# zhouxian/act3d-chained-diffuser

Measured on AMD Instinct MI355X. Metric: train samples/sec (Act3D keypose fwd+bwd+AdamW step), higher is better.
Workload: dtype fp16 / bf16 MFMA on two-part operands (x = hi + lo; fp32 accumulate) in attention; fp32-accurate linears (f32 MFMA; bf16x3 MFMA from 4096 rows); bf16 frozen backbone + FPN; 1 GPU; Act3D keypose training step, 18-PerAct-task shapes: 4 cameras 256x256, 3 ghost-point levels, 1000 ghost points (333/level), E=60, frozen synthetic CLIP-RN50-shaped backbone + trainable FPN included in the step; per_gpu_batch_keyframes=64, global_batch=64, parallelism=dp1, hipgraph=True, backbone_prefetch=True

## Files before the change

### act3d-chained-diffuser_amd/csrc/a3d_common.h

```cpp
#pragma once
#include <hip/hip_runtime.h>
#include <stdint.h>
#include <math.h>

#define A3D_OK 0
#define A3D_ERR_ARG (-22)
#define A3D_ERR_LAUNCH (-5)
#define A3D_ERR_NOMEM (-12)

namespace a3d {

void set_error(const char* fmt, ...);
int check_launch(const char* what);
int zero_words(void* p, size_t bytes, hipStream_t s, const char* what);

typedef __attribute__((ext_vector_type(4))) float f32x4;
typedef __attribute__((ext_vector_type(8))) short s16x8;
typedef __attribute__((ext_vector_type(8))) __bf16 bf16x8;
typedef __attribute__((ext_vector_type(4))) short s16x4;

constexpr int HD = 15;
constexpr float LOG2E_F = 1.4426950408889634f;
constexpr int HDP = 16;

// ... 83 lines not shown
  *sn = (q & 2) ? -s0 : s0;
  *cs = ((q + 1) & 2) ? -c0 : c0;
}
__host__ __device__ __forceinline__ void fast_sincos(float x, float* sn, float* cs) {
#if defined(A3D_LIBM_SINCOS) && defined(__HIP_DEVICE_COMPILE__)
  sincosf(x, sn, cs);
#else
  if (fabsf(x) >= 200.0f) {
    const double t = (double)x;
    const double k = rint(t * 0.15915494309189535);
    x = (float)fma(-k, 2.4492935982947064e-16, fma(-k, 6.283185307179586, t));
  }
  sincos_poly(x, sn, cs);
#endif
}

__device__ __forceinline__ float add_rn(float a, float b) {
#pragma clang fp contract(off)
  return a + b;
}
__device__ __forceinline__ float sub_rn(float a, float b) {
#pragma clang fp contract(off)
  return a - b;
}
__device__ __forceinline__ float mul_rn(float a, float b) {
#pragma clang fp contract(off)
  return a * b;
}
__device__ __forceinline__ float sqrt_rn(float a) { return __builtin_sqrtf(a); }

__host__ __device__ __forceinline__ void philox4x32_10(uint32_t c0, uint32_t c1, uint32_t c2, uint32_t c3,
                                                       uint32_t k0, uint32_t k1, uint32_t out[4]) {
  for (int r = 0; r < 10; ++r) {
    const uint64_t p0 = (uint64_t)0xD2511F53u * c0;
    const uint64_t p1 = (uint64_t)0xCD9E8D57u * c2;
    const uint32_t n0 = (uint32_t)(p1 >> 32) ^ c1 ^ k0;
    const uint32_t n1 = (uint32_t)p1;
    const uint32_t n2 = (uint32_t)(p0 >> 32) ^ c3 ^ k1;
    const uint32_t n3 = (uint32_t)p0;
    c0 = n0; c1 = n1; c2 = n2; c3 = n3;
    k0 += 0x9E3779B9u; k1 += 0xBB67AE85u;
  }
  out[0] = c0; out[1] = c1; out[2] = c2; out[3] = c3;
}

struct DropKey { uint32_t k0, k1; };
__device__ __forceinline__ DropKey drop_key(const unsigned long long* state) {
  const unsigned long long seed = state[0], offs = state[1];
  const unsigned long long key = seed + offs * 0x9E3779B97F4A7C15ull;
  DropKey k;
  k.k0 = (uint32_t)key;
  k.k1 = (uint32_t)(key >> 32);
  return k;
}
__device__ __forceinline__ uint32_t drop_keep8(DropKey k, uint32_t c0, uint32_t c1, uint32_t c2, uint32_t site,
                                               uint32_t thr16) {
  uint32_t r[4];
  philox4x32_10(c0, c1, c2, site, k.k0, k.k1, r);
  uint32_t bits = 0;
#pragma unroll
  for (int w = 0; w < 4; ++w) {
    bits |= ((r[w] & 0xFFFFu) >= thr16 ? 1u : 0u) << (2 * w);
    bits |= ((r[w] >> 16) >= thr16 ? 1u : 0u) << (2 * w + 1);
  }
  return bits;
}

__device__ __forceinline__ bool xcd_decode(int per_group, int ngroups, int& group, int& within) {
  const int id = blockIdx.x;
  const int xcd = id & 7, slot = id >> 3;
  group = (slot / per_group) * 8 + xcd;
  within = slot % per_group;
  return group < ngroups;
}
static inline int xcd_grid(int ngroups, int per_group) { return ((ngroups + 7) / 8) * 8 * per_group; }

static inline int cdiv(int a, int b) { return (a + b - 1) / b; }

bool conv1x1_deep_serves(int K, int N);
int conv1x1_deep_slabs(size_t M, int K, int N);
int conv1x1_deep_launch(const void* x, const void* w, const float* in_scale, const float* in_shift, int in_relu, void* y, float* partial,
                        size_t M, int K, int N, hipStream_t s);

}
```

### act3d-chained-diffuser_amd/csrc/attention16.hip

```cpp
#include "attn_ring.h"
#include "../../include/act3d_hip.h"
#include <stdlib.h>

namespace a3d {

constexpr float LO_SPAN = 6.0f;
constexpr int A3D_ATTN16_V_ROWS = 1, A3D_ATTN16_NOGRAD = 2;
constexpr int FWD_NB = 4;
template <bool DROP, int QT, int PP, bool VR>
__global__ __launch_bounds__(256, 2) void attn16_fwd_kernel(
    const unsigned short* __restrict__ Qr, const unsigned short* __restrict__ Kr, const unsigned short* __restrict__ Vp,
    const unsigned char* __restrict__ kmask, float* __restrict__ O, float* __restrict__ LSE2, float* __restrict__ Op,
    float* __restrict__ Mp, float* __restrict__ Lp, int B, int H, int Lq, int Lqp, int S, int Sp, int nsplit,
    const unsigned long long* __restrict__ drop_state, unsigned int drop_site, unsigned int drop_thr, float drop_scale) {
  __shared__ __attribute__((aligned(16))) unsigned short Ksm[FWD_NB][C16 * 32];
  __shared__ __attribute__((aligned(16))) unsigned short Vsm[FWD_NB][4 * 16 * 32];
  __shared__ unsigned int maskW[MASKW];

  const int t = threadIdx.x, lane = t & 63;
  const int wave = __builtin_amdgcn_readfirstlane(t >> 6);
  const int li = lane & 15, g = lane >> 4;
  constexpr int QW = 64 * QT;
  const int tiles_x = (Lqp + QW - 1) / QW;
  int group, within;
// ... 568 lines not shown
      s16x8 kf[2], vf[2], kp[2];
#pragma unroll
      for (int T = 0; T < 2; ++T) {
        kf[T] = *reinterpret_cast<const s16x8*>(kb + DQ_KJ(hf * 2 + T));
        vf[T] = *reinterpret_cast<const s16x8*>(kb + C16 * 32 + DQ_KJ(hf * 2 + T));
      }
      kp[0] = tr_frag(tb0 + hf * 1024, 0, 128);
      kp[1] = tr_frag(tb1 + hf * 1024, 0, 128);
      f32x4 sT[QT][2], dpT[QT][2];
      if (masked) {
        const unsigned int word = maskW[c * 2 + hf];
#pragma unroll
        for (int T = 0; T < 2; ++T) {
          const f32x4 b4 = bias_of(word, g, T);
#pragma unroll
          for (int u = 0; u < QT; ++u) sT[u][T] = mfma_f16(kf[T], qhi[u], cS[u] + b4);
        }
      } else {
#pragma unroll
        for (int u = 0; u < QT; ++u)
#pragma unroll
          for (int T = 0; T < 2; ++T) sT[u][T] = mfma_f16(kf[T], qhi[u], cS[u]);
      }
#pragma unroll
      for (int u = 0; u < QT; ++u)
#pragma unroll
        for (int T = 0; T < 2; ++T) {
          dpT[u][T] = mfma_f16(vf[T], dohi[u], cD[u]);
          sT[u][T] = mfma_f16(kf[T], qlo[u], sT[u][T]);
        }
#pragma unroll
      for (int u = 0; u < QT; ++u)
#pragma unroll
        for (int T = 0; T < 2; ++T) dpT[u][T] = mfma_f16(vf[T], dolo[u], dpT[u][T]);
#pragma unroll
      for (int u = 0; u < QT; ++u) {
        unsigned int keep = 0xFFu;
        if (DROP) keep = drop_keep8(dkey, (uint32_t)(c * (C16 / 8) + hf * 4 + g), (uint32_t)(qbase + u * 16 + li), (uint32_t)bh, drop_site, drop_thr);
        unsigned int w[4], wl[4];
#pragma unroll
        for (int T = 0; T < 2; ++T) {
#pragma unroll
          for (int pr = 0; pr < 2; ++pr) {
            const float p0 = __builtin_amdgcn_exp2f(sT[u][T][2 * pr]), p1 = __builtin_amdgcn_exp2f(sT[u][T][2 * pr + 1]);
            float g0, g1;
            if (DROP) {
              const int j = T * 4 + 2 * pr;
              const float m0 = ((keep >> j) & 1u) ? drop_scale : 0.f, m1 = ((keep >> (j + 1)) & 1u) ? drop_scale : 0.f;
              g0 = p0 * __builtin_fmaf(m0, dpT[u][T][2 * pr], nd[u]);
              g1 = p1 * __builtin_fmaf(m1, dpT[u][T][2 * pr + 1], nd[u]);
            } else {
              g0 = p0 * dpT[u][T][2 * pr];
              g1 = p1 * dpT[u][T][2 * pr + 1];
            }
            if (GP == 2) pk_f16_2(g0, g1, w[T * 2 + pr], wl[T * 2 + pr]);
            else w[T * 2 + pr] = pk_f16(g0, g1);
          }
        }
        const s16x8 gf = __builtin_bit_cast(s16x8, (u32x4_){w[0], w[1], w[2], w[3]});
        f32x4& acc = hf ? acc1[u] : acc0[u];
        acc = mfma_f16(kp[0], gf, acc);
        acc = mfma_f16(kp[1], gf, acc);
        if (GP == 2) acc = mfma_f16(kp[0], __builtin_bit_cast(s16x8, (u32x4_){wl[0], wl[1], wl[2], wl[3]}), acc);
      }
    }
  }
  wait_vm<0>();
#undef DQ_KJ
#pragma unroll
  for (int u = 0; u < QT; ++u) {
    if (!active[u]) continue;
    const size_t row = (((size_t)sp * B + b) * H + h) * Lqp + qbase + u * 16 + li;
    f32x4 acc;
#pragma unroll
    for (int r = 0; r < 4; ++r) acc[r] = (acc0[u][r] + acc1[u][r]) * rs[u];
    *reinterpret_cast<f32x4*>(&dQp[row * HDP + g * 4]) = acc;
  }
}

constexpr int DKV_NB = 2;
template <bool DROP, int KT, int GP>
__global__ __launch_bounds__(256, 2) void attn16_bwd_dkv_kernel(
    const unsigned short* __restrict__ pack, const unsigned short* __restrict__ Kr, const unsigned short* __restrict__ Vr,
    const unsigned char* __restrict__ kmask, float* __restrict__ dK, float* __restrict__ dV, int B, int H, int Lqp, int S,
    int Sp, const unsigned long long* __restrict__ drop_state, unsigned int drop_site, unsigned int drop_thr,
    float drop_scale) {
  __shared__ __attribute__((aligned(16))) unsigned short pk[DKV_NB][PK_HALFS];
  __shared__ __attribute__((aligned(16))) unsigned char maskS[2][DROP ? 8 * KT * C16 : 16];
  const int t = threadIdx.x, lane = t & 63;
  const int wave = __builtin_amdgcn_readfirstlane(t >> 6);
  const int li = lane & 15, g = lane >> 4;
  constexpr int KW = 64 * KT;
  int group, within;
  if (!xcd_decode((Sp + KW - 1) / KW, B * H, group, within)) return;
  group = __builtin_amdgcn_readfirstlane(group);
  within = __builtin_amdgcn_readfirstlane(within);
  const int b = __builtin_amdgcn_readfirstlane(group / H), h = group - b * H;
  const size_t bh = (size_t)b * H + h;

  s16x8 khh[KT], kll[KT], vhh[KT], vll[KT];
  f32x4 bias4[KT];
  int key[KT];
#pragma unroll
  for (int u = 0; u < KT; ++u) {
    key[u] = within * KW + (wave * KT + u) * 16 + li;
    khh[u] = s16x8{0, 0, 0, 0, 0, 0, 0, 0};
    kll[u] = khh[u]; vhh[u] = khh[u]; vll[u] = khh[u];
    bool valid = false;
    if (key[u] < Sp) {
      const unsigned short* kp = Kr + (bh * Sp + key[u]) * 32;
      const unsigned short* vp = Vr + (bh * Sp + key[u]) * 32;
      khh[u] = *reinterpret_cast<const s16x8*>(kp + (g & 1) * 8);
      kll[u] = *reinterpret_cast<const s16x8*>(kp + 16 + (g & 1) * 8);
      vhh[u] = *reinterpret_cast<const s16x8*>(vp + (g & 1) * 8);
      vll[u] = *reinterpret_cast<const s16x8*>(vp + 16 + (g & 1) * 8);
      valid = key[u] < S;
      if (valid && kmask) valid = kmask[(size_t)b * S + key[u]] == 0;
    }
    const float bias_k = valid ? 0.f : -INFINITY;
    bias4[u] = f32x4{bias_k, bias_k, bias_k, bias_k};
  }
  const bool masked = (kmask != nullptr) || (within * KW + KW > S);
  bool live[KT];
  bool any_live = false;
#pragma unroll
  for (int u = 0; u < KT; ++u) {
    live[u] = within * KW + (wave * KT + u) * 16 < S;
    any_live = any_live || live[u];
  }
  DropKey dkey = {0u, 0u};
  if (DROP) dkey = drop_key(drop_state);
#pragma unroll
  for (int u = 0; u < KT; ++u) { A3D_PIN(khh[u]); A3D_PIN(kll[u]); A3D_PIN(vhh[u]); A3D_PIN(vll[u]); A3D_PIN(bias4[u]); }
  if (DROP) { A3D_PIN(dkey.k0); A3D_PIN(dkey.k1); }

  const int nch = Lqp / C16;
  const unsigned short* pbase = pack + bh * nch * (size_t)PK_HALFS + wave * 2560 + lane * 8;
  auto issue = [&](int c, int slot) {
    const unsigned short* src = pbase + (size_t)min(c, nch - 1) * PK_HALFS;
#pragma unroll
    for (int i = 0; i < 5; ++i) glds16(src + i * 512, &pk[slot][wave * 2560 + i * 512]);
  };

#define DKV_QJ(j) ((((j) >> 1) * 32 + ((j) & 1) * 4) * 32)
  const int qoff0 = tile_off((li >> 2) * 8 + (li & 3), g);
  const int poff = plane_off(li, g);

  f32x4 dk0[KT], dk1[KT], dv0[KT], dv1[KT];
#pragma unroll
  for (int u = 0; u < KT; ++u) { dk0[u] = f32x4{0.f, 0.f, 0.f, 0.f}; dk1[u] = dk0[u]; dv0[u] = dk0[u]; dv1[u] = dk0[u]; }
  int e_ref = -1000;
#pragma unroll
  for (int i = 0; i < DKV_NB - 1; ++i) issue(i, i);
  for (int c = 0; c < nch; ++c) {
    const int slot = c % DKV_NB;
    wait_vm<5 * (DKV_NB - 2)>();
    ring_barrier();
    issue(c + DKV_NB - 1, (slot + DKV_NB - 1) % DKV_NB);
    const unsigned short* P = pk[slot];
    const int e_c = __builtin_amdgcn_readfirstlane(*reinterpret_cast<const int*>(P + PK_HDR));
    if (e_c <= -1000) continue;
    const int halves = __builtin_amdgcn_readfirstlane(reinterpret_cast<const int*>(P + PK_HDR)[1]);
    if (e_c != e_ref) {
      if (e_ref > -1000) {
        const float f = ldexpf(1.0f, min(e_ref - e_c, 126));
#pragma unroll
        for (int u = 0; u < KT; ++u)
#pragma unroll
          for (int r = 0; r < 4; ++r) { dk0[u][r] *= f; dk1[u][r] *= f; dv0[u][r] *= f; dv1[u][r] *= f; }
// ... 26 lines not shown
#pragma unroll
      for (int pl = 0; pl < 2; ++pl) {
        qtp[pl] = *reinterpret_cast<const s16x8*>(Pp + PK_QPL + ((pl * 2 + hf) * 16) * 32);
        otp[pl] = *reinterpret_cast<const s16x8*>(Pp + PK_OPL + ((pl * 2 + hf) * 16) * 32);
      }
      f32x4 s[KT][2], dp[KT][2];
      if (masked) {
#pragma unroll
        for (int u = 0; u < KT; ++u)
#pragma unroll
          for (int T = 0; T < 2; ++T) s[u][T] = mfma_f16(qf[T], khh[u], nl4[T] + bias4[u]);
      } else {
#pragma unroll
        for (int u = 0; u < KT; ++u)
#pragma unroll
          for (int T = 0; T < 2; ++T) s[u][T] = mfma_f16(qf[T], khh[u], nl4[T]);
      }
#pragma unroll
      for (int u = 0; u < KT; ++u)
#pragma unroll
        for (int T = 0; T < 2; ++T) {
          dp[u][T] = mfma_f16(of[T], vhh[u], DROP ? f32x4{0.f, 0.f, 0.f, 0.f} : nd4[T]);
          s[u][T] = mfma_f16(qf[T], kll[u], s[u][T]);
        }
#pragma unroll
      for (int u = 0; u < KT; ++u)
#pragma unroll
        for (int T = 0; T < 2; ++T) dp[u][T] = mfma_f16(of[T], vll[u], dp[u][T]);
#pragma unroll
      for (int u = 0; u < KT; ++u) {
        if (!live[u]) continue;
        unsigned long long keep8 = 0;
        if (DROP) keep8 = *reinterpret_cast<const unsigned long long*>(&maskS[c & 1][((wave * KT + u) * 2 + (li >> 3)) * C16 + hf * 32 + g * 8]);
        unsigned int pw[4], pl_[4], gw[4], gl[4];
#pragma unroll
        for (int T = 0; T < 2; ++T) {
#pragma unroll
          for (int pr = 0; pr < 2; ++pr) {
            float p0 = __builtin_amdgcn_exp2f(s[u][T][2 * pr]), p1 = __builtin_amdgcn_exp2f(s[u][T][2 * pr + 1]);
            float g0, g1;
            if (DROP) {
              const int j = T * 4 + 2 * pr;
              const float m0 = ((keep8 >> (8 * j + (li & 7))) & 1ull) ? drop_scale : 0.f;
              const float m1 = ((keep8 >> (8 * (j + 1) + (li & 7))) & 1ull) ? drop_scale : 0.f;
              g0 = p0 * __builtin_fmaf(m0, dp[u][T][2 * pr], nd4[T][2 * pr]);
              g1 = p1 * __builtin_fmaf(m1, dp[u][T][2 * pr + 1], nd4[T][2 * pr + 1]);
              p0 *= m0;
              p1 *= m1;
            } else {
              g0 = p0 * dp[u][T][2 * pr];
              g1 = p1 * dp[u][T][2 * pr + 1];
            }
#ifdef A3D_BF16_SPLIT_RNE
            pk_bf16_2(p0, p1, pw[T * 2 + pr], pl_[T * 2 + pr]);
            pk_bf16_2(g0, g1, gw[T * 2 + pr], gl[T * 2 + pr]);
#else
            pk_bf16_2t(p0, p1, pw[T * 2 + pr], pl_[T * 2 + pr]);
            pk_bf16_2t(g0, g1, gw[T * 2 + pr], gl[T * 2 + pr]);
#endif
          }
        }
        const s16x8 pf = __builtin_bit_cast(s16x8, (u32x4_){pw[0], pw[1], pw[2], pw[3]});
        const s16x8 gf = __builtin_bit_cast(s16x8, (u32x4_){gw[0], gw[1], gw[2], gw[3]});
        f32x4& dv = hf ? dv1[u] : dv0[u];
        f32x4& dk = hf ? dk1[u] : dk0[u];
        dv = mfma_bf16_16x16x32(otp[0], pf, dv);
        dk = mfma_bf16_16x16x32(qtp[0], gf, dk);
        dv = mfma_bf16_16x16x32(otp[1], pf, dv);
        dk = mfma_bf16_16x16x32(qtp[1], gf, dk);
        dv = mfma_bf16_16x16x32(otp[0], __builtin_bit_cast(s16x8, (u32x4_){pl_[0], pl_[1], pl_[2], pl_[3]}), dv);
        dk = mfma_bf16_16x16x32(qtp[0], __builtin_bit_cast(s16x8, (u32x4_){gl[0], gl[1], gl[2], gl[3]}), dk);
      }
    }
  }
  wait_vm<0>();
#undef DKV_QJ
  const float sk = (e_ref > -1000) ? ldexpf(1.0f, e_ref - (int)B_OFF) : 0.f, sv = sk * LOG2E_F;
#pragma unroll
  for (int u = 0; u < KT; ++u) {
    if (key[u] >= Sp) continue;
    f32x4 dk, dv;
#pragma unroll
    for (int r = 0; r < 4; ++r) { dk[r] = (dk0[u][r] + dk1[u][r]) * sk; dv[r] = (dv0[u][r] + dv1[u][r]) * sv; }
    *reinterpret_cast<f32x4*>(&dK[(bh * Sp + key[u]) * HDP + g * 4]) = dk;
    *reinterpret_cast<f32x4*>(&dV[(bh * Sp + key[u]) * HDP + g * 4]) = dv;
  }
}

}

using namespace a3d;

int a3d::attn16_check_shapes(const char* fn, int B, int H, int Lq, int Lqp, int S, int Sp, int nsplit, int qmod) {
  if (B <= 0 || H <= 0 || Lq <= 0 || Lqp < Lq || (Lqp % qmod) != 0 || S <= 0 || Sp < S || (Sp % C16) != 0 || nsplit < 1 ||
      nsplit > 64 || Sp > MASKW * 32) {
    set_error("%s: bad argument (B=%d H=%d Lq=%d Lqp=%d S=%d Sp=%d nsplit=%d; need Lqp %% %d == 0, Sp %% 64 == 0, Sp <= %d)", fn,
              B, H, Lq, Lqp, S, Sp, nsplit, qmod, MASKW * 32);
    return A3D_ERR_ARG;
  }
  return A3D_OK;
}

static int drop_params(const char* fn, const unsigned long long* drop_state, float drop_p, bool& drop, unsigned int& thr,
                       float& dscale) {
  drop = drop_state != nullptr && drop_p > 0.f;
  if (drop_state && !(drop_p >= 0.f && drop_p < 1.f)) {
    set_error("%s: dropout probability %g outside [0, 1)", fn, (double)drop_p);
    return A3D_ERR_ARG;
  }
  thr = drop ? (unsigned int)lrintf(drop_p * 65536.0f) : 0u;
  dscale = drop ? 1.0f / (1.0f - drop_p) : 1.0f;
  return A3D_OK;
}

static int attn16_fwd_launch(const char* fn, const void* Qr, const void* Kr, const void* Vp, const unsigned char* kmask, float* O,
                             float* LSE2, float* ws, int B, int H, int Lq, int Lqp, int S, int Sp, int nsplit,
                             const unsigned long long* drop_state, unsigned int drop_site, float drop_p, int flags, void* stream);
extern "C" int a3d_attn16_fwd(const void* Qr, const void* Kr, const void* Vp, const unsigned char* kmask, float* O,
                              float* LSE2, float* ws, int B, int H, int Lq, int Lqp, int S, int Sp, int nsplit,
                              const unsigned long long* drop_state, unsigned int drop_site, float drop_p, void* stream) {
  return attn16_fwd_launch("a3d_attn16_fwd", Qr, Kr, Vp, kmask, O, LSE2, ws, B, H, Lq, Lqp, S, Sp, nsplit, drop_state, drop_site,
                           drop_p, 0, stream);
}
extern "C" int a3d_attn16_fwd_rows(const void* Qr, const void* Kr, const void* Vr, const unsigned char* kmask, float* O,
                                   float* LSE2, float* ws, int B, int H, int Lq, int Lqp, int S, int Sp, int nsplit,
                                   const unsigned long long* drop_state, unsigned int drop_site, float drop_p, int nograd,
                                   void* stream) {
  return attn16_fwd_launch("a3d_attn16_fwd_rows", Qr, Kr, Vr, kmask, O, LSE2, ws, B, H, Lq, Lqp, S, Sp, nsplit, drop_state,
                           drop_site, drop_p, A3D_ATTN16_V_ROWS | (nograd ? A3D_ATTN16_NOGRAD : 0), stream);
}
static int attn16_fwd_launch(const char* fn, const void* Qr, const void* Kr, const void* Vp, const unsigned char* kmask, float* O,
                             float* LSE2, float* ws, int B, int H, int Lq, int Lqp, int S, int Sp, int nsplit,
                             const unsigned long long* drop_state, unsigned int drop_site, float drop_p, int flags, void* stream) {
  const bool v_rows = (flags & A3D_ATTN16_V_ROWS) != 0, nograd = (flags & A3D_ATTN16_NOGRAD) != 0;
  int rc = attn16_check_shapes(fn, B, H, Lq, Lqp, S, Sp, nsplit, 16);
  if (rc) return rc;
  if (!Qr || !Kr || !Vp || !O || !LSE2 || (nsplit > 1 && !ws)) { set_error("%s: null pointer", fn); return A3D_ERR_ARG; }
  bool drop; unsigned int thr; float dscale;
  rc = drop_params(fn, drop_state, drop_p, drop, thr, dscale);
  if (rc) return rc;
  hipStream_t s = (hipStream_t)stream;
  const size_t rows = (size_t)B * H * Lqp;
  float* Op = ws;
  float* Mp = ws ? ws + (size_t)nsplit * rows * HDP : nullptr;
  float* Lp = ws ? Mp + (size_t)nsplit * rows : nullptr;
  static const int qt_env = getenv("A3D_ATTN_QT") ? atoi(getenv("A3D_ATTN_QT")) : 0;
  const int QT = qt_env ? qt_env : (Lq > 64 ? 2 : 1);
  dim3 grid(xcd_grid(B * H, cdiv(Lqp, 64 * QT) * nsplit));
  const unsigned long long* nostate = nullptr;
  static const bool fast = getenv("A3D_ATTN_FAST") && atoi(getenv("A3D_ATTN_FAST")) != 0;
#define A3D_L16F(DROPV, QTV, PPV, ST, SITE, THR, SC)                                                                     \
  do { if (v_rows) hipLaunchKernelGGL((attn16_fwd_kernel<DROPV, QTV, PPV, true>), grid, dim3(256), 0, s, (const unsigned short*)Qr, \
                     (const unsigned short*)Kr, (const unsigned short*)Vp, kmask, O, LSE2, Op, Mp, Lp, B, H, Lq, Lqp, S, \
                     Sp, nsplit, ST, SITE, THR, SC);                                                                     \
       else hipLaunchKernelGGL((attn16_fwd_kernel<DROPV, QTV, PPV, false>), grid, dim3(256), 0, s, (const unsigned short*)Qr, \
                     (const unsigned short*)Kr, (const unsigned short*)Vp, kmask, O, LSE2, Op, Mp, Lp, B, H, Lq, Lqp, S, \
                     Sp, nsplit, ST, SITE, THR, SC); } while (0)
  static const bool lo_adapt_env = getenv("A3D_ATTN_LO_ADAPT") && atoi(getenv("A3D_ATTN_LO_ADAPT")) != 0;
  const bool lo_adapt = nograd || lo_adapt_env;
#define A3D_L16F_PP(DROPV, QTV, ST, SITE, THR, SC)                                                                       \
  do { if (fast) A3D_L16F(DROPV, QTV, 1, ST, SITE, THR, SC); else if (lo_adapt) A3D_L16F(DROPV, QTV, 2, ST, SITE, THR, SC);   \
       else A3D_L16F(DROPV, QTV, 3, ST, SITE, THR, SC); } while (0)
  if (drop) {
    if (QT == 2) A3D_L16F_PP(true, 2, drop_state, drop_site, thr, dscale);
    else A3D_L16F_PP(true, 1, drop_state, drop_site, thr, dscale);
  } else {
    if (QT == 2) A3D_L16F_PP(false, 2, nostate, 0u, 0u, 1.0f);
    else A3D_L16F_PP(false, 1, nostate, 0u, 0u, 1.0f);
  }
#undef A3D_L16F_PP
#undef A3D_L16F
  rc = check_launch(fn);
  if (rc) return rc;
  if (nsplit > 1) rc = attn16_launch_combine(Op, Mp, Lp, O, LSE2, B, H, Lq, Lqp, nsplit, s);
  return rc;
}

int a3d::attn16_launch_combine(const float* Op, const float* Mp, const float* Lp, float* O, float* LSE2, int B, int H, int Lq,
                               int Lqp, int nsplit, hipStream_t s) {
  const size_t rows = (size_t)B * H * Lqp;
  const int cg = (int)std::min<size_t>((rows * HDP + 255) / 256, 4096);
  hipLaunchKernelGGL(attn16_combine_kernel, dim3(cg), dim3(256), 0, s, Op, Mp, Lp, O, LSE2, B, H, Lq, Lqp, nsplit);
  return check_launch("a3d_attn16_fwd(combine)");
}

extern "C" size_t a3d_attn16_bwd_pack_bytes(int B, int H, int Lqp) {
  return (size_t)B * H * (Lqp / C16) * PK_HALFS * sizeof(unsigned short);
}

extern "C" int a3d_attn16_bwd(const void* Qr, const void* Qp, const void* Kr, const void* Kp, const void* Vr,
                              const unsigned char* kmask, const float* O, const float* dO, const float* LSE2, void* dOr,
                              void* pack, float* D, int* rexp, float* dQp, float* dK, float* dV, int B, int H, int Lq,
                              int Lqp, int S, int Sp, int nsplit, const unsigned long long* drop_state,
                              unsigned int drop_site, float drop_p, void* stream) {
  int rc = attn16_check_shapes("a3d_attn16_bwd", B, H, Lq, Lqp, S, Sp, nsplit, 64);
  if (rc) return rc;
  (void)Qp; (void)Kp;
  if (!Qr || !Kr || !Vr || !O || !dO || !LSE2 || !dOr || !pack || !D || !rexp || !dQp || !dK || !dV) {
    set_error("a3d_attn16_bwd: null pointer");
    return A3D_ERR_ARG;
  }
  bool drop; unsigned int thr; float dscale;
  rc = drop_params("a3d_attn16_bwd", drop_state, drop_p, drop, thr, dscale);
  if (rc) return rc;
  hipStream_t s = (hipStream_t)stream;
  const size_t lds = (size_t)Lqp * 12 + (size_t)2 * PREP_GROUP * 64 * 64;
  constexpr size_t PREP_LDS_MAX = 150 * 1024;
  if (lds > PREP_LDS_MAX) {
    const size_t max_lqp = (PREP_LDS_MAX - (size_t)2 * PREP_GROUP * 64 * 64) / 12 / 64 * 64;
    set_error("a3d_attn16_bwd: Lqp = %d exceeds the per-(b, h) row sort of the prep kernel (12 B of LDS per query: Lqp <= %zu); "
              "use the bf16x3 backward (a3d_attn_bwd_bf16) for longer query sets", Lqp, max_lqp);
    return A3D_ERR_ARG;
  }
  static bool attr_set = false;
  if (!attr_set) {
    (void)hipFuncSetAttribute((const void*)attn16_bwd_prep_kernel, hipFuncAttributeMaxDynamicSharedMemorySize, (int)PREP_LDS_MAX);
    attr_set = true;
  }
  hipLaunchKernelGGL(attn16_bwd_prep_kernel, dim3(B * H), dim3(256), lds, s, dO, O, LSE2, (const unsigned short*)Qr,
                     (unsigned short*)dOr, D, rexp, (unsigned short*)pack, B, H, Lq, Lqp);
  rc = check_launch("a3d_attn16_bwd(prep)");
  if (rc) return rc;
  static const int qt_env = getenv("A3D_ATTN_QT") ? atoi(getenv("A3D_ATTN_QT")) : 0;
  const int QT = qt_env ? qt_env : (Lq > 64 ? 2 : 1);
  const int KT = qt_env ? qt_env : (((size_t)B * H * (Sp / 128) >= 1024 && Lq > 16) ? 2 : 1);
  const dim3 gq(xcd_grid(B * H, cdiv(Lqp, 64 * QT) * nsplit)), gk(xcd_grid(B * H, cdiv(Sp, 64 * KT)));
  const unsigned long long* nostate = nullptr;
  static const bool fast = getenv("A3D_ATTN_FAST") && atoi(getenv("A3D_ATTN_FAST")) != 0;
#define A3D_L16Q_(DROPV, QTV, GPV, ST, SITE, THR, SC)                                                                     \
  hipLaunchKernelGGL((attn16_bwd_dq_kernel<DROPV, QTV, GPV>), gq, dim3(256), 0, s, (const unsigned short*)Qr,            \
                     (const unsigned short*)Kr, (const unsigned short*)Vr, kmask,                                         \
                     (const unsigned short*)dOr, LSE2, D, rexp, dQp, B, H, Lq, Lqp, S, Sp, nsplit, ST, SITE, THR, SC)
#define A3D_L16K_(DROPV, KTV, GPV, ST, SITE, THR, SC)                                                                     \
  hipLaunchKernelGGL((attn16_bwd_dkv_kernel<DROPV, KTV, GPV>), gk, dim3(256), 0, s, (const unsigned short*)pack,         \
                     (const unsigned short*)Kr, (const unsigned short*)Vr, kmask, dK, dV, B, H, Lqp, S, Sp, ST, SITE,    \
                     THR, SC)
#define A3D_L16Q(DROPV, QTV, ST, SITE, THR, SC) \
  do { if (fast) A3D_L16Q_(DROPV, QTV, 1, ST, SITE, THR, SC); else A3D_L16Q_(DROPV, QTV, 2, ST, SITE, THR, SC); } while (0)
#define A3D_L16K(DROPV, KTV, ST, SITE, THR, SC) \
  do { if (fast) A3D_L16K_(DROPV, KTV, 1, ST, SITE, THR, SC); else A3D_L16K_(DROPV, KTV, 2, ST, SITE, THR, SC); } while (0)
  if (drop) {
    if (QT == 2) A3D_L16Q(true, 2, drop_state, drop_site, thr, dscale);
    else A3D_L16Q(true, 1, drop_state, drop_site, thr, dscale);
  } else {
    if (QT == 2) A3D_L16Q(false, 2, nostate, 0u, 0u, 1.0f);
    else A3D_L16Q(false, 1, nostate, 0u, 0u, 1.0f);
  }
  rc = check_launch("a3d_attn16_bwd(dq)");
  if (rc) return rc;
  if (drop) {
    if (KT == 2) A3D_L16K(true, 2, drop_state, drop_site, thr, dscale);
    else A3D_L16K(true, 1, drop_state, drop_site, thr, dscale);
  } else {
    if (KT == 2) A3D_L16K(false, 2, nostate, 0u, 0u, 1.0f);
    else A3D_L16K(false, 1, nostate, 0u, 0u, 1.0f);
  }
#undef A3D_L16Q
#undef A3D_L16K
#undef A3D_L16Q_
#undef A3D_L16K_
  return check_launch("a3d_attn16_bwd(dkv)");
}
```

### act3d-chained-diffuser_amd/csrc/linear.hip

```cpp
#include "a3d_common.h"
#include "../../include/act3d_hip.h"
#include <stdlib.h>

namespace a3d {

bool linear_split_applicable(const float* X, int ldx, const float* W, int ldw, const float* bias, const float* Y, int ldy,
                             const float* mask, int ldm, int M, int N, int K, int act);
int linear_split_launch(const float* X, int ldx, const float* W, int ldw, const float* bias, float* Y, int ldy, const float* mask,
                        int ldm, int M, int N, int K, int act, int w_transposed, hipStream_t s);
bool linear_wgrad_split_applicable(const float* dY, int lddy, const float* X, int ldx, int M);
int linear_wgrad_split_launch(const float* dY, int lddy, const float* X, int ldx, int has_bias, int M, int N, int K, int nsplit,
                              int rows_per_split, float* partial, hipStream_t s);

constexpr int LT_BM = 64;
constexpr int LT_BN = 64;
constexpr int LT_KC = 64;
constexpr int LT_LD = 68;

__device__ __forceinline__ float4 ld4_guard(const float* p, int k, int K, bool vec) {
  float4 v = make_float4(0.f, 0.f, 0.f, 0.f);
  if (vec && k + 3 < K) return *reinterpret_cast<const float4*>(p);
  if (k + 0 < K) v.x = p[0];
  if (k + 1 < K) v.y = p[1];
  if (k + 2 < K) v.z = p[2];
  if (k + 3 < K) v.w = p[3];
  return v;
}

template <bool WT, bool DROP>
__global__ __launch_bounds__(256) void linear_fwd_kernel(
    const float* __restrict__ X, int ldx, const float* __restrict__ W, int ldw,
    const float* __restrict__ bias, float* __restrict__ Y, int ldy,
    const float* __restrict__ mask, int ldm, int M, int N, int K, int act,
    const unsigned long long* __restrict__ drop_state, uint32_t drop_site, uint32_t drop_thr16, float drop_scale) {
  __shared__ __attribute__((aligned(16))) float Xs[LT_BM * LT_LD];
  __shared__ __attribute__((aligned(16))) float Ws[LT_BN * LT_LD];
  const int t = threadIdx.x;
  const int lane = t & 63, wave = t >> 6;
  const int li = lane & 15, g = lane >> 4;
  const int m0 = blockIdx.x * LT_BM, n0 = blockIdx.y * LT_BN;

  f32x4 acc[4];
#pragma unroll
  for (int i = 0; i < 4; ++i) acc[i] = f32x4{0.f, 0.f, 0.f, 0.f};

  const bool x_vec = ((ldx & 3) == 0) && ((((uintptr_t)X) & 15) == 0);
  const bool w_vec = ((ldw & 3) == 0) && ((((uintptr_t)W) & 15) == 0);
  const int sr = t >> 2, sk = (t & 3) * 4;
  const int tk = t >> 4, tn = (t & 15) * 4;

  float4 xr[4], wr[4];
  auto load_chunk = [&](int k0) {
#pragma unroll
    for (int i = 0; i < 4; ++i) {
      const int k = k0 + sk + 16 * i;
      const int m = m0 + sr;
      xr[i] = (m < M && k < K) ? ld4_guard(X + (size_t)m * ldx + k, k, K, x_vec) : make_float4(0.f, 0.f, 0.f, 0.f);
      if (!WT) {
        const int n = n0 + sr;
        wr[i] = (n < N && k < K) ? ld4_guard(W + (size_t)n * ldw + k, k, K, w_vec) : make_float4(0.f, 0.f, 0.f, 0.f);
      } else {
        const int kk = k0 + tk + 16 * i, n = n0 + tn;
        wr[i] = (kk < K && n < N) ? ld4_guard(W + (size_t)kk * ldw + n, n, N, w_vec) : make_float4(0.f, 0.f, 0.f, 0.f);
      }
    }
  };
  auto store_chunk = [&]() {
#pragma unroll
    for (int i = 0; i < 4; ++i) {
      *reinterpret_cast<float4*>(&Xs[sr * LT_LD + sk + 16 * i]) = xr[i];
      if (!WT) {
        *reinterpret_cast<float4*>(&Ws[sr * LT_LD + sk + 16 * i]) = wr[i];
      } else {
        const int kk = tk + 16 * i;
        Ws[(tn + 0) * LT_LD + kk] = wr[i].x;
        Ws[(tn + 1) * LT_LD + kk] = wr[i].y;
        Ws[(tn + 2) * LT_LD + kk] = wr[i].z;
        Ws[(tn + 3) * LT_LD + kk] = wr[i].w;
      }
    }
  };

  load_chunk(0);
  for (int k0 = 0; k0 < K; k0 += LT_KC) {
    store_chunk();
    __syncthreads();
    if (k0 + LT_KC < K) load_chunk(k0 + LT_KC);
    const int ksteps = min(4, (K - k0 + 15) >> 4);
    for (int s4 = 0; s4 < ksteps; ++s4) {
      const float4 a = *reinterpret_cast<const float4*>(&Xs[(wave * 16 + li) * LT_LD + s4 * 16 + g * 4]);
#pragma unroll
      for (int nt = 0; nt < 4; ++nt) {
        const float4 b = *reinterpret_cast<const float4*>(&Ws[(nt * 16 + li) * LT_LD + s4 * 16 + g * 4]);
        acc[nt] = mfma_f32_16x16x4(a.x, b.x, acc[nt]);
        acc[nt] = mfma_f32_16x16x4(a.y, b.y, acc[nt]);
// ... 36 lines not shown
__global__ __launch_bounds__(256) void linear_wgrad_kernel(
    const float* __restrict__ dY, int lddy, const float* __restrict__ X, int ldx,
    float* __restrict__ dW, int lddw, float* __restrict__ db, int M, int N, int K, int rows_per_split,
    float* __restrict__ partial) {
  __shared__ __attribute__((aligned(16))) float Ys[WG_MC * WG_LD];
  __shared__ __attribute__((aligned(16))) float Xs[WG_MC * WG_LD];
  const int t = threadIdx.x;
  const int lane = t & 63, wave = t >> 6;
  const int li = lane & 15, g = lane >> 4;
  const int n0 = blockIdx.x * 64, k0 = blockIdx.y * 64;
  const int mbeg = blockIdx.z * rows_per_split;
  const int mend = min(M, mbeg + rows_per_split);
  const int KE = db ? K + 1 : K;

  f32x4 acc[4];
#pragma unroll
  for (int i = 0; i < 4; ++i) acc[i] = f32x4{0.f, 0.f, 0.f, 0.f};

  const bool y_vec = ((lddy & 3) == 0) && ((((uintptr_t)dY) & 15) == 0) && ((n0 & 3) == 0);
  const bool x_vec = ((ldx & 3) == 0) && ((((uintptr_t)X) & 15) == 0);
  const int sm = t >> 4, sc = (t & 15) * 4;
  float4 yr[4], xr[4];
  auto load_stage = [&](int mb) {
#pragma unroll
    for (int i = 0; i < 4; ++i) {
      const int m = mb + sm + 16 * i;
      float4 vy = make_float4(0.f, 0.f, 0.f, 0.f), vx = vy;
      if (m < mend) {
        vy = ld4_guard(dY + (size_t)m * lddy + n0 + sc, n0 + sc, N, y_vec);
        const int k = k0 + sc;
        vx = ld4_guard(X + (size_t)m * ldx + k, k, K, x_vec);
        if (db) {
          if (k + 0 == K) vx.x = 1.f;
          if (k + 1 == K) vx.y = 1.f;
          if (k + 2 == K) vx.z = 1.f;
          if (k + 3 == K) vx.w = 1.f;
        }
      }
      yr[i] = vy;
      xr[i] = vx;
    }
  };
  load_stage(mbeg);
  for (int mb = mbeg; mb < mend; mb += WG_MC) {
#pragma unroll
    for (int i = 0; i < 4; ++i) {
      *reinterpret_cast<float4*>(&Ys[(sm + 16 * i) * WG_LD + sc]) = yr[i];
      *reinterpret_cast<float4*>(&Xs[(sm + 16 * i) * WG_LD + sc]) = xr[i];
    }
    __syncthreads();
    if (mb + WG_MC < mend) load_stage(mb + WG_MC);
    const int msteps = min(4, (mend - mb + 15) >> 4);
    for (int mm = 0; mm < msteps; ++mm) {
      float a[4];
#pragma unroll
      for (int j = 0; j < 4; ++j) a[j] = Ys[(mm * 16 + g * 4 + j) * WG_LD + wave * 16 + li];
#pragma unroll
      for (int kt = 0; kt < 4; ++kt) {
#pragma unroll
        for (int j = 0; j < 4; ++j) {
          const float b = Xs[(mm * 16 + g * 4 + j) * WG_LD + kt * 16 + li];
          acc[kt] = mfma_f32_16x16x4(a[j], b, acc[kt]);
        }
      }
    }
    __syncthreads();
  }
#pragma unroll
  for (int kt = 0; kt < 4; ++kt) {
    const int k = k0 + kt * 16 + li;
    if (k >= KE) continue;
#pragma unroll
    for (int r = 0; r < 4; ++r) {
      const int n = n0 + wave * 16 + g * 4 + r;
      if (n >= N) continue;
      const float v = acc[kt][r];
      if (partial) partial[((size_t)blockIdx.z * N + n) * KE + k] = v;
      else if (k < K) atomicAdd(&dW[(size_t)n * lddw + k], v);
      else atomicAdd(&db[n], v);
    }
  }
}

__global__ __launch_bounds__(1024) void wgrad_reduce_kernel(const float* __restrict__ partial, int nsplit,
                                                            float* __restrict__ dW, int lddw, float* __restrict__ db,
                                                            int N, int K, int KE) {
  __shared__ float red[16][64];
  const int lane = threadIdx.x & 63, zg = threadIdx.x >> 6;
  const int idx = blockIdx.x * 64 + lane;
  const int total = N * KE;
  float s0 = 0.f, s1 = 0.f;
  if (idx < total) {
    int z = zg;
    for (; z + 16 < nsplit; z += 32) {
      s0 += partial[(size_t)z * total + idx];
      s1 += partial[(size_t)(z + 16) * total + idx];
    }
    if (z < nsplit) s0 += partial[(size_t)z * total + idx];
  }
  red[zg][lane] = s0 + s1;
  __syncthreads();
  if (zg != 0 || idx >= total) return;
  float v = 0.f;
#pragma unroll
  for (int u = 0; u < 16; ++u) v += red[u][lane];
  const int n = idx / KE, k = idx - n * KE;
  if (k < K) dW[(size_t)n * lddw + k] += v;
  else db[n] += v;
}

__global__ __launch_bounds__(256) void add_ln_fwd_kernel(
    const float* __restrict__ A, const float* __restrict__ R, const float* __restrict__ gamma,
    const float* __restrict__ beta, float* __restrict__ Y, float* __restrict__ mean_out,
    float* __restrict__ rstd_out, int M, int E, float eps) {
  const int lane = threadIdx.x & 63;
  const int wave_global = blockIdx.x * 4 + (threadIdx.x >> 6);
  const int nwaves = gridDim.x * 4;
  for (int m = wave_global; m < M; m += nwaves) {
    float v[8];
    float s = 0.f;
#pragma unroll
    for (int i = 0; i < 8; ++i) {
      const int e = lane + i * 64;
      float x = 0.f;
      if (e < E) {
        x = A[(size_t)m * E + e];
        if (R) x += R[(size_t)m * E + e];
      }
      v[i] = x;
      s += x;
    }
    const float mean = wave_sum(s) / (float)E;
    float q = 0.f;
#pragma unroll
    for (int i = 0; i < 8; ++i) {
      const int e = lane + i * 64;
      if (e < E) { const float d = v[i] - mean; q += d * d; }
    }
    const float var = wave_sum(q) / (float)E;
    const float rstd = 1.0f / sqrtf(var + eps);
#pragma unroll
    for (int i = 0; i < 8; ++i) {
      const int e = lane + i * 64;
      if (e < E) Y[(size_t)m * E + e] = (v[i] - mean) * rstd * gamma[e] + beta[e];
    }
    if (lane == 0) { mean_out[m] = mean; rstd_out[m] = rstd; }
  }
}

__global__ __launch_bounds__(256) void add_ln_bwd_kernel(
    const float* __restrict__ A, const float* __restrict__ R, const float* __restrict__ gamma,
    const float* __restrict__ mean_in, const float* __restrict__ rstd_in,
    const float* __restrict__ dY, float* __restrict__ dS, float* __restrict__ dgamma,
    float* __restrict__ dbeta, int M, int E) {
  __shared__ float red_g[4][512];
  __shared__ float red_b[4][512];
  const int lane = threadIdx.x & 63, wave = threadIdx.x >> 6;
  const int wave_global = blockIdx.x * 4 + wave;
  const int nwaves = gridDim.x * 4;
  float pg[8], pb[8];
#pragma unroll
  for (int i = 0; i < 8; ++i) { pg[i] = 0.f; pb[i] = 0.f; }
  for (int m = wave_global; m < M; m += nwaves) {
    const float mean = mean_in[m], rstd = rstd_in[m];
    float xh[8], gy[8];
    float s1 = 0.f, s2 = 0.f;
#pragma unroll
    for (int i = 0; i < 8; ++i) {
      const int e = lane + i * 64;
      xh[i] = 0.f; gy[i] = 0.f;
      if (e < E) {
        float x = A[(size_t)m * E + e];
        if (R) x += R[(size_t)m * E + e];
        const float dy = dY[(size_t)m * E + e];
        xh[i] = (x - mean) * rstd;
        gy[i] = dy * gamma[e];
        pg[i] += dy * xh[i];
        pb[i] += dy;
        s1 += gy[i];
        s2 += gy[i] * xh[i];
      }
    }
    s1 = wave_sum(s1) / (float)E;
    s2 = wave_sum(s2) / (float)E;
#pragma unroll
    for (int i = 0; i < 8; ++i) {
      const int e = lane + i * 64;
      if (e < E) dS[(size_t)m * E + e] = rstd * (gy[i] - s1 - xh[i] * s2);
    }
  }
  if (dgamma) {
// ... 27 lines not shown
  const int e0 = l * 4;
  const bool act = e0 < E;
  float gm[4] = {0.f, 0.f, 0.f, 0.f};
  if (act) {
#pragma unroll
    for (int j = 0; j < 4; ++j) gm[j] = gamma[e0 + j];
  }
  float pg[4] = {0.f, 0.f, 0.f, 0.f}, pb[4] = {0.f, 0.f, 0.f, 0.f};
  const int m_beg = blockIdx.x * rows_per_wg, m_end = min(M, m_beg + rows_per_wg);
  const float inv_e = 1.0f / (float)E;
  for (int m0 = m_beg + wave * RPW; m0 < m_end; m0 += 4 * RPW) {
    const int m = m0 + sub;
    const bool ok = act && m < m_end;
    float4 x = make_float4(0.f, 0.f, 0.f, 0.f), dy = x;
    float mean = 0.f, rstd = 0.f;
    if (ok) {
      x = *reinterpret_cast<const float4*>(A + (size_t)m * E + e0);
      if (R) {
        const float4 r = *reinterpret_cast<const float4*>(R + (size_t)m * E + e0);
        x.x += r.x; x.y += r.y; x.z += r.z; x.w += r.w;
      }
      dy = *reinterpret_cast<const float4*>(dY + (size_t)m * E + e0);
      mean = mean_in[m];
      rstd = rstd_in[m];
    }
    const float xv[4] = {x.x, x.y, x.z, x.w}, dv[4] = {dy.x, dy.y, dy.z, dy.w};
    float xh[4], gy[4], s1 = 0.f, s2 = 0.f;
#pragma unroll
    for (int j = 0; j < 4; ++j) {
      xh[j] = ok ? (xv[j] - mean) * rstd : 0.f;
      gy[j] = dv[j] * gm[j];
      pg[j] += dv[j] * xh[j];
      pb[j] += dv[j];
      s1 += gy[j];
      s2 += gy[j] * xh[j];
    }
#pragma unroll
    for (int o = 1; o < LPR; o <<= 1) { s1 += __shfl_xor(s1, o, 64); s2 += __shfl_xor(s2, o, 64); }
    s1 *= inv_e;
    s2 *= inv_e;
    if (ok) {
      const float4 o = make_float4(rstd * (gy[0] - s1 - xh[0] * s2), rstd * (gy[1] - s1 - xh[1] * s2),
                                   rstd * (gy[2] - s1 - xh[2] * s2), rstd * (gy[3] - s1 - xh[3] * s2));
      *reinterpret_cast<float4*>(dS + (size_t)m * E + e0) = o;
      if (DROP) {
        const size_t idx = (size_t)m * E + e0;
        const uint32_t keep = drop_keep8(drop_key(drop_state), (uint32_t)(idx >> 3), (uint32_t)(idx >> 35), 0xFFFFFFFFu, drop_site,
                                         drop_thr16) >> (idx & 4);
        *reinterpret_cast<float4*>(dSd + idx) = make_float4((keep & 1u) ? o.x * drop_scale : 0.f, (keep & 2u) ? o.y * drop_scale : 0.f,
                                                            (keep & 4u) ? o.z * drop_scale : 0.f, (keep & 8u) ? o.w * drop_scale : 0.f);
      }
    }
  }
  if (dgamma) {
#pragma unroll
    for (int j = 0; j < 4; ++j) { red_g[wave * RPW + sub][e0 + j] = pg[j]; red_b[wave * RPW + sub][e0 + j] = pb[j]; }
    __syncthreads();
    for (int e = t; e < E; e += 256) {
      float sg = 0.f, sb = 0.f;
#pragma unroll
      for (int u = 0; u < SLOTS; ++u) { sg += red_g[u][e]; sb += red_b[u][e]; }
      atomicAdd(&dgamma[e], sg);
      atomicAdd(&dbeta[e], sb);
    }
  }
}

}

using namespace a3d;

extern "C" int a3d_linear_fwd(const float* X, int ldx, const float* W, int ldw, const float* bias,
                              float* Y, int ldy, const float* mask, int ldm, int M, int N, int K,
                              int act, int w_transposed, void* stream) {
  if (!X || !W || !Y || M < 0 || N <= 0 || K <= 0 || ldx < K || ldy < N) {
    set_error("a3d_linear_fwd: bad argument (M=%d N=%d K=%d ldx=%d ldy=%d)", M, N, K, ldx, ldy);
    return A3D_ERR_ARG;
  }
  if (act == 2 && !mask) { set_error("a3d_linear_fwd: act=2 needs a mask"); return A3D_ERR_ARG; }
  if (M == 0) return A3D_OK;
  dim3 grid(cdiv(M, LT_BM), cdiv(N, LT_BN));
  hipStream_t s = (hipStream_t)stream;
  if (linear_split_applicable(X, ldx, W, ldw, bias, Y, ldy, mask, ldm, M, N, K, act))
    return linear_split_launch(X, ldx, W, ldw, bias, Y, ldy, mask, ldm, M, N, K, act, w_transposed, s);
  if (w_transposed)
    hipLaunchKernelGGL((linear_fwd_kernel<true, false>), grid, dim3(256), 0, s, X, ldx, W, ldw, bias, Y, ldy, mask, ldm, M, N, K, act,
                       (const unsigned long long*)nullptr, 0u, 0u, 0.f);
  else
    hipLaunchKernelGGL((linear_fwd_kernel<false, false>), grid, dim3(256), 0, s, X, ldx, W, ldw, bias, Y, ldy, mask, ldm, M, N, K, act,
                       (const unsigned long long*)nullptr, 0u, 0u, 0.f);
  return check_launch("a3d_linear_fwd");
}

static int linear_drop_params(const char* fn, float p, uint32_t* thr16, float* scale) {
  if (!(p >= 0.f) || !(p < 1.f)) {
    set_error("%s: dropout probability %g outside [0, 1)", fn, (double)p);
    return A3D_ERR_ARG;
  }
  *thr16 = (uint32_t)lrintf(p * 65536.0f);
  *scale = 1.0f / (1.0f - p);
  return A3D_OK;
}

extern "C" int a3d_linear_fwd_drop(const float* X, int ldx, const float* W, int ldw, const float* bias, float* Y, int ldy,
                                   const float* mask, int ldm, int M, int N, int K, int act, int w_transposed,
                                   const unsigned long long* state, unsigned int site, float p, void* stream) {
  if (!X || !W || !Y || !state || M < 0 || N <= 0 || K <= 0 || ldx < K || ldy != N || act == 3) {
    set_error("a3d_linear_fwd_drop: bad argument (M=%d N=%d K=%d ldx=%d ldy=%d act=%d; the output must be contiguous, ldy == N, and "
              "act 3 has no dropout form)", M, N, K, ldx, ldy, act);
    return A3D_ERR_ARG;
  }
  if (act == 2 && !mask) { set_error("a3d_linear_fwd_drop: act=2 needs a mask"); return A3D_ERR_ARG; }
  uint32_t thr; float scale;
  int rc = linear_drop_params("a3d_linear_fwd_drop", p, &thr, &scale);
  if (rc) return rc;
  if (M == 0) return A3D_OK;
  if ((N & 7) || linear_split_applicable(X, ldx, W, ldw, bias, Y, ldy, mask, ldm, M, N, K, act)) {
    rc = a3d_linear_fwd(X, ldx, W, ldw, bias, Y, ldy, mask, ldm, M, N, K, act, w_transposed, stream);
    return rc ? rc : a3d_dropout(Y, Y, (size_t)M * N, state, site, p, stream);
  }
  dim3 grid(cdiv(M, LT_BM), cdiv(N, LT_BN));
  hipStream_t s = (hipStream_t)stream;
  if (w_transposed)
    hipLaunchKernelGGL((linear_fwd_kernel<true, true>), grid, dim3(256), 0, s, X, ldx, W, ldw, bias, Y, ldy, mask, ldm, M, N, K, act,
                       state, (uint32_t)site, thr, scale);
  else
    hipLaunchKernelGGL((linear_fwd_kernel<false, true>), grid, dim3(256), 0, s, X, ldx, W, ldw, bias, Y, ldy, mask, ldm, M, N, K, act,
                       state, (uint32_t)site, thr, scale);
  return check_launch("a3d_linear_fwd_drop");
}

static int wg_two_stage_min_rows() {
  static const int v = getenv("A3D_WGRAD_TWO_STAGE_MIN_ROWS") ? atoi(getenv("A3D_WGRAD_TWO_STAGE_MIN_ROWS")) : 1024;
  return v;
}

static void wgrad_plan(int M, int N, int KE, bool have_ws, int* nsplit_out, int* rows_out, bool* two_stage) {
  const int tiles = cdiv(N, 64) * cdiv(KE, 64);
  int nsplit;
  *two_stage = have_ws && M >= wg_two_stage_min_rows();
  if (*two_stage) {
    static int target2 = getenv("A3D_WGRAD_WGS2") ? atoi(getenv("A3D_WGRAD_WGS2")) : 1024;
    nsplit = max(1, min(cdiv(M, WG_MC), cdiv(target2, tiles)));
    if (cdiv(M, nsplit) > 256) nsplit = max(nsplit, min(cdiv(M, 256), 4 * cdiv(target2, tiles)));
  } else {
    static int target_wgs = getenv("A3D_WGRAD_WGS") ? atoi(getenv("A3D_WGRAD_WGS")) : 256;
    nsplit = max(1, min(cdiv(M, 256), cdiv(target_wgs, tiles)));
  }
  int rows = cdiv(cdiv(M, nsplit), WG_MC) * WG_MC;
  *nsplit_out = cdiv(M, rows);
  *rows_out = rows;
}

extern "C" size_t a3d_linear_wgrad_ws_bytes(int M, int N, int K, int has_bias) {
  if (M <= 0 || N <= 0 || K <= 0) return 0;
  const int KE = has_bias ? K + 1 : K;
  int nsplit, rows;
  bool two;
  wgrad_plan(M, N, KE, true, &nsplit, &rows, &two);
  return two ? (size_t)nsplit * N * KE * sizeof(float) : 0;
}

extern "C" int a3d_linear_wgrad_ws(const float* dY, int lddy, const float* X, int ldx, float* dW, int lddw,
                                   float* db, int M, int N, int K, float* ws, size_t ws_bytes, void* stream) {
  if (!dY || !X || !dW || M < 0 || N <= 0 || K <= 0) {
    set_error("a3d_linear_wgrad: bad argument (M=%d N=%d K=%d)", M, N, K);
    return A3D_ERR_ARG;
  }
  if (M == 0) return A3D_OK;
  const int KE = db ? K + 1 : K;
  int nsplit, rows;
  bool two_stage;
  wgrad_plan(M, N, KE, ws != nullptr, &nsplit, &rows, &two_stage);
  if (two_stage && ws_bytes < (size_t)nsplit * N * KE * sizeof(float)) {
    set_error("a3d_linear_wgrad_ws: workspace too small (%zu bytes, need %zu)", ws_bytes,
              (size_t)nsplit * N * KE * sizeof(float));
    return A3D_ERR_ARG;
  }
  dim3 grid(cdiv(N, 64), cdiv(KE, 64), nsplit);
  if (two_stage && linear_wgrad_split_applicable(dY, lddy, X, ldx, M)) {
    const int rc = linear_wgrad_split_launch(dY, lddy, X, ldx, db != nullptr, M, N, K, nsplit, rows, ws, (hipStream_t)stream);
    if (rc) return rc;
  } else
  hipLaunchKernelGGL(linear_wgrad_kernel, grid, dim3(256), 0, (hipStream_t)stream, dY, lddy, X, ldx, dW,
                     lddw, db, M, N, K, rows, two_stage ? ws : nullptr);
  if (two_stage)
    hipLaunchKernelGGL(wgrad_reduce_kernel, dim3(cdiv(N * KE, 64)), dim3(1024), 0, (hipStream_t)stream, ws, nsplit, dW,
                       lddw, db, N, K, KE);
  return check_launch("a3d_linear_wgrad");
}

extern "C" int a3d_sq_wgrad_reduce(const float* partial, int nsplit, float* dW, int lddw, float* db, int E, void* stream) {
  if (!partial || !dW || !db || nsplit < 1 || E <= 0) { set_error("a3d_sq_wgrad_reduce: bad argument"); return A3D_ERR_ARG; }
  hipLaunchKernelGGL(wgrad_reduce_kernel, dim3(cdiv(E * (E + 1), 64)), dim3(1024), 0, (hipStream_t)stream, partial, nsplit, dW,
                     lddw, db, E, E, E + 1);
  return check_launch("a3d_sq_wgrad_reduce");
}

extern "C" int a3d_linear_wgrad(const float* dY, int lddy, const float* X, int ldx, float* dW, int lddw,
                                float* db, int M, int N, int K, void* stream) {
  return a3d_linear_wgrad_ws(dY, lddy, X, ldx, dW, lddw, db, M, N, K, nullptr, 0, stream);
}

extern "C" int a3d_add_layernorm_fwd(const float* A, const float* R, const float* gamma, const float* beta,
                                     float* Y, float* mean, float* rstd, int M, int E, float eps,
                                     void* stream) {
  if (!A || !gamma || !beta || !Y || !mean || !rstd || E <= 0 || E > 512 || M < 0) {
    set_error("a3d_add_layernorm_fwd: bad argument (M=%d E=%d)", M, E);
    return A3D_ERR_ARG;
  }
  if (M == 0) return A3D_OK;
  const int grid = min(cdiv(M, 4), 4096);
  hipLaunchKernelGGL(add_ln_fwd_kernel, dim3(grid), dim3(256), 0, (hipStream_t)stream, A, R, gamma, beta, Y,
                     mean, rstd, M, E, eps);
  return check_launch("a3d_add_layernorm_fwd");
}

extern "C" int a3d_add_layernorm_bwd(const float* A, const float* R, const float* gamma, const float* mean,
                                     const float* rstd, const float* dY, float* dS, float* dgamma,
                                     float* dbeta, int M, int E, void* stream) {
  if (!A || !gamma || !mean || !rstd || !dY || !dS || E <= 0 || E > 512 || M < 0 || (!dgamma != !dbeta)) {
    set_error("a3d_add_layernorm_bwd: bad argument (M=%d E=%d)", M, E);
    return A3D_ERR_ARG;
  }
  if (M == 0) return A3D_OK;
  if (E > 64 && E <= 128 && (E & 3) == 0 && ((((uintptr_t)A) | ((uintptr_t)R) | ((uintptr_t)dY) | ((uintptr_t)dS)) & 15) == 0) {
    const int per_pass = E <= 64 ? 16 : 8;
    int rpw = per_pass;
    while (cdiv(M, rpw) > 2048 && rpw < 16 * per_pass) rpw *= 2;
    const int grid = cdiv(M, rpw);
    if (E <= 64)
      hipLaunchKernelGGL((add_ln_bwd_rows_kernel<16, false>), dim3(grid), dim3(256), 0, (hipStream_t)stream, A, R, gamma, mean, rstd, dY, dS,
                         dgamma, dbeta, M, E, rpw, (float*)nullptr, (const unsigned long long*)nullptr, 0u, 0u, 0.f);
    else
      hipLaunchKernelGGL((add_ln_bwd_rows_kernel<32, false>), dim3(grid), dim3(256), 0, (hipStream_t)stream, A, R, gamma, mean, rstd, dY, dS,
                         dgamma, dbeta, M, E, rpw, (float*)nullptr, (const unsigned long long*)nullptr, 0u, 0u, 0.f);
    return check_launch("a3d_add_layernorm_bwd");
  }
  const int grid = min(cdiv(M, 16), 1024);
  hipLaunchKernelGGL(add_ln_bwd_kernel, dim3(grid), dim3(256), 0, (hipStream_t)stream, A, R, gamma, mean,
                     rstd, dY, dS, dgamma, dbeta, M, E);
  return check_launch("a3d_add_layernorm_bwd");
}

extern "C" int a3d_add_layernorm_bwd_drop(const float* A, const float* R, const float* gamma, const float* mean, const float* rstd,
                                          const float* dY, float* dS, float* dS_drop, float* dgamma, float* dbeta, int M, int E,
                                          const unsigned long long* state, unsigned int site, float p, void* stream) {
  if (!A || !gamma || !mean || !rstd || !dY || !dS || !dS_drop || !state || dS_drop == dS || E <= 0 || E > 512 || M < 0 ||
      (!dgamma != !dbeta)) {
    set_error("a3d_add_layernorm_bwd_drop: bad argument (M=%d E=%d; dS_drop must be a second buffer)", M, E);
    return A3D_ERR_ARG;
  }
  uint32_t thr; float scale;
  int rc = linear_drop_params("a3d_add_layernorm_bwd_drop", p, &thr, &scale);
  if (rc) return rc;
  if (M == 0) return A3D_OK;
  if (E > 64 && E <= 128 && (E & 7) == 0 &&
      ((((uintptr_t)A) | ((uintptr_t)R) | ((uintptr_t)dY) | ((uintptr_t)dS) | ((uintptr_t)dS_drop)) & 15) == 0) {
    int rpw = 8;
    while (cdiv(M, rpw) > 2048 && rpw < 128) rpw *= 2;
    hipLaunchKernelGGL((add_ln_bwd_rows_kernel<32, true>), dim3(cdiv(M, rpw)), dim3(256), 0, (hipStream_t)stream, A, R, gamma, mean, rstd,
                       dY, dS, dgamma, dbeta, M, E, rpw, dS_drop, state, (uint32_t)site, thr, scale);
    return check_launch("a3d_add_layernorm_bwd_drop");
  }
  rc = a3d_add_layernorm_bwd(A, R, gamma, mean, rstd, dY, dS, dgamma, dbeta, M, E, stream);
  return rc ? rc : a3d_dropout(dS, dS_drop, (size_t)M * E, state, site, p, stream);
}
```

### act3d-chained-diffuser_amd/csrc/linear_split.hip

```cpp
#include "a3d_common.h"
#include "../../include/act3d_hip.h"
#include <stdlib.h>

namespace a3d {

typedef __attribute__((ext_vector_type(2))) float ls_f32x2;
typedef __attribute__((ext_vector_type(2))) __bf16 ls_bf16x2;

__device__ __forceinline__ void split3(float a, float b, unsigned int& h, unsigned int& m, unsigned int& l) {
  h = __builtin_bit_cast(unsigned int, __builtin_convertvector((ls_f32x2){a, b}, ls_bf16x2));
  float ra = a - __uint_as_float(h << 16), rb = b - __uint_as_float(h & 0xFFFF0000u);
  m = __builtin_bit_cast(unsigned int, __builtin_convertvector((ls_f32x2){ra, rb}, ls_bf16x2));
  ra -= __uint_as_float(m << 16);
  rb -= __uint_as_float(m & 0xFFFF0000u);
  l = __builtin_bit_cast(unsigned int, __builtin_convertvector((ls_f32x2){ra, rb}, ls_bf16x2));
}

template <int WN, bool WT>
__global__ __launch_bounds__(256, 2) void linear_split_kernel(
    const float* __restrict__ X, int ldx, const float* __restrict__ W, int ldw, const float* __restrict__ bias,
    float* __restrict__ Y, int ldy, const float* __restrict__ mask, int ldm, int M, int N, int K, int act) {
  constexpr int WM = 4 / WN, BM = 32 * WM, BN = 64 * WN;
  constexpr int XL = BM * 8 / 256, WL = BN * 8 / 256;
  __shared__ __attribute__((aligned(16))) unsigned short Xs[3][BM * 32];
  __shared__ __attribute__((aligned(16))) unsigned short Ws[3][BN * 32];
  const int t = threadIdx.x, lane = t & 63, wave = t >> 6;
  const int li = lane & 15, g = lane >> 4;
  const int wm = wave / WN, wn = wave % WN;
  const int ncb = (N + BN - 1) / BN, nrb = (M + BM - 1) / BM;
  int rb, cb;
  if (!xcd_decode(ncb, nrb, rb, cb)) return;
  const int m0 = rb * BM, n0 = cb * BN;
  const int ksteps = (K + 31) >> 5;

  const bool w_vec = ((ldw & 3) == 0) && ((((uintptr_t)W) & 15) == 0);
  auto ldw4 = [&](const float* p) {
    if (w_vec) return *reinterpret_cast<const float4*>(p);
    return make_float4(p[0], p[1], p[2], p[3]);
  };
  float4 xr[XL], wr[WL];
  auto load = [&](int ks) {
#pragma unroll
    for (int i = 0; i < XL; ++i) {
      const int idx = t + i * 256, row = idx >> 3, k = ks * 32 + (idx & 7) * 4;
      const int m = min(m0 + row, M - 1);
      xr[i] = (k < K) ? *reinterpret_cast<const float4*>(X + (size_t)m * ldx + k) : make_float4(0.f, 0.f, 0.f, 0.f);
    }
#pragma unroll
    for (int i = 0; i < WL; ++i) {
      const int idx = t + i * 256;
      if (!WT) {
        const int row = idx >> 3, k = ks * 32 + (idx & 7) * 4;
        const int n = min(n0 + row, N - 1);
        wr[i] = (k < K) ? ldw4(W + (size_t)n * ldw + k) : make_float4(0.f, 0.f, 0.f, 0.f);
      } else {
        const int kk = idx / (BN / 4), j = idx - kk * (BN / 4);
        const int k = ks * 32 + kk, n = min(n0 + j * 4, N - 4);
        wr[i] = (k < K) ? ldw4(W + (size_t)k * ldw + n) : make_float4(0.f, 0.f, 0.f, 0.f);
      }
    }
  };
  auto stage = [&]() {
#pragma unroll
    for (int i = 0; i < XL; ++i) {
      const int idx = t + i * 256, row = idx >> 3, s4 = idx & 7;
      unsigned int h0, m0_, l0, h1, m1, l1;
      split3(xr[i].x, xr[i].y, h0, m0_, l0);
      split3(xr[i].z, xr[i].w, h1, m1, l1);
      const int off = plane_off(row, s4 >> 1) + (s4 & 1) * 4;
      *reinterpret_cast<uint2*>(&Xs[0][off]) = make_uint2(h0, h1);
      *reinterpret_cast<uint2*>(&Xs[1][off]) = make_uint2(m0_, m1);
      *reinterpret_cast<uint2*>(&Xs[2][off]) = make_uint2(l0, l1);
    }
#pragma unroll
    for (int i = 0; i < WL; ++i) {
      const int idx = t + i * 256;
      unsigned int h0, m0_, l0, h1, m1, l1;
      split3(wr[i].x, wr[i].y, h0, m0_, l0);
      split3(wr[i].z, wr[i].w, h1, m1, l1);
      if (!WT) {
        const int row = idx >> 3, s4 = idx & 7;
        const int off = plane_off(row, s4 >> 1) + (s4 & 1) * 4;
        *reinterpret_cast<uint2*>(&Ws[0][off]) = make_uint2(h0, h1);
        *reinterpret_cast<uint2*>(&Ws[1][off]) = make_uint2(m0_, m1);
        *reinterpret_cast<uint2*>(&Ws[2][off]) = make_uint2(l0, l1);
      } else {
        const int kk = idx / (BN / 4), j = idx - kk * (BN / 4);
        const unsigned int hs[4] = {h0 & 0xFFFFu, h0 >> 16, h1 & 0xFFFFu, h1 >> 16};
        const unsigned int ms[4] = {m0_ & 0xFFFFu, m0_ >> 16, m1 & 0xFFFFu, m1 >> 16};
        const unsigned int ls[4] = {l0 & 0xFFFFu, l0 >> 16, l1 & 0xFFFFu, l1 >> 16};
#pragma unroll
        for (int e = 0; e < 4; ++e) {
          const int off = plane_off(j * 4 + e, kk >> 3) + (kk & 7);
          Ws[0][off] = (unsigned short)hs[e];
          Ws[1][off] = (unsigned short)ms[e];
          Ws[2][off] = (unsigned short)ls[e];
        }
      }
    }
  };

  f32x4 acc[4][2];
#pragma unroll
  for (int a = 0; a < 4; ++a)
#pragma unroll
    for (int b = 0; b < 2; ++b) acc[a][b] = f32x4{0.f, 0.f, 0.f, 0.f};

  load(0);
  for (int ks = 0; ks < ksteps; ++ks) {
    if (ks > 0) __syncthreads();
    stage();
    __syncthreads();
    if (ks + 1 < ksteps) load(ks + 1);
    s16x8 xa[3][2], wb[3][4];
#pragma unroll
    for (int p = 0; p < 3; ++p) {
#pragma unroll
      for (int tm = 0; tm < 2; ++tm) xa[p][tm] = *reinterpret_cast<const s16x8*>(&Xs[p][plane_off(wm * 32 + tm * 16 + li, g)]);
#pragma unroll
      for (int tn = 0; tn < 4; ++tn) wb[p][tn] = *reinterpret_cast<const s16x8*>(&Ws[p][plane_off(wn * 64 + tn * 16 + li, g)]);
    }
#pragma unroll
    for (int tn = 0; tn < 4; ++tn)
#pragma unroll
      for (int tm = 0; tm < 2; ++tm) {
        f32x4 c = acc[tn][tm];
        c = mfma_bf16_16x16x32(wb[1][tn], xa[1][tm], c);
        c = mfma_bf16_16x16x32(wb[0][tn], xa[2][tm], c);
        c = mfma_bf16_16x16x32(wb[2][tn], xa[0][tm], c);
        c = mfma_bf16_16x16x32(wb[0][tn], xa[1][tm], c);
        c = mfma_bf16_16x16x32(wb[1][tn], xa[0][tm], c);
        c = mfma_bf16_16x16x32(wb[0][tn], xa[0][tm], c);
        acc[tn][tm] = c;
      }
  }

#pragma unroll
  for (int tm = 0; tm < 2; ++tm) {
    const int m = m0 + wm * 32 + tm * 16 + li;
    if (m >= M) continue;
#pragma unroll
    for (int tn = 0; tn < 4; ++tn) {
      const int n = n0 + wn * 64 + tn * 16 + g * 4;
      if (n >= N) continue;
      float4 v = make_float4(acc[tn][tm][0], acc[tn][tm][1], acc[tn][tm][2], acc[tn][tm][3]);
      if (bias) { v.x += bias[n]; v.y += bias[n + 1]; v.z += bias[n + 2]; v.w += bias[n + 3]; }
      if (act == 1) {
        v.x = fmaxf(v.x, 0.f); v.y = fmaxf(v.y, 0.f); v.z = fmaxf(v.z, 0.f); v.w = fmaxf(v.w, 0.f);
      } else if (act == 2) {
        const float4 mk = *reinterpret_cast<const float4*>(mask + (size_t)m * ldm + n);
        v.x = mk.x > 0.f ? v.x : 0.f; v.y = mk.y > 0.f ? v.y : 0.f; v.z = mk.z > 0.f ? v.z : 0.f; v.w = mk.w > 0.f ? v.w : 0.f;
      } else if (act == 3) {
        const float4 old = *reinterpret_cast<const float4*>(Y + (size_t)m * ldy + n);
        v.x += old.x; v.y += old.y; v.z += old.z; v.w += old.w;
      }
      *reinterpret_cast<float4*>(Y + (size_t)m * ldy + n) = v;
    }
  }
}

bool linear_split_applicable(const float* X, int ldx, const float* W, int ldw, const float* bias, const float* Y, int ldy,
                             const float* mask, int ldm, int M, int N, int K, int act) {
  static const bool on = !(getenv("A3D_LINEAR_SPLIT") && atoi(getenv("A3D_LINEAR_SPLIT")) == 0);
  static const int min_m = getenv("A3D_LINEAR_SPLIT_MIN_M") ? atoi(getenv("A3D_LINEAR_SPLIT_MIN_M")) : 4096;
  if (!on || M < min_m || K < 32 || N < 32 || (K & 3) || (N & 3) || ((ldx | ldy) & 3)) return false;
  if ((((uintptr_t)X | (uintptr_t)Y) & 15) != 0) return false;
  if (act == 2 && (!mask || (ldm & 3) || (((uintptr_t)mask) & 15) != 0)) return false;
  return true;
}

int linear_split_launch(const float* X, int ldx, const float* W, int ldw, const float* bias, float* Y, int ldy, const float* mask,
                        int ldm, int M, int N, int K, int act, int w_transposed, hipStream_t s) {
  const bool wide = N > 64;
  const int BM = wide ? 64 : 128, BN = wide ? 128 : 64;
  dim3 grid(xcd_grid(cdiv(M, BM), cdiv(N, BN)));
#define A3D_LS(WNV, WTV) \
  hipLaunchKernelGGL((linear_split_kernel<WNV, WTV>), grid, dim3(256), 0, s, X, ldx, W, ldw, bias, Y, ldy, mask, ldm, M, N, K, act)
  if (wide) { if (w_transposed) A3D_LS(2, true); else A3D_LS(2, false); }
  else { if (w_transposed) A3D_LS(1, true); else A3D_LS(1, false); }
#undef A3D_LS
  return check_launch("a3d_linear_fwd(split)");
}

__global__ __launch_bounds__(256, 2) void linear_wgrad_split_kernel(
    const float* __restrict__ dY, int lddy, const float* __restrict__ X, int ldx, int has_bias, int M, int N, int K,
    int rows_per_split, float* __restrict__ partial) {
  __shared__ __attribute__((aligned(16))) unsigned short Ys[3][64 * 32];
  __shared__ __attribute__((aligned(16))) unsigned short Xt[3][64 * 32];
  const int t = threadIdx.x, lane = t & 63, wave = t >> 6;
  const int li = lane & 15, g = lane >> 4;
  const int n0 = blockIdx.x * 64, k0 = blockIdx.y * 64;
  const int mbeg = blockIdx.z * rows_per_split;
  const int mend = min(M, mbeg + rows_per_split);
  const int KE = has_bias ? K + 1 : K;
  const int mp = t >> 4, c4 = (t & 15) * 4;

  auto ld4 = [&](const float* base, int ld, int m, int c, int C, bool ones) {
    float4 v = make_float4(0.f, 0.f, 0.f, 0.f);
    if (m >= mend) return v;
    const float* p = base + (size_t)m * ld + c;
    if (c + 3 < C) return *reinterpret_cast<const float4*>(p);
    if (c + 0 < C) v.x = p[0]; else if (ones && c + 0 == C) v.x = 1.f;
    if (c + 1 < C) v.y = p[1]; else if (ones && c + 1 == C) v.y = 1.f;
    if (c + 2 < C) v.z = p[2]; else if (ones && c + 2 == C) v.z = 1.f;
    if (c + 3 < C) v.w = p[3]; else if (ones && c + 3 == C) v.w = 1.f;
    return v;
  };
  float4 yr[2], xr[2];
  auto load = [&](int mb) {
#pragma unroll
    for (int u = 0; u < 2; ++u) {
      yr[u] = ld4(dY, lddy, mb + 2 * mp + u, n0 + c4, N, false);
      xr[u] = ld4(X, ldx, mb + 2 * mp + u, k0 + c4, K, has_bias != 0);
    }
  };
  auto stage_one = [&](unsigned short (*T)[64 * 32], const float4& r0, const float4& r1) {
    const float a[4] = {r0.x, r0.y, r0.z, r0.w}, b[4] = {r1.x, r1.y, r1.z, r1.w};
#pragma unroll
    for (int e = 0; e < 4; ++e) {
      unsigned int h, m, l;
      split3(a[e], b[e], h, m, l);
      const int off = plane_off(c4 + e, mp >> 2) + (mp & 3) * 2;
      *reinterpret_cast<unsigned int*>(&T[0][off]) = h;
      *reinterpret_cast<unsigned int*>(&T[1][off]) = m;
      *reinterpret_cast<unsigned int*>(&T[2][off]) = l;
    }
  };

  f32x4 acc[4];
#pragma unroll
  for (int i = 0; i < 4; ++i) acc[i] = f32x4{0.f, 0.f, 0.f, 0.f};
  load(mbeg);
  for (int mb = mbeg; mb < mend; mb += 32) {
    if (mb > mbeg) __syncthreads();
    stage_one(Ys, yr[0], yr[1]);
    stage_one(Xt, xr[0], xr[1]);
    __syncthreads();
    if (mb + 32 < mend) load(mb + 32);
    s16x8 ya[3], xb[3][4];
#pragma unroll
    for (int p = 0; p < 3; ++p) {
      ya[p] = *reinterpret_cast<const s16x8*>(&Ys[p][plane_off(wave * 16 + li, g)]);
#pragma unroll
      for (int kt = 0; kt < 4; ++kt) xb[p][kt] = *reinterpret_cast<const s16x8*>(&Xt[p][plane_off(kt * 16 + li, g)]);
    }
#pragma unroll
    for (int kt = 0; kt < 4; ++kt) {
      f32x4 c = acc[kt];
      c = mfma_bf16_16x16x32(ya[1], xb[1][kt], c);
      c = mfma_bf16_16x16x32(ya[0], xb[2][kt], c);
      c = mfma_bf16_16x16x32(ya[2], xb[0][kt], c);
      c = mfma_bf16_16x16x32(ya[0], xb[1][kt], c);
      c = mfma_bf16_16x16x32(ya[1], xb[0][kt], c);
      c = mfma_bf16_16x16x32(ya[0], xb[0][kt], c);
      acc[kt] = c;
    }
  }
#pragma unroll
  for (int kt = 0; kt < 4; ++kt) {
    const int k = k0 + kt * 16 + li;
    if (k >= KE) continue;
#pragma unroll
    for (int r = 0; r < 4; ++r) {
      const int n = n0 + wave * 16 + g * 4 + r;
      if (n < N) partial[((size_t)blockIdx.z * N + n) * KE + k] = acc[kt][r];
    }
  }
}

bool linear_wgrad_split_applicable(const float* dY, int lddy, const float* X, int ldx, int M) {
  static const bool on = !(getenv("A3D_LINEAR_SPLIT") && atoi(getenv("A3D_LINEAR_SPLIT")) == 0) &&
                         !(getenv("A3D_WGRAD_SPLIT") && atoi(getenv("A3D_WGRAD_SPLIT")) == 0);
  static const int min_m = getenv("A3D_LINEAR_SPLIT_MIN_M") ? atoi(getenv("A3D_LINEAR_SPLIT_MIN_M")) : 4096;
  return on && M >= min_m && ((lddy | ldx) & 3) == 0 && ((((uintptr_t)dY | (uintptr_t)X) & 15) == 0);
}

int linear_wgrad_split_launch(const float* dY, int lddy, const float* X, int ldx, int has_bias, int M, int N, int K, int nsplit,
                              int rows_per_split, float* partial, hipStream_t s) {
  const int KE = has_bias ? K + 1 : K;
  dim3 grid(cdiv(N, 64), cdiv(KE, 64), nsplit);
  hipLaunchKernelGGL(linear_wgrad_split_kernel, grid, dim3(256), 0, s, dY, lddy, X, ldx, has_bias, M, N, K, rows_per_split, partial);
  return check_launch("a3d_linear_wgrad(split)");
}

}
```

### act3d-chained-diffuser_amd/lib.py

```python
import ctypes as C
import os

import torch

_PKG_DIR = os.path.dirname(os.path.abspath(__file__))
LIB_PATH = os.path.join(_PKG_DIR, os.path.basename(os.environ.get("A3D_LIB", "libact3d_hip.so")))

_p = C.c_void_p
_i = C.c_int
_f = C.c_float
_z = C.c_size_t
_u64 = C.c_ulonglong



def _struct(name, fields):
    return type(name, (C.Structure,), {"_fields_": [(f, t) for f, t in fields]})


DnHeadParams = _struct("DnHeadParams", [(n, _p) for n in ("enc_w0", "enc_b0", "enc_w1", "enc_b1", "sem", "lang_kv")] +
                       [("S_lang", _i)] + [(n, _p) for n in ("q_w", "q_b", "out_w", "out_b", "ln_g", "ln_b")])
DnCrossParams = _struct("DnCrossParams", [(n, _p) for n in ("sem", "mod", "q_w", "q_b", "freq", "Kf", "Vt")])
DnRestParams = _struct("DnRestParams", [(n, _p) for n in (
    "c_out_w", "c_out_b", "c_ln_g", "c_ln_b", "sem", "s_mod", "s_in_w", "s_in_b", "s_out_w", "s_out_b", "s_ln_g", "s_ln_b", "freq",
    "kmask", "f_mod", "f_w1", "f_b1", "f_w2", "f_b2", "f_ln_g", "f_ln_b")] + [("F", _i)])
DnLayerParams = _struct("DnLayerParams", [("cross", DnCrossParams), ("rest", DnRestParams)])
DnTailParams = _struct("DnTailParams", [(n, _p) for n in (
    "pos_w0", "pos_b0", "pos_w1", "pos_b1", "rot_w0", "rot_b0", "rot_w1", "rot_b1", "noise", "cond_data", "cond_mask", "coef_pos",
    "coef_rot")])

QsParams = _struct("QsParams", [(n, _p) for n in ("wv", "bv", "wo", "bo", "g1", "b1", "w1", "c1", "w2", "c2", "g2", "b2")])
QsGrads = _struct("QsGrads", [(n, _p) for n in ("dwv", "dbv", "dwo", "dbo", "dg1", "db1", "dw1", "dc1", "dw2", "dc2", "dg2", "db2")])

SIGNATURES = {
    "a3d_version": (_i, []),
    "a3d_last_error_string": (C.c_char_p, []),
    "a3d_linear_fwd": (_i, [_p, _i, _p, _i, _p, _p, _i, _p, _i, _i, _i, _i, _i, _i, _p]),
    "a3d_linear_wgrad": (_i, [_p, _i, _p, _i, _p, _i, _p, _i, _i, _i, _p]),
    "a3d_linear_wgrad_ws": (_i, [_p, _i, _p, _i, _p, _i, _p, _i, _i, _i, _p, _z, _p]),
    "a3d_linear_wgrad_ws_bytes": (_z, [_i, _i, _i, _i]),
    "a3d_add_layernorm_fwd": (_i, [_p, _p, _p, _p, _p, _p, _p, _i, _i, _f, _p]),
    "a3d_add_layernorm_bwd": (_i, [_p, _p, _p, _p, _p, _p, _p, _p, _p, _i, _i, _p]),
    "a3d_rope_split_qk": (_i, [_p, _i, _p, _p, _f, _p, _i, _i, _i, _i, _i, _p]),
    "a3d_split_vt": (_i, [_p, _i, _p, _i, _i, _i, _i, _i, _p]),
    "a3d_proj_rope_split": (_i, [_p, _i, _p, _i, _p, _i, _p, _f, _p, _i, _p, _p, _f, _p, _i, _p, _p, _i, _i, _i, _i, _i, _p]),
    "a3d_rope_split": (_i, [_p, _i, _p, _p, _f, _p, _i, _p, _i, _i, _i, _i, _i, _p]),
    "a3d_rope_merge_bwd": (_i, [_p, _i, _p, _p, _f, _p, _i, _i, _i, _i, _i, _i, _p]),
    "a3d_attn_fwd": (_i, [_p, _p, _p, _p, _p, _p, _p, _i, _i, _i, _i, _i, _i, _i, _p]),
    "a3d_attn_fwd_ws_floats": (_z, [_i, _i, _i, _i]),
    "a3d_attn_bwd_bf16": (_i, [_p] * 15 + [_i] * 7 + [_p]),
    "a3d_rope_split16": (_i, [_p, _i, _p, _p, _f, _p, _p, _i, _i, _i, _i, _i, _i, _p]),
    "a3d_proj_rope_split16": (_i, [_p, _i, _p, _i, _p, _i, _p, _f, _p, _p, _i, _p, _f, _p, _p, _i, _p, _i, _i, _i, _i, _i, _p]),
    "a3d_attn16_fwd": (_i, [_p] * 7 + [_i] * 7 + [_p, C.c_uint, _f, _p]),
    "a3d_attn16_fwd_rows": (_i, [_p] * 7 + [_i] * 7 + [_p, C.c_uint, _f, _i, _p]),
    "a3d_conv3x3_tile_count": (_z, [_z, _i, _i]),
    "a3d_conv3x3_dgrad_tiles_ws_ints": (_z, [_z, _i, _i]),
    "a3d_conv3x3_mark_tiles": (_i, [_p, _i, _i, _i, _i, _i, _p, _p]),
    "a3d_conv3x3_dgrad_tiles": (_i, [_p, _p, _p, _p, _p, _z, _i, _i, _p]),
    "a3d_conv3x3_wgrad_tokens_ws_floats": (_z, []),
    "a3d_conv3x3_wgrad_tokens": (_i, [_p, _p, _p, _i, _i, _p, _p, _i, _i, _i, _i, _i, _i, _p]),
    "a3d_attn16_bwd_pack_bytes": (_z, [_i, _i, _i]),
    "a3d_dbg_dn_prof": (_i, [_p]),
    "a3d_attn8_operand_bytes": (_z, [_i, _i, _i]),
    "a3d_attn8_fwd": (_i, [_p] * 8 + [_i] * 7 + [_p]),
    "a3d_attn16_bwd": (_i, [_p] * 16 + [_i] * 7 + [_p, C.c_uint, _f, _p]),
    "a3d_pose_to_signal": (_i, [_p, _p, _p, _i, _i, _p]),
    "a3d_signal_to_pose": (_i, [_p, _p, _p, _i, _i, _p]),
    "a3d_traj_condition": (_i, [_p, _i, _p, _i, _p] + [_p] * 8 + [_i] * 5 + [_p]),
    "a3d_traj_rank": (_i, [_p, _p, _p, _i, _p] + [_f] * 6 + [_p] * 5 + [_i] * 4 + [_p]),
    "a3d_traj_errors": (_i, [_p, _p, _p, _i, _i, _i, _p]),
    "a3d_keypose_errors": (_i, [_p, _p, _p, _p, _i, _p, _i, _i, _i, _p]),
    "a3d_sym_quat_loss": (_i, [_p, _p, _i, _f, _p, _p, _i, _p]),
    "a3d_sq_fwd_ws_floats": (_z, [_i, _i, _i, _i]),
    "a3d_sq_attn_fwd": (_i, [_p, _p, _p, _i, _p, _p, _i, _p, _p, _p, _p, _p, _p, _p, _i, _i, _i, _i, _i, _p]),
    "a3d_sq_bwd_ws_floats": (_z, [_i, _i, _i, _i]),
    "a3d_sq_attn_bwd": (_i, [_p, _p, _p, _i, _p, _p, _i, _p, _p, _p, _p, _p, _p, _p, _p, _p, _i, _p, _p, _i, _p, _i, _i, _i, _i,
                             _i, _p]),
    "a3d_sq_attn_bwd_acc": (_i, [_p, _p, _p, _i, _p, _p, _i, _p, _p, _p, _p, _p, _p, _p, _p, _p, _i, _p, _p, _i, _p, _i, _i, _i, _i,
                                 _i, _i, _p]),
    "a3d_qs_pre_fwd": (_i, [_p, _p, _p, _p, _p, _f, _p, _i, _i, _i, _p]),
    "a3d_qs_pre_bwd": (_i, [_p, _i, _p, _p, _f, _p, _p, _p, _p, _p, _i, _i, _i, _p]),
    "a3d_qs_save_floats": (_z, [_i, _i]),
    "a3d_qs_post_fwd": (_i, [_p, _p, _p, _p, _p, _i, _i, _i, _p]),
    "a3d_qs_post_bwd": (_i, [_p, _p, _p, _p, _p, _p, _p, _p, _p, _i, _i, _i, _p]),
    "a3d_sq_wgrad_reduce": (_i, [_p, _i, _p, _i, _p, _i, _p]),
    "a3d_dn_head": (_i, [_p, _i, _p, _p, _i, _i, _i, _i, _p]),
    "a3d_dn_cross_ws_floats": (_z, [_i, _i, _i]),
    "a3d_dn_cross": (_i, [_p, _p, _i, _p, _p, _i, _i, _i, _i, _i, _i, _i, _p]),
    "a3d_dn_rest": (_i, [_p, _p, _i, _p, _p, _p, _i, _i, _i, _i, _i, _p]),
    "a3d_dn_tail": (_i, [_p, _p, _p, _i, _p, _p, _i, _i, _i, _i, _p]),
    "a3d_dn_tail_sched": (_i, [_p, _p, _p, _i, _p, _p, _i, _i, _i, _i, _i, _p]),
    "a3d_dn_persist_splits": (_i, [_i, _i]),
    "a3d_dn_persist_sync_ints": (_z, [_i, _i, _i, _i]),
    "a3d_dn_persist_kvx_floats": (_z, [_i, _i, _i]),
    "a3d_dn_persist_prof": (_i, [_p, _i, _i, _i, _i, _p]),
    "a3d_dn_persist_xbuf_floats": (_z, [_i, _i]),
    "a3d_dn_persist": (_i, [_p, _i, _i, _i, _p, _p, _p, _p, _p, _p, _p, _p] + [_i] * 10 + [_p]),
    "a3d_dn_persist_sched": (_i, [_p, _i, _i, _i, _p, _p, _p, _p, _p, _p, _p, _p] + [_i] * 12 + [_p]),
    "a3d_dn_persist_group_of": (_i, [_i, _i, _i, _i, _p]),
    "a3d_dn_persist_group": (_i, [_p, _i, _i, _i, _p, _p, _p, _p, _p, _p, _p, _p] + [_i] * 13 + [_p]),
    "a3d_rope_rows_f32": (_i, [_p, _i, _p, _p, _f, _p, _i, _i, _i, _i, _i, _p]),
    "a3d_dropout": (_i, [_p, _p, _z, _p, C.c_uint, _f, _p]),
    "a3d_dropout_mask": (_i, [_p, _z, _p, C.c_uint, C.c_uint, C.c_uint, _f, _p]),
    "a3d_linear_fwd_drop": (_i, [_p, _i, _p, _i, _p, _p, _i, _p, _i, _i, _i, _i, _i, _i, _p, C.c_uint, _f, _p]),
    "a3d_add_layernorm_bwd_drop": (_i, [_p] * 10 + [_i, _i, _p, C.c_uint, _f, _p]),
    "a3d_attn_fwd_dropout": (_i, [_p, _p, _p, _p, _p, _p, _p, _i, _i, _i, _i, _i, _i, _i, _p, C.c_uint, _f, _p]),
    "a3d_attn_bwd_bf16_dropout": (_i, [_p] * 15 + [_i] * 7 + [_p, C.c_uint, _f, _p]),
    "a3d_pcd_downsample": (_i, [_p, _p, _i, _i, _i, _i, _i, _p]),
    "a3d_knn_topk_ws_bytes": (_z, [_i, _i]),
    "a3d_knn_topk": (_i, [_p, _p, _p, _p, _p, _i, _i, _i, _p]),
    "a3d_traj_nn_topk": (_i, [_p, _i, _p, _p, _p, _p, _i, _i, _i, _p]),
    "a3d_build_context": (_i, [_p, _p, _p, _p, _i, _i, _i, _i, _i, _p]),
    "a3d_build_context_bwd": (_i, [_p, _p, _p, _p, _i, _i, _i, _i, _i, _i, _p]),
    "a3d_build_context_bf16": (_i, [_p, _i, _p, _p, _p, _p, _i, _i, _i, _i, _i, _p]),
    "a3d_colsum_rows_ws_floats": (_z, [_i, _i, _i]),
    "a3d_colsum_rows": (_i, [_p, _i, _i, _i, _i, _i, _p, _i, _p, _p]),
    "a3d_build_context_bwd_bf16": (_i, [_p, _p, _p, _i, _p, _i, _i, _i, _i, _i, _i, _p]),
    "a3d_mask_logits_fwd": (_i, [_p, _p, _p, _i, _i, _i, _p]),
    "a3d_mask_logits_bwd": (_i, [_p, _p, _p, _p, _p, _i, _i, _i, _i, _p]),
    "a3d_argmax_gather": (_i, [_p, _p, _p, _p, _i, _i, _p]),
    "a3d_soft_ce_loss": (_i, [_p, _p, _p, _p, _p, _p, _i, _i, _f, _f, _f, _p]),
    "a3d_elem_loss": (_i, [_p, _p, _i, _i, _f, _p, _p, _p]),
    "a3d_scale_by_scalar": (_i, [_p, _p, _p, _z, _p]),
    "a3d_quat_sigmoid_fwd": (_i, [_p, _p, _p, _i, _p]),
    "a3d_quat_sigmoid_bwd": (_i, [_p, _p, _p, _p, _i, _p]),
    "a3d_ortho6d_sigmoid_fwd": (_i, [_p, _p, _p, _i, _p]),
    "a3d_ortho6d_sigmoid_bwd": (_i, [_p, _p, _p, _p, _i, _p]),
    "a3d_select_row_fwd": (_i, [_p, _p, _p, _i, _i, _i, _p]),
    "a3d_select_row_bwd": (_i, [_p, _p, _p, _i, _i, _i, _p]),
    "a3d_sample_ghost_points": (_i, [_p, _p, _p, _f, _p, _i, _i, _i, _i, _p]),
    "a3d_rng_advance": (_i, [_p, _u64, _p]),
    "a3d_philox4x32_10_host": (None, [_p, _p, _p]),
    "a3d_sincos_host": (None, [_p, _p, _p, _z]),
    "a3d_adamw_step": (_i, [_p, _p, _p, _p, _p, _p, _p, _i, _z, _z, _f, _f, _f, _f, _f, _f, _f, _p]),
    "a3d_dbg_mfma_bf16": (_i, [_p, _p, _p, _p]),
    "a3d_dbg_mfma_f32": (_i, [_p, _p, _p, _p]),
    "a3d_dbg_cvt_pk_bf16": (_i, [_p, _p, _i, _p]),
    "a3d_bn_nslab": (_i, [_z, _i]),
    "a3d_bn_grid_cap": (_i, [_i]),
    "a3d_conv1x1_streams": (_i, [_i, _i]),
    "a3d_conv1x1_nslab": (_i, [_z, _i, _i]),
    "a3d_conv1x1_bn_fwd": (_i, [_p, _p, _p, _p, _i, _p, _p, _z, _i, _i, _p]),
    "a3d_conv1x1_topdown_serves": (_i, [_i, _i]),
    "a3d_conv1x1_topdown_fwd": (_i, [_p, _p, _p, _i, _p, _p, _z, _i, _i, _i, _i, _p]),
    "a3d_conv3x3_serves": (_i, [_i, _i, _i, _i]),
    "a3d_conv1x1_deep_mode": (_i, [_i]),
    "a3d_stem_conv_nslab": (_i, [_z, _i, _i]),
    "a3d_stem_conv_bn_fwd": (_i, [_p, _p, _p, _p, _p, _p, _z, _i, _i, _p]),
# ... 85 lines not shown
```

### act3d-chained-diffuser_amd/ops.py

```python
import math
import os

import torch

from . import lib as L

F32 = torch.float32
QKW = 48


def ceil_to(x, m):
    return (x + m - 1) // m * m


def _c(t):
    return t if t.is_contiguous() else t.contiguous()


def grad_buf(p):
    if p.grad is None:
        p.grad = torch.zeros_like(p, memory_format=torch.contiguous_format)
    return p.grad


_freq_cache = {}


def rope_freq(E, device):
    key = (E, str(device))
    if key not in _freq_cache:
        _freq_cache[key] = torch.exp(
            torch.arange(0, E // 3, 2, dtype=F32, device=device) * (-math.log(10000.0) / (E // 3))).contiguous()
    return _freq_cache[key]


DROP_FOLD = os.environ.get("A3D_DROPOUT_FOLD", "1") != "0"


def linear_raw(x_ptr, ldx, W_ptr, ldw, b_ptr, M, N, K, device, act=0, mask_ptr=None, ldm=0, transposed=False,
               out=None, drop=None, site=0):
    y = out if out is not None else torch.empty((M, N), device=device, dtype=F32)
    if drop is not None and DROP_FOLD:
        L.call("a3d_linear_fwd_drop", x_ptr, ldx, W_ptr, ldw, b_ptr, y.data_ptr(), N, mask_ptr, ldm, M, N, K, act,
               1 if transposed else 0, drop.state.data_ptr(), int(site), drop.p, L.stream())
        return y
    L.call("a3d_linear_fwd", x_ptr, ldx, W_ptr, ldw, b_ptr, y.data_ptr(), N, mask_ptr, ldm, M, N, K, act,
           1 if transposed else 0, L.stream())
    if drop is not None:
        L.call("a3d_dropout", y.data_ptr(), y.data_ptr(), y.numel(), drop.state.data_ptr(), int(site), drop.p, L.stream())
    return y


def linear2d(x2d, W, b, act=0, drop=None, site=0):
    M, K = x2d.shape
    N = W.shape[0]
    if W.shape[1] != K or (b is not None and b.numel() != N):
        raise ValueError("linear: activation rows of %d features against a weight of shape %s / bias of %s" %
                         (K, tuple(W.shape), None if b is None else tuple(b.shape)))
    return linear_raw(x2d.data_ptr(), K, W.data_ptr(), W.shape[1], None if b is None else b.data_ptr(), M, N, K,
                      x2d.device, act=act, drop=drop, site=site)


def dgrad2d(dy2d, W, mask=None, drop=None, site=0, accum_into=None):
    M, N = dy2d.shape
    K = W.shape[1]
    if accum_into is not None:
        if mask is not None or drop is not None or tuple(accum_into.shape) != (M, K) or not accum_into.is_contiguous():
            raise ValueError("dgrad2d: accum_into takes a contiguous [M, K] buffer and neither mask nor dropout")
        return linear_raw(dy2d.data_ptr(), N, W.data_ptr(), K, None, M, K, N, dy2d.device, act=3, transposed=True, out=accum_into)
    return linear_raw(dy2d.data_ptr(), N, W.data_ptr(), K, None, M, K, N, dy2d.device,
                      act=2 if mask is not None else 0, mask_ptr=None if mask is None else mask.data_ptr(),
                      ldm=K, transposed=True, drop=drop, site=site)


def wgrad_raw(dy_ptr, lddy, x_ptr, ldx, gw_ptr, lddw, gb_ptr, M, N, K, device, st=None):
    nbytes = L.load().a3d_linear_wgrad_ws_bytes(M, N, K, 0 if gb_ptr is None else 1)
    ws = torch.empty((nbytes // 4,), device=device, dtype=F32) if nbytes else None
    L.call("a3d_linear_wgrad_ws", dy_ptr, lddy, x_ptr, ldx, gw_ptr, lddw, gb_ptr, M, N, K,
           None if ws is None else ws.data_ptr(), nbytes, st if st is not None else L.stream())


def wgrad2d(dy2d, x2d, W, b):
    M, N = dy2d.shape
    K = x2d.shape[1]
    gW = grad_buf(W)
    gb = grad_buf(b) if b is not None else None
    wgrad_raw(dy2d.data_ptr(), N, x2d.data_ptr(), K, gW.data_ptr(), gW.shape[1],
              None if gb is None else gb.data_ptr(), M, N, K, dy2d.device)


def add_layernorm(a2d, r2d, g, b, eps=1e-5):
    M, E = a2d.shape
    y = torch.empty_like(a2d)
    mean = torch.empty((M,), device=a2d.device, dtype=F32)
    rstd = torch.empty((M,), device=a2d.device, dtype=F32)
    L.call("a3d_add_layernorm_fwd", a2d.data_ptr(), None if r2d is None else r2d.data_ptr(), g.data_ptr(),
           b.data_ptr(), y.data_ptr(), mean.data_ptr(), rstd.data_ptr(), M, E, eps, L.stream())
    return y, mean, rstd


def add_layernorm_bwd(a2d, r2d, g, b, mean, rstd, dy2d, drop=None, site=0):
    M, E = a2d.shape
    ds = torch.empty_like(a2d)
    gg, gb = grad_buf(g), grad_buf(b)
    if drop is not None and DROP_FOLD:
        dsd = torch.empty_like(a2d)
        L.call("a3d_add_layernorm_bwd_drop", a2d.data_ptr(), None if r2d is None else r2d.data_ptr(), g.data_ptr(),
               mean.data_ptr(), rstd.data_ptr(), dy2d.data_ptr(), ds.data_ptr(), dsd.data_ptr(), gg.data_ptr(), gb.data_ptr(),
               M, E, drop.state.data_ptr(), int(site), drop.p, L.stream())
        return ds, dsd
    L.call("a3d_add_layernorm_bwd", a2d.data_ptr(), None if r2d is None else r2d.data_ptr(), g.data_ptr(),
           mean.data_ptr(), rstd.data_ptr(), dy2d.data_ptr(), ds.data_ptr(), gg.data_ptr(), gb.data_ptr(), M, E,
           L.stream())
    if drop is not None:
        return ds, dropout_raw(ds, drop, site)
    return ds


ATTN_TARGET_WGS = int(os.environ.get("A3D_ATTN_WGS", "768"))


def pick_nsplit(B, H, Lqp, Sp):
    qw = 128 if Lqp > 64 else 64
    wgs = B * H * ((Lqp + qw - 1) // qw)
    ns = max(1, min(16, Sp // 64, -(-ATTN_TARGET_WGS // wgs)))
    return ns


ATTN_MODE = os.environ.get("A3D_ATTN_MODE", "f16")
if ATTN_MODE not in ("f16", "bf16x3", "fp8"):
    raise ValueError("A3D_ATTN_MODE must be f16, bf16x3 or fp8, got %r" % ATTN_MODE)
LOG2E = 1.4426950408889634


ATTN16_BWD_MAX_LQP = 7296


def _use16(Lq, need_bwd):
    return ATTN_MODE in ("f16", "fp8") and not (need_bwd and ceil_to(Lq, 64) > ATTN16_BWD_MAX_LQP)


PLANE_PARTS = 2


V_PLANES = 2 | 4
V_ROWS = 2 | 8

ROWS_ONLY = os.environ.get("A3D_ATTN_ROWS_ONLY", "1") == "1"


def _rows_only():
    return ROWS_ONLY and ATTN_MODE != "fp8"


def _alloc16(B, H, Lqp, Sp, device, need_bwd):
    hf = torch.float16
    Qr = torch.empty((B, H, Lqp, 32), device=device, dtype=hf)
    Kr = torch.empty((B, H, Sp, 32), device=device, dtype=hf)
    if _rows_only():
        return Qr, Kr, None, None, None, torch.empty((B, H, Sp, 32), device=device, dtype=hf)
# ... 109 lines not shown
        proj(q_in, 0, (qx, scale, Qs.data_ptr(), QKW, nz(Qt)), None, Lq, Lqp)
        if mode == "kv":
            proj(k_in, E, (kx, 1.0, Ks.data_ptr(), QKW, nz(Kt)), (None, 1.0, nz(Vs), 32, Vt.data_ptr()), S, Sp)
        else:
            proj(k_in, E, (kx, 1.0, Ks.data_ptr(), QKW, nz(Kt)), None, S, Sp)
            proj(v_in, 2 * E, (None, 1.0, nz(Vs), 32, Vt.data_ptr()), None, S, Sp)
    return Qs, Ks, Vt, Lqp, Sp, scale, freq, (Qt, Kt, Vs)


class DropCtx:

    def __init__(self, state, p):
        self.state, self.p = state, float(p)


def site_id(name, sub=0):
    import zlib
    return ((zlib.crc32(name.encode()) & 0xFFFFFFF8) | sub) & 0xFFFFFFFF


def dropout_raw(x, drop, site, out=None):
    y = torch.empty_like(x) if out is None else out
    L.call("a3d_dropout", x.data_ptr(), y.data_ptr(), x.numel(), drop.state.data_ptr(), int(site), drop.p, L.stream())
    return y


class DropoutFn(torch.autograd.Function):

    @staticmethod
    def forward(ctx, x, drop, site):
        L.require_gpu(x)
        ctx.drop, ctx.site = drop, site
        return dropout_raw(_c(x), drop, site)

    @staticmethod
    def backward(ctx, dy):
        return dropout_raw(_c(dy), ctx.drop, ctx.site), None, None


def dropout_mask(drop, site, n, bh=None, q=None):
    out = torch.empty((n,), device=drop.state.device, dtype=torch.uint8)
    L.call("a3d_dropout_mask", out.data_ptr(), n, drop.state.data_ptr(), 0xFFFFFFFF if bh is None else int(bh),
           0 if q is None else int(q), int(site), drop.p, L.stream())
    return out


def attn_core_fwd(Qs, Ks, Vt, kmask, B, H, Lq, Lqp, S, Sp, nsplit, drop=None, site=0, need_bwd=False, nograd=False):
    dev = Qs.device
    E = H * 15
    O = torch.empty((B, Lq, E), device=dev, dtype=F32)
    LSE = torch.empty((B, H, Lqp), device=dev, dtype=F32)
    ws = None
    if nsplit > 1:
        ws = torch.empty((nsplit * B * H * Lqp * 18,), device=dev, dtype=F32)
    if Qs.dtype == torch.float16:
        dropping = drop is not None and drop.p > 0
        if ATTN_MODE == "fp8" and not dropping and not need_bwd:
            if Vt.dim() == 4:
                raise RuntimeError("attn_core_fwd: the fp8 mode packs its value operand from value PLANES; these operands were built "
                                   "in the rows-only set (build them with ops.ATTN_MODE == 'fp8')")
            ops8 = torch.empty((L.load().a3d_attn8_operand_bytes(B, H, Sp),), device=dev, dtype=torch.uint8)
            L.call("a3d_attn8_fwd", Qs.data_ptr(), Ks.data_ptr(), Vt.data_ptr(), ops8.data_ptr(),
                   None if kmask is None else kmask.data_ptr(), O.data_ptr(), LSE.data_ptr(),
                   None if ws is None else ws.data_ptr(), B, H, Lq, Lqp, S, Sp, nsplit, L.stream())
            return O, LSE
        if Vt.dim() == 4:
            L.call("a3d_attn16_fwd_rows", Qs.data_ptr(), Ks.data_ptr(), Vt.data_ptr(), None if kmask is None else kmask.data_ptr(),
                   O.data_ptr(), LSE.data_ptr(), None if ws is None else ws.data_ptr(), B, H, Lq, Lqp, S, Sp, nsplit,
                   drop.state.data_ptr() if dropping else None, int(site), drop.p if dropping else 0.0, 1 if nograd else 0, L.stream())
            return O, LSE
        L.call("a3d_attn16_fwd", Qs.data_ptr(), Ks.data_ptr(), Vt.data_ptr(), None if kmask is None else kmask.data_ptr(),
               O.data_ptr(), LSE.data_ptr(), None if ws is None else ws.data_ptr(), B, H, Lq, Lqp, S, Sp, nsplit,
               drop.state.data_ptr() if dropping else None, int(site), drop.p if dropping else 0.0, L.stream())
        return O, LSE
    args = (Qs.data_ptr(), Ks.data_ptr(), Vt.data_ptr(), None if kmask is None else kmask.data_ptr(),
            O.data_ptr(), LSE.data_ptr(), None if ws is None else ws.data_ptr(), B, H, Lq, Lqp, S, Sp, nsplit)
    if drop is not None and drop.p > 0:
        L.call("a3d_attn_fwd_dropout", *args, drop.state.data_ptr(), int(site), drop.p, L.stream())
    else:
        L.call("a3d_attn_fwd", *args, L.stream())
    return O, LSE


def attn_core_bwd(Qs, Ks, Vt, kmask, O, dO, LSE, B, H, Lq, Lqp, S, Sp, nsplit, extra=None, drop=None, site=0):
    dev = Qs.device
    dropping = drop is not None and drop.p > 0
    D = torch.empty((B, H, Lqp), device=dev, dtype=F32)
    dQp = torch.empty((nsplit, B, H, Lqp, 16), device=dev, dtype=F32)
    dK = torch.empty((B, H, Sp, 16), device=dev, dtype=F32)
    dV = torch.empty((B, H, Sp, 16), device=dev, dtype=F32)
    km = None if kmask is None else kmask.data_ptr()
    if Qs.dtype == torch.float16:
        if extra is None or extra[2] is None:
            raise RuntimeError("attn_core_bwd: the forward wrote no value rows (it ran with need_bwd=False on the planes operand set)")
        Vr = extra[2]
        dOr = torch.empty((B, H, Lqp, 32), device=dev, dtype=torch.float16)
        dOp = torch.empty((L.load().a3d_attn16_bwd_pack_bytes(B, H, Lqp) // 2,), device=dev, dtype=torch.float16)
        rexp = torch.empty((B, H, Lqp), device=dev, dtype=torch.int32)
        L.call("a3d_attn16_bwd", Qs.data_ptr(), None, Ks.data_ptr(), None, Vr.data_ptr(), km, O.data_ptr(),
               dO.data_ptr(), LSE.data_ptr(), dOr.data_ptr(), dOp.data_ptr(), D.data_ptr(), rexp.data_ptr(), dQp.data_ptr(),
               dK.data_ptr(), dV.data_ptr(), B, H, Lq, Lqp, S, Sp, nsplit, drop.state.data_ptr() if dropping else None,
               int(site), drop.p if dropping else 0.0, L.stream())
        return dQp, dK, dV
    if extra is None or extra[0] is None:
        raise RuntimeError("attn_core_bwd: the forward wrote no backward operand formats (it ran with need_bwd=False)")
    Qt, Kt, Vs = extra
    dOs = torch.empty((B, H, Lqp, 32), device=dev, dtype=torch.bfloat16)
    dOt = torch.empty((B, H, 2, 16, Lqp), device=dev, dtype=torch.bfloat16)
    args = (Qs.data_ptr(), Qt.data_ptr(), Ks.data_ptr(), Kt.data_ptr(), Vs.data_ptr(), km,
            O.data_ptr(), dO.data_ptr(), LSE.data_ptr(), dOs.data_ptr(), dOt.data_ptr(), D.data_ptr(), dQp.data_ptr(),
            dK.data_ptr(), dV.data_ptr(), B, H, Lq, Lqp, S, Sp, nsplit)
    if dropping:
        L.call("a3d_attn_bwd_bf16_dropout", *args, drop.state.data_ptr(), int(site), drop.p, L.stream())
    else:
        L.call("a3d_attn_bwd_bf16", *args, L.stream())
    return dQp, dK, dV


def rope_merge(dR, nsplit, xyz, freq, scale, out_ptr, ldy, B, N, Npad, E, H):
    L.call("a3d_rope_merge_bwd", dR.data_ptr(), nsplit, None if xyz is None else xyz.data_ptr(), freq.data_ptr(),
           scale, out_ptr, ldy, B, N, Npad, E, H, L.stream())


CTX_GRAD_SINK = os.environ.get("A3D_CTX_SINK", "1") not in ("0", "", "off")


CTX_DEFER = os.environ.get("A3D_CTX_DEFER", "1") not in ("0", "", "off")


class GradSink:
    live = []

    def __init__(self, shape, device):
        self.shape, self.device = tuple(shape), device
        self.buf, self.event = None, None
        self.writers = 0
        self.expected = 0
        self.dkv, self.parked, self.x = None, [], None

    def park(self, x, E2):
        cur = torch.cuda.current_stream(self.device)
        if self.event is not None:
            cur.wait_event(self.event)
        M = self.shape[0] * self.shape[1]
        cap = max(self.expected, len(self.parked) + 1)
        if self.dkv is None:
            self.dkv = torch.empty((M, cap * E2), device=self.device, dtype=F32)
            self.x = x
        else:
            self.dkv.record_stream(cur)
        if (len(self.parked) + 1) * E2 > self.dkv.shape[1]:
            raise RuntimeError("GradSink.park: more deferred writers than registered consumers")
        return self.dkv.data_ptr() + len(self.parked) * E2 * 4, self.dkv.shape[1]

    def parked_done(self, w_kv, gw_kv, gb_kv):
        self.parked.append((w_kv, gw_kv, gb_kv))
        return self.end()

    def _flush_parked(self):
        n = len(self.parked)
        E2, E = self.parked[0][0].shape
        M, K, ld = self.dkv.shape[0], n * E2, self.dkv.shape[1]
        wstack = torch.cat([w for w, _, _ in self.parked], dim=0)
        acc = self.buf is not None
        if not acc:
            self.buf = torch.empty(self.shape, device=self.device, dtype=F32)
        linear_raw(self.dkv.data_ptr(), ld, wstack.data_ptr(), E, None, M, E, K, self.device, act=3 if acc else 0, transposed=True,
                   out=self.buf.view(M, E))
        gstack = torch.zeros((K, E), device=self.device, dtype=F32)
        gbstack = torch.zeros((K,), device=self.device, dtype=F32)
        wgrad_raw(self.dkv.data_ptr(), ld, self.x.data_ptr(), E, gstack.data_ptr(), E, gbstack.data_ptr(), M, K, E, self.device)
        for i, (_, gw, gb) in enumerate(self.parked):
            gw.add_(gstack[i * E2:(i + 1) * E2])
            gb.add_(gbstack[i * E2:(i + 1) * E2])
        self.dkv, self.parked, self.x = None, [], None

    def begin(self):
        cur = torch.cuda.current_stream(self.device)
        if self.event is not None:
            cur.wait_event(self.event)
        acc = self.buf is not None
        if not acc:
            self.buf = torch.empty(self.shape, device=self.device, dtype=F32)
        else:
            self.buf.record_stream(cur)
        return self.buf, acc

    def end(self):
        self.event = torch.cuda.Event()
        self.event.record(torch.cuda.current_stream(self.device))
        self.writers += 1
        return None

    def drain(self):
        cur = torch.cuda.current_stream(self.device)
        if self.event is not None:
            cur.wait_event(self.event)
        if self.parked:
            if self.buf is not None:
                self.buf.record_stream(cur)
            self.dkv.record_stream(cur)
            self._flush_parked()
        out = self.buf
        if out is not None:
            out.record_stream(cur)
        self.buf, self.event, self.writers = None, None, 0
        return out


class _SinkGateFn(torch.autograd.Function):
    @staticmethod
    def forward(ctx, t, sink):
        ctx.sink = sink
        ctx.set_materialize_grads(False)
        return t.view_as(t)

    @staticmethod
    def backward(ctx, g):
        total = ctx.sink.drain()
        if total is None:
            return g, None
        return (total if g is None else total + g), None


def begin_grad_sinks():
    for sk in GradSink.live:
        sk.buf, sk.event, sk.writers = None, None, 0
        sk.dkv, sk.parked, sk.x = None, [], None
    GradSink.live = []


def attach_grad_sink(t, registry=None):
    if not (CTX_GRAD_SINK and t.is_cuda and t.requires_grad and t.dtype == F32 and torch.is_grad_enabled()):
        return t
    sk = GradSink(t.shape, t.device)
    (GradSink.live if registry is None else registry).append(sk)
    out = _SinkGateFn.apply(t, sk)
    out._a3d_sink = sk
    return out


class AttnBlockFn(torch.autograd.Function):
    @staticmethod
    def forward(ctx, q_in, k_in, v_in, resid, q_xyz, k_xyz, kmask, in_w, in_b, out_w, out_b, ln_g, ln_b, H, mode,
                drop=None, site=0, grad_mode=True, sink=None, q_is_resid=False):
        L.require_gpu(q_in, k_in, v_in, resid)
        if drop is not None and drop.p <= 0:
            drop = None
        q_in, k_in, v_in, resid = _c(q_in), _c(k_in), _c(v_in), _c(resid)
        B, Lq, E = q_in.shape
        S = k_in.shape[1]
        dev = q_in.device
        if q_xyz is not None:
            q_xyz, k_xyz = _c(q_xyz.to(F32)), _c(k_xyz.to(F32))
        if kmask is not None:
            kmask = _c(kmask.to(torch.uint8))
        wp, bp = in_w.data_ptr(), in_b.data_ptr()
        f4 = 4
        need_bwd = bool(grad_mode) and (any(ctx.needs_input_grad) or in_w.requires_grad)
        if FUSED_PROJ and E % 4 == 0 and E <= 128:
            fused = attn_operands_fused16 if _use16(Lq, need_bwd) else attn_operands_fused
            Qs, Ks, Vt, Lqp, Sp, scale, freq, extra = fused(mode, q_in, k_in, v_in, wp, bp, q_xyz, k_xyz, B, Lq, S, E, H, dev,
                                                            need_bwd)
        else:
            if mode == "qk":
                qk_pre = linear_raw(q_in.data_ptr(), E, wp, E, bp, B * Lq, 2 * E, E, dev)
                q_ptr, ldq = qk_pre.data_ptr(), 2 * E
                k_ptr, ldk = qk_pre.data_ptr() + E * f4, 2 * E
                v_pre = linear_raw(v_in.data_ptr(), E, wp + 2 * E * E * f4, E, bp + 2 * E * f4, B * S, E, E, dev)
                v_ptr, ldv = v_pre.data_ptr(), E
                keep = (qk_pre, v_pre)
            else:
                q_pre = linear_raw(q_in.data_ptr(), E, wp, E, bp, B * Lq, E, E, dev)
                q_ptr, ldq = q_pre.data_ptr(), E
                if mode == "kv":
                    kv_pre = linear_raw(k_in.data_ptr(), E, wp + E * E * f4, E, bp + E * f4, B * S, 2 * E, E, dev)
                    k_ptr, ldk = kv_pre.data_ptr(), 2 * E
                    v_ptr, ldv = kv_pre.data_ptr() + E * f4, 2 * E
                    keep = (q_pre, kv_pre)
                else:
                    k_pre = linear_raw(k_in.data_ptr(), E, wp + E * E * f4, E, bp + E * f4, B * S, E, E, dev)
                    v_pre = linear_raw(v_in.data_ptr(), E, wp + 2 * E * E * f4, E, bp + 2 * E * f4, B * S, E, E, dev)
                    k_ptr, ldk, v_ptr, ldv = k_pre.data_ptr(), E, v_pre.data_ptr(), E
                    keep = (q_pre, k_pre, v_pre)
            unfused = attn_operands16 if _use16(Lq, need_bwd) else attn_operands
            Qs, Ks, Vt, Lqp, Sp, scale, freq, extra = unfused(q_ptr, ldq, k_ptr, ldk, v_ptr, ldv, q_xyz, k_xyz, B, Lq,
                                                              S, E, H, dev, need_bwd=need_bwd)
            del keep
        nsplit = pick_nsplit(B, H, Lqp, Sp)
        O, LSE = attn_core_fwd(Qs, Ks, Vt, kmask, B, H, Lq, Lqp, S, Sp, nsplit, drop=drop, site=site, need_bwd=need_bwd,
                               nograd=not need_bwd)
        Y = linear2d(O.view(B * Lq, E), out_w, out_b, drop=drop, site=site + 1)
        y, mean, rstd = add_layernorm(resid.view(B * Lq, E), Y, ln_g, ln_b)
        ctx.save_for_backward(q_in, k_in, v_in, resid, Y, mean, rstd, Qs, Ks, Vt, O, LSE,
                              q_xyz if q_xyz is not None else torch.empty(0, device=dev),
                              k_xyz if k_xyz is not None else torch.empty(0, device=dev),
                              kmask if kmask is not None else torch.empty(0, device=dev))
        ctx.params = (in_w, in_b, out_w, out_b, ln_g, ln_b)
        ctx.extra = extra
        ctx.need_bwd = need_bwd
        ctx.drop, ctx.site = drop, site
        ctx.meta = (B, Lq, S, E, H, Lqp, Sp, scale, nsplit, mode, q_xyz is not None, kmask is not None)
        ctx.q_is_resid = bool(q_is_resid)
        ctx.sink = sink if (sink is not None and need_bwd and mode == "kv" and ctx.needs_input_grad[1] and
                            tuple(k_in.shape) == sink.shape) else None
        if ctx.sink is not None:
            ctx.sink.expected += 1
        return y.view(B, Lq, E)

    @staticmethod
    def backward(ctx, dy):
        (q_in, k_in, v_in, resid, Y, mean, rstd, Qs, Ks, Vt, O, LSE, q_xyz, k_xyz, kmask) = ctx.saved_tensors
        in_w, in_b, out_w, out_b, ln_g, ln_b = ctx.params
        B, Lq, S, E, H, Lqp, Sp, scale, nsplit, mode, has_xyz, has_mask = ctx.meta
        dev = dy.device
        if not ctx.need_bwd:
            raise RuntimeError("AttnBlockFn.backward: the forward ran with grad_mode=False (a gradient-free pass: adaptive low part "
                               "of P, no backward operand formats); call it through ops.attn_block or pass "
                               "grad_mode=torch.is_grad_enabled()")
        if not has_xyz:
            q_xyz = k_xyz = None
        if not has_mask:
            kmask = None
        freq = rope_freq(E, dev)
        dy = _c(dy).view(B * Lq, E)
        f4 = 4
        if ctx.drop is None:
            dS = dYo = add_layernorm_bwd(resid.view(B * Lq, E), Y, ln_g, ln_b, mean, rstd, dy)
        else:
            dS, dYo = add_layernorm_bwd(resid.view(B * Lq, E), Y, ln_g, ln_b, mean, rstd, dy, drop=ctx.drop, site=ctx.site + 1)
        dO = dgrad2d(dYo, out_w)
        wgrad2d(dYo, O.view(B * Lq, E), out_w, out_b)
        dQp, dK, dV = attn_core_bwd(Qs, Ks, Vt, kmask, O, dO.view(B, Lq, E), LSE, B, H, Lq, Lqp, S, Sp, nsplit,
                                    extra=ctx.extra, drop=ctx.drop, site=ctx.site)
        gW, gb = grad_buf(in_w), grad_buf(in_b)
        st = L.stream()
        need_q, need_k, need_v = ctx.needs_input_grad[0], ctx.needs_input_grad[1], ctx.needs_input_grad[2]
        d_q_in = d_k_in = d_v_in = None
        fold_q = ctx.q_is_resid and ctx.needs_input_grad[3]
        if mode == "qk":
            dqk = torch.empty((B * Lq, 2 * E), device=dev, dtype=F32)
            rope_merge(dQp, nsplit, q_xyz, freq, scale, dqk.data_ptr(), 2 * E, B, Lq, Lqp, E, H)
            rope_merge(dK, 1, k_xyz, freq, 1.0, dqk.data_ptr() + E * f4, 2 * E, B, S, Sp, E, H)
            dv_pre = torch.empty((B * S, E), device=dev, dtype=F32)
            rope_merge(dV, 1, None, freq, 1.0, dv_pre.data_ptr(), E, B, S, Sp, E, H)
            wgrad_raw(dqk.data_ptr(), 2 * E, q_in.data_ptr(), E, gW.data_ptr(), E, gb.data_ptr(),
                   B * Lq, 2 * E, E, dev, st)
            wgrad_raw(dv_pre.data_ptr(), E, v_in.data_ptr(), E, gW.data_ptr() + 2 * E * E * f4, E,
                   gb.data_ptr() + 2 * E * f4, B * S, E, E, dev, st)
            if (need_q or need_k) and fold_q:
                linear_raw(dqk.data_ptr(), 2 * E, in_w.data_ptr(), E, None, B * Lq, E, 2 * E, dev, act=3, transposed=True, out=dS)
            elif need_q or need_k:
                d_q_in = linear_raw(dqk.data_ptr(), 2 * E, in_w.data_ptr(), E, None, B * Lq, E, 2 * E, dev,
                                    transposed=True).view(B, Lq, E)
            if need_v:
                d_v_in = linear_raw(dv_pre.data_ptr(), E, in_w.data_ptr() + 2 * E * E * f4, E, None, B * S, E, E, dev,
                                    transposed=True).view(B, S, E)
        else:
            dq_pre = torch.empty((B * Lq, E), device=dev, dtype=F32)
            rope_merge(dQp, nsplit, q_xyz, freq, scale, dq_pre.data_ptr(), E, B, Lq, Lqp, E, H)
            wgrad_raw(dq_pre.data_ptr(), E, q_in.data_ptr(), E, gW.data_ptr(), E, gb.data_ptr(),
                   B * Lq, E, E, dev, st)
            if need_q and fold_q:
                dgrad2d(dq_pre, in_w[:E], accum_into=dS)
            elif need_q:
                d_q_in = dgrad2d(dq_pre, in_w[:E]).view(B, Lq, E)
            if mode == "kv" and ctx.sink is not None and CTX_DEFER:
                ptr, ld = ctx.sink.park(k_in, 2 * E)
                rope_merge(dK, 1, k_xyz, freq, 1.0, ptr, ld, B, S, Sp, E, H)
                rope_merge(dV, 1, None, freq, 1.0, ptr + E * f4, ld, B, S, Sp, E, H)
                d_k_in = ctx.sink.parked_done(in_w[E:], gW[E:], gb[E:])
            elif mode == "kv":
                dkv = torch.empty((B * S, 2 * E), device=dev, dtype=F32)
                rope_merge(dK, 1, k_xyz, freq, 1.0, dkv.data_ptr(), 2 * E, B, S, Sp, E, H)
                rope_merge(dV, 1, None, freq, 1.0, dkv.data_ptr() + E * f4, 2 * E, B, S, Sp, E, H)
                wgrad_raw(dkv.data_ptr(), 2 * E, k_in.data_ptr(), E, gW.data_ptr() + E * E * f4, E,
                       gb.data_ptr() + E * f4, B * S, 2 * E, E, dev, st)
                if ctx.sink is not None:
                    buf, acc = ctx.sink.begin()
                    linear_raw(dkv.data_ptr(), 2 * E, in_w.data_ptr() + E * E * f4, E, None, B * S, E, 2 * E, dev,
                               act=3 if acc else 0, transposed=True, out=buf.view(B * S, E))
                    d_k_in = ctx.sink.end()
                elif need_k or need_v:
                    d_k_in = linear_raw(dkv.data_ptr(), 2 * E, in_w.data_ptr() + E * E * f4, E, None, B * S, E, 2 * E,
                                        dev, transposed=True).view(B, S, E)
            else:
                dk_pre = torch.empty((B * S, E), device=dev, dtype=F32)
                dv_pre = torch.empty((B * S, E), device=dev, dtype=F32)
                rope_merge(dK, 1, k_xyz, freq, 1.0, dk_pre.data_ptr(), E, B, S, Sp, E, H)
                rope_merge(dV, 1, None, freq, 1.0, dv_pre.data_ptr(), E, B, S, Sp, E, H)
                wgrad_raw(dk_pre.data_ptr(), E, k_in.data_ptr(), E, gW.data_ptr() + E * E * f4, E,
                       gb.data_ptr() + E * f4, B * S, E, E, dev, st)
                wgrad_raw(dv_pre.data_ptr(), E, v_in.data_ptr(), E, gW.data_ptr() + 2 * E * E * f4,
                       E, gb.data_ptr() + 2 * E * f4, B * S, E, E, dev, st)
                if need_k:
                    d_k_in = dgrad2d(dk_pre, in_w[E:2 * E]).view(B, S, E)
                if need_v:
                    d_v_in = dgrad2d(dv_pre, in_w[2 * E:]).view(B, S, E)
        d_resid = dS.view(B, Lq, E) if ctx.needs_input_grad[3] else None
        return (d_q_in, d_k_in, d_v_in, d_resid) + (None,) * 16


SINGLE_QUERY = os.environ.get("A3D_SINGLE_QUERY", "1") == "1"
SQ_TARGET_WGS = int(os.environ.get("A3D_SQ_WGS", "512"))


def sq_nsplit(B, S):
    return max(1, min((S + 63) // 64, SQ_TARGET_WGS // B))


class SingleQueryAttnBlockFn(torch.autograd.Function):

    @staticmethod
    def forward(ctx, q_in, kv_in, resid, q_xyz, k_xyz, in_w, in_b, out_w, out_b, ln_g, ln_b, H):
        L.require_gpu(q_in, kv_in, resid)
        q_in, kv_in, resid = _c(q_in), _c(kv_in), _c(resid)
        B, _, E = q_in.shape
        S = kv_in.shape[1]
        dev = q_in.device
        f4 = 4
        if q_xyz is not None:
            q_xyz, k_xyz = _c(q_xyz.to(F32)), _c(k_xyz.to(F32))
        freq = rope_freq(E, dev)
        scale = float(E // H) ** -0.5
        wp, bp = in_w.data_ptr(), in_b.data_ptr()
        nz = lambda t: None if t is None else t.data_ptr()
        q_pre = linear_raw(q_in.data_ptr(), E, wp, E, bp, B, E, E, dev)
        qrot = torch.empty((B, H, 1, 16), device=dev, dtype=F32)
        L.call("a3d_rope_rows_f32", q_pre.data_ptr(), E, nz(q_xyz), freq.data_ptr(), scale, qrot.data_ptr(), B, 1, 1, E, H, L.stream())
        nsplit = sq_nsplit(B, S)
        lib = L.load()
        ws = torch.empty((lib.a3d_sq_fwd_ws_floats(B, H, E, nsplit),), device=dev, dtype=F32)
        xbar = torch.empty((B, H, E), device=dev, dtype=F32)
        lse = torch.empty((B, H), device=dev, dtype=F32)
        o = torch.empty((B, E), device=dev, dtype=F32)
        L.call("a3d_sq_attn_fwd", kv_in.data_ptr(), nz(k_xyz), wp + E * E * f4, E, bp + E * f4, wp + 2 * E * E * f4, E,
               bp + 2 * E * f4, qrot.data_ptr(), freq.data_ptr(), ws.data_ptr(), xbar.data_ptr(), lse.data_ptr(), o.data_ptr(), B, S, E,
               H, nsplit, L.stream())
        Y = linear2d(o, out_w, out_b)
        y, mean, rstd = add_layernorm(resid.view(B, E), Y, ln_g, ln_b)
        ctx.save_for_backward(q_in, kv_in, resid, Y, mean, rstd, qrot, xbar, lse, o,
                              q_xyz if q_xyz is not None else torch.empty(0, device=dev),
                              k_xyz if k_xyz is not None else torch.empty(0, device=dev))
        ctx.params = (in_w, in_b, out_w, out_b, ln_g, ln_b)
        ctx.meta = (B, S, E, H, scale, nsplit, q_xyz is not None)
        return y.view(B, 1, E)

    @staticmethod
    def backward(ctx, dy):
        q_in, kv_in, resid, Y, mean, rstd, qrot, xbar, lse, o, q_xyz, k_xyz = ctx.saved_tensors
        in_w, in_b, out_w, out_b, ln_g, ln_b = ctx.params
        B, S, E, H, scale, nsplit, has_xyz = ctx.meta
        dev = dy.device
        f4 = 4
        if not has_xyz:
            q_xyz = k_xyz = None
        freq = rope_freq(E, dev)
        nz = lambda t: None if t is None else t.data_ptr()
        dS = add_layernorm_bwd(resid.view(B, E), Y, ln_g, ln_b, mean, rstd, _c(dy).view(B, E))
        dO = dgrad2d(dS, out_w)
        wgrad2d(dS, o, out_w, out_b)
        gW, gb = grad_buf(in_w), grad_buf(in_b)
        wp, bp = in_w.data_ptr(), in_b.data_ptr()
        lib = L.load()
        ws = torch.empty((lib.a3d_sq_bwd_ws_floats(B, H, E, nsplit),), device=dev, dtype=F32)
        dX = torch.empty((B, S, E), device=dev, dtype=F32)
        dqp = torch.empty((nsplit, B, H, 1, 16), device=dev, dtype=F32)
        L.call("a3d_sq_attn_bwd", kv_in.data_ptr(), nz(k_xyz), wp + E * E * f4, E, bp + E * f4, wp + 2 * E * E * f4, E, qrot.data_ptr(),
# ... 721 lines not shown
```

### include/act3d_hip.h

```cpp
#ifndef ACT3D_HIP_H
#define ACT3D_HIP_H
#include <stddef.h>
#include <stdint.h>
#ifdef __cplusplus
extern "C" {
#endif

int a3d_version(void);
const char* a3d_last_error_string(void);

int a3d_linear_fwd(const float* X, int ldx, const float* W, int ldw, const float* bias, float* Y, int ldy,
                   const float* mask, int ldm, int M, int N, int K, int act, int w_transposed, void* stream);
int a3d_linear_wgrad(const float* dY, int lddy, const float* X, int ldx, float* dW, int lddw, float* db, int M,
                     int N, int K, void* stream);
size_t a3d_linear_wgrad_ws_bytes(int M, int N, int K, int has_bias);
int a3d_linear_wgrad_ws(const float* dY, int lddy, const float* X, int ldx, float* dW, int lddw, float* db, int M,
                        int N, int K, float* ws, size_t ws_bytes, void* stream);
int a3d_add_layernorm_fwd(const float* A, const float* R, const float* gamma, const float* beta, float* Y,
                          float* mean, float* rstd, int M, int E, float eps, void* stream);
int a3d_add_layernorm_bwd(const float* A, const float* R, const float* gamma, const float* mean, const float* rstd,
                          const float* dY, float* dS, float* dgamma, float* dbeta, int M, int E, void* stream);

int a3d_rope_split_qk(const float* Y, int ldy, const float* xyz, const float* freq, float scale, void* dst, int B,
                      int N, int Npad, int E, int H, void* stream);
int a3d_split_vt(const float* Y, int ldy, void* dst, int B, int N, int Npad, int E, int H, void* stream);
int a3d_rope_split(const float* Y, int ldy, const float* xyz, const float* freq, float scale, void* rows_out,
                   int rows_width, void* planes_out, int B, int N, int Npad, int E, int H, void* stream);
int a3d_proj_rope_split(const float* X, int ldx, const float* W, int ldw, const float* bias, int K, const float* xyz0,
                        float scale0, void* rows0, int rows0_width, void* planes0, const float* xyz1, float scale1,
                        void* rows1, int rows1_width, void* planes1, const float* freq, int B, int N, int Npad, int E,
                        int H, void* stream);
int a3d_rope_merge_bwd(const float* dR, int nsplit, const float* xyz, const float* freq, float scale, float* dY,
                       int ldy, int B, int N, int Npad, int E, int H, void* stream);

int a3d_attn_fwd(const void* Qs, const void* Ks, const void* Vt, const unsigned char* kmask, float* O, float* LSE,
                 float* ws, int B, int H, int Lq, int Lqp, int S, int Sp, int nsplit, void* stream);
size_t a3d_attn_fwd_ws_floats(int B, int H, int Lqp, int nsplit);
int a3d_attn_bwd_bf16(const void* Qs, const void* Qt, const void* Ks, const void* Kt, const void* Vs,
                      const unsigned char* kmask, const float* O, const float* dO, const float* LSE, void* dOs,
                      void* dOt, float* D, float* dQp, float* dK, float* dV, int B, int H, int Lq, int Lqp, int S,
                      int Sp, int nsplit, void* stream);

int a3d_dropout(const float* x, float* y, size_t n, const unsigned long long* drop_state, unsigned int site, float p,
                void* stream);
int a3d_linear_fwd_drop(const float* X, int ldx, const float* W, int ldw, const float* bias, float* Y, int ldy,
                        const float* mask, int ldm, int M, int N, int K, int act, int w_transposed,
                        const unsigned long long* drop_state, unsigned int site, float p, void* stream);
int a3d_add_layernorm_bwd_drop(const float* A, const float* R, const float* gamma, const float* mean, const float* rstd,
                               const float* dY, float* dS, float* dS_drop, float* dgamma, float* dbeta, int M, int E,
                               const unsigned long long* drop_state, unsigned int site, float p, void* stream);
int a3d_dropout_mask(unsigned char* out, size_t n, const unsigned long long* drop_state, unsigned int c2, unsigned int c1,
                     unsigned int site, float p, void* stream);
int a3d_rope_split16(const float* Y, int ldy, const float* xyz, const float* freq, float scale, void* rows_out,
                     void* planes_out, int plane_parts, int B, int N, int Npad, int E, int H, void* stream);
int a3d_proj_rope_split16(const float* X, int ldx, const float* W, int ldw, const float* bias, int K, const float* xyz0,
                          float scale0, void* rows0, void* planes0, int parts0, const float* xyz1, float scale1, void* rows1,
                          void* planes1, int parts1, const float* freq, int B, int N, int Npad, int E, int H, void* stream);
int a3d_attn16_fwd(const void* Qr, const void* Kr, const void* Vp, const unsigned char* kmask, float* O, float* LSE2,
                   float* ws, int B, int H, int Lq, int Lqp, int S, int Sp, int nsplit,
                   const unsigned long long* drop_state, unsigned int drop_site, float drop_p, void* stream);
int a3d_attn16_fwd_rows(const void* Qr, const void* Kr, const void* Vr, const unsigned char* kmask, float* O, float* LSE2,
                        float* ws, int B, int H, int Lq, int Lqp, int S, int Sp, int nsplit,
                        const unsigned long long* drop_state, unsigned int drop_site, float drop_p, int nograd, void* stream);
size_t a3d_attn16_bwd_pack_bytes(int B, int H, int Lqp);
int a3d_attn16_bwd(const void* Qr, const void* Qp, const void* Kr, const void* Kp, const void* Vr,
                   const unsigned char* kmask, const float* O, const float* dO, const float* LSE2, void* dOr, void* pack,
                   float* D, int* rexp, float* dQp, float* dK, float* dV, int B, int H, int Lq, int Lqp, int S, int Sp,
                   int nsplit, const unsigned long long* drop_state, unsigned int drop_site, float drop_p, void* stream);

size_t a3d_attn8_operand_bytes(int B, int H, int Sp);
int a3d_attn8_fwd(const void* Qr, const void* Kr, const void* Vp, void* ops8, const unsigned char* kmask, float* O,
                  float* LSE2, float* ws, int B, int H, int Lq, int Lqp, int S, int Sp, int nsplit, void* stream);

int a3d_attn_fwd_dropout(const void* Qs, const void* Ks, const void* Vt, const unsigned char* kmask, float* O, float* LSE,
                         float* ws, int B, int H, int Lq, int Lqp, int S, int Sp, int nsplit,
                         const unsigned long long* drop_state, unsigned int site, float p, void* stream);
int a3d_attn_bwd_bf16_dropout(const void* Qs, const void* Qt, const void* Ks, const void* Kt, const void* Vs,
                              const unsigned char* kmask, const float* O, const float* dO, const float* LSE, void* dOs,
                              void* dOt, float* D, float* dQp, float* dK, float* dV, int B, int H, int Lq, int Lqp, int S,
                              int Sp, int nsplit, const unsigned long long* drop_state, unsigned int site, float p,
                              void* stream);

size_t a3d_sq_fwd_ws_floats(int B, int H, int E, int nsplit);
int a3d_sq_attn_fwd(const float* X, const float* xyz, const float* Wk, int ldw, const float* bk, const float* Wv, int ldwv,
                    const float* bv, const float* qrot, const float* freq, float* ws, float* xbar, float* lse, float* o, int B,
                    int S, int E, int H, int nsplit, void* stream);
size_t a3d_sq_bwd_ws_floats(int B, int H, int E, int nsplit);
int a3d_sq_attn_bwd(const float* X, const float* xyz, const float* Wk, int ldw, const float* bk, const float* Wv, int ldwv,
                    const float* qrot, const float* freq, const float* xbar, const float* lse, const float* dO, float* ws,
                    float* dX, float* dqp, float* dWk, int lddwk, float* dbk, float* dWv, int lddwv, float* dbv, int B, int S,
                    int E, int H, int nsplit, void* stream);
int a3d_sq_attn_bwd_acc(const float* X, const float* xyz, const float* Wk, int ldw, const float* bk, const float* Wv, int ldwv,
                        const float* qrot, const float* freq, const float* xbar, const float* lse, const float* dO, float* ws,
                        float* dX, float* dqp, float* dWk, int lddwk, float* dbk, float* dWv, int lddwv, float* dbv, int B, int S,
                        int E, int H, int nsplit, int accumulate_dX, void* stream);
int a3d_sq_wgrad_reduce(const float* partial, int nsplit, float* dW, int lddw, float* db, int E, void* stream);

int a3d_pcd_downsample(const float* pcd, float* out_xyz, int B, int C, int Hin, int Win, int factor, void* stream);
size_t a3d_knn_topk_ws_bytes(int B, int N);
int a3d_knn_topk(const float* pos, const float* xyz, void* ws, long long* idx_out, float* dist_out, int B, int N,
                 int k, void* stream);
int a3d_traj_nn_topk(const float* traj_xyz, int L, const float* xyz, void* ws, long long* idx_out, float* dist_out, int B,
                     int N, int k, void* stream);
int a3d_build_context(const float* feat, const long long* idx, const float* extra, float* ctx, int B, int Npts,
                      int k, int X, int W, void* stream);
int a3d_build_context_bwd(const float* dctx, const long long* idx, float* dfeat, float* dextra, int B, int Npts,
                          int k, int X, int W, int accumulate, void* stream);

int a3d_build_context_bf16(const void* feat, int ldf, const long long* idx, const float* extra, const float* bias, float* ctx,
                           int B, int Npts, int k, int X, int W, void* stream);
int a3d_build_context_bwd_bf16(const float* dctx, const long long* idx, void* dfeat, int ldf, float* dextra, int B,
                               int Npts, int k, int X, int W, int accumulate, void* stream);
size_t a3d_conv3x3_wgrad_tokens_ws_floats(void);
int a3d_conv3x3_wgrad_tokens(const void* X, const long long* idx, const float* G, int g_rows, int E, float* ws, float* dW,
                             int accumulate, int B, int k, int ncam, int H, int W, void* stream);
size_t a3d_conv3x3_tile_count(size_t images, int H, int W);
size_t a3d_conv3x3_dgrad_tiles_ws_ints(size_t images, int H, int W);
int a3d_conv3x3_mark_tiles(const long long* idx, int B, int k, int ncam, int H, int W, unsigned char* mask, void* stream);
int a3d_conv3x3_dgrad_tiles(const void* dy, const void* wt, const unsigned char* mask, int* ws, void* dx, size_t images, int H, int W,
                            void* stream);
size_t a3d_colsum_rows_ws_floats(int B, int k, int C);
int a3d_colsum_rows(const float* src, int B, int S, int k, int ld, int C, float* out, int nout, float* ws, void* stream);

int a3d_mask_logits_fwd(const float* q, const float* F, float* out, int B, int Ng, int E, void* stream);
int a3d_mask_logits_bwd(const float* q, const float* F, const float* dlog, float* dF, float* dq, int B, int Ng,
                        int E, int accumulate_dF, void* stream);
int a3d_argmax_gather(const float* logits, const float* ghost, long long* top_idx, float* pos, int B, int Ng,
                      void* stream);
int a3d_soft_ce_loss(const float* ghost, const float* gt, const float* logits, float* loss_b, float* loss,
                     float* dlogits, int B, int Ng, float spread, float label_smoothing, float coeff, void* stream);
int a3d_elem_loss(const float* pred, const float* target, int n, int kind, float coeff, float* loss, float* grad,
                  void* stream);
int a3d_scale_by_scalar(const float* x, const float* scalar, float* y, size_t n, void* stream);
int a3d_quat_sigmoid_fwd(const float* pred, float* rot, float* grip, int B, void* stream);
int a3d_quat_sigmoid_bwd(const float* pred, const float* drot, const float* dgrip, float* dpred, int B, void* stream);
int a3d_ortho6d_sigmoid_fwd(const float* pred, float* rot, float* grip, int B, void* stream);
int a3d_ortho6d_sigmoid_bwd(const float* pred, const float* drot, const float* dgrip, float* dpred, int B, void* stream);
int a3d_select_row_fwd(const float* x, const long long* idx, float* y, int B, int N, int W, void* stream);
int a3d_select_row_bwd(const float* dy, const long long* idx, float* dx, int B, int N, int W, void* stream);
int a3d_sample_ghost_points(const unsigned long long* state, const float* bounds, const float* anchor, float radius,
                            float* out, int B, int Ng, int level, int max_attempts, void* stream);
int a3d_rng_advance(unsigned long long* state, unsigned long long n, void* stream);
void a3d_philox4x32_10_host(const uint32_t ctr[4], const uint32_t key[2], uint32_t out[4]);
void a3d_sincos_host(const float* x, float* sn, float* cs, size_t n);
int a3d_adamw_step(float* p, const float* g, float* m, float* v, float* step, const long long* seg_off, float* seg_state,
                   int nseg, size_t n, size_t n_nodecay, float lr, float beta1, float beta2, float eps, float wd_nodecay,
                   float wd_decay, float grad_scale, void* stream);

typedef struct {
  const float *wv, *bv;
  const float *wo, *bo;
// ... 161 lines not shown
```

Before: 3478 samples/s.

## Fuse rope-merge of context dK/dV into attention bwd and rotating GEMM loaders

The attention backward dK/dV kernel can now write unrotated, unpadded per-row gradients straight into the merged context rows. The bf16x3 linear dgrad and wgrad kernels gain a rotating loader that applies the rotary transform while loading, and a sliced wgrad reduce writes each parked block's weight gradient directly. Together these remove the separate rope_merge passes and their padded dK/dV intermediates for the kv-context cross-attention. In exchange the GEMM loaders do more work and there are new fallback paths with warnings when a block's rotation does not match.

```diff
diff --git a/act3d-chained-diffuser_amd/csrc/a3d_common.h b/act3d-chained-diffuser_amd/csrc/a3d_common.h
--- a/act3d-chained-diffuser_amd/csrc/a3d_common.h
+++ b/act3d-chained-diffuser_amd/csrc/a3d_common.h
@@ -189,4 +189,10 @@
 int conv1x1_deep_launch(const void* x, const void* w, const float* in_scale, const float* in_shift, int in_relu, void* y, float* partial,
                         size_t M, int K, int N, hipStream_t s);
 
+struct RotArgs {
+  const float* xyz;
+  const float* freq;
+  int period, width, third;
+};
+
 }
diff --git a/act3d-chained-diffuser_amd/csrc/attention16.hip b/act3d-chained-diffuser_amd/csrc/attention16.hip
--- a/act3d-chained-diffuser_amd/csrc/attention16.hip
+++ b/act3d-chained-diffuser_amd/csrc/attention16.hip
@@ -674,9 +674,9 @@
 template <bool DROP, int KT, int GP>
 __global__ __launch_bounds__(256, 2) void attn16_bwd_dkv_kernel(
     const unsigned short* __restrict__ pack, const unsigned short* __restrict__ Kr, const unsigned short* __restrict__ Vr,
-    const unsigned char* __restrict__ kmask, float* __restrict__ dK, float* __restrict__ dV, int B, int H, int Lqp, int S,
-    int Sp, const unsigned long long* __restrict__ drop_state, unsigned int drop_site, unsigned int drop_thr,
-    float drop_scale) {
+    const unsigned char* __restrict__ kmask, float* __restrict__ dK, float* __restrict__ dV, float* __restrict__ dKm,
+    float* __restrict__ dVm, int ldm, int B, int H, int Lqp, int S, int Sp, const unsigned long long* __restrict__ drop_state,
+    unsigned int drop_site, unsigned int drop_thr, float drop_scale) {
   __shared__ __attribute__((aligned(16))) unsigned short pk[DKV_NB][PK_HALFS];
   __shared__ __attribute__((aligned(16))) unsigned char maskS[2][DROP ? 8 * KT * C16 : 16];
   const int t = threadIdx.x, lane = t & 63;
@@ -869,6 +869,14 @@
     f32x4 dk, dv;
 #pragma unroll
     for (int r = 0; r < 4; ++r) { dk[r] = (dk0[u][r] + dk1[u][r]) * sk; dv[r] = (dv0[u][r] + dv1[u][r]) * sv; }
+    if (dKm) {
+      if (key[u] >= S) continue;
+      const size_t o = ((size_t)b * S + key[u]) * ldm + h * HD + g * 4;
+#pragma unroll
+      for (int r = 0; r < 4; ++r)
+        if (g * 4 + r < HD) { dKm[o + r] = dk[r]; dVm[o + r] = dv[r]; }
+      continue;
+    }
     *reinterpret_cast<f32x4*>(&dK[(bh * Sp + key[u]) * HDP + g * 4]) = dk;
     *reinterpret_cast<f32x4*>(&dV[(bh * Sp + key[u]) * HDP + g * 4]) = dv;
   }
@@ -980,11 +988,25 @@
                               void* pack, float* D, int* rexp, float* dQp, float* dK, float* dV, int B, int H, int Lq,
                               int Lqp, int S, int Sp, int nsplit, const unsigned long long* drop_state,
                               unsigned int drop_site, float drop_p, void* stream) {
+  return a3d_attn16_bwd_merged(Qr, Qp, Kr, Kp, Vr, kmask, O, dO, LSE2, dOr, pack, D, rexp, dQp, dK, dV, B, H, Lq, Lqp, S, Sp, nsplit,
+                               drop_state, drop_site, drop_p, nullptr, nullptr, 0, stream);
+}
+
+extern "C" int a3d_attn16_bwd_merged(const void* Qr, const void* Qp, const void* Kr, const void* Kp, const void* Vr,
+                                     const unsigned char* kmask, const float* O, const float* dO, const float* LSE2, void* dOr,
+                                     void* pack, float* D, int* rexp, float* dQp, float* dK, float* dV, int B, int H, int Lq,
+                                     int Lqp, int S, int Sp, int nsplit, const unsigned long long* drop_state,
+                                     unsigned int drop_site, float drop_p, float* dKm, float* dVm, int ldm, void* stream) {
   int rc = attn16_check_shapes("a3d_attn16_bwd", B, H, Lq, Lqp, S, Sp, nsplit, 64);
   if (rc) return rc;
   (void)Qp; (void)Kp;
-  if (!Qr || !Kr || !Vr || !O || !dO || !LSE2 || !dOr || !pack || !D || !rexp || !dQp || !dK || !dV) {
+  const bool merged = dKm != nullptr || dVm != nullptr;
+  if (!Qr || !Kr || !Vr || !O || !dO || !LSE2 || !dOr || !pack || !D || !rexp || !dQp || (merged ? (!dKm || !dVm) : (!dK || !dV))) {
     set_error("a3d_attn16_bwd: null pointer");
+    return A3D_ERR_ARG;
+  }
+  if (merged && ldm < H * HD) {
+    set_error("a3d_attn16_bwd_merged: row stride %d of the merged rows is below H * 15 = %d", ldm, H * HD);
     return A3D_ERR_ARG;
   }
   bool drop; unsigned int thr; float dscale;
@@ -1020,8 +1042,8 @@
                      (const unsigned short*)dOr, LSE2, D, rexp, dQp, B, H, Lq, Lqp, S, Sp, nsplit, ST, SITE, THR, SC)
 #define A3D_L16K_(DROPV, KTV, GPV, ST, SITE, THR, SC)                                                                     \
   hipLaunchKernelGGL((attn16_bwd_dkv_kernel<DROPV, KTV, GPV>), gk, dim3(256), 0, s, (const unsigned short*)pack,         \
-                     (const unsigned short*)Kr, (const unsigned short*)Vr, kmask, dK, dV, B, H, Lqp, S, Sp, ST, SITE,    \
-                     THR, SC)
+                     (const unsigned short*)Kr, (const unsigned short*)Vr, kmask, dK, dV, dKm, dVm, ldm, B, H, Lqp, S, \
+                     Sp, ST, SITE, THR, SC)
 #define A3D_L16Q(DROPV, QTV, ST, SITE, THR, SC) \
   do { if (fast) A3D_L16Q_(DROPV, QTV, 1, ST, SITE, THR, SC); else A3D_L16Q_(DROPV, QTV, 2, ST, SITE, THR, SC); } while (0)
 #define A3D_L16K(DROPV, KTV, ST, SITE, THR, SC) \
diff --git a/act3d-chained-diffuser_amd/csrc/linear.hip b/act3d-chained-diffuser_amd/csrc/linear.hip
--- a/act3d-chained-diffuser_amd/csrc/linear.hip
+++ b/act3d-chained-diffuser_amd/csrc/linear.hip
@@ -7,10 +7,12 @@
 bool linear_split_applicable(const float* X, int ldx, const float* W, int ldw, const float* bias, const float* Y, int ldy,
                              const float* mask, int ldm, int M, int N, int K, int act);
 int linear_split_launch(const float* X, int ldx, const float* W, int ldw, const float* bias, float* Y, int ldy, const float* mask,
-                        int ldm, int M, int N, int K, int act, int w_transposed, hipStream_t s);
+                        int ldm, int M, int N, int K, int act, int w_transposed, const RotArgs& rot, hipStream_t s);
 bool linear_wgrad_split_applicable(const float* dY, int lddy, const float* X, int ldx, int M);
+bool linear_split_serves_rows(int M);
+bool linear_wgrad_split_serves_rows(int M);
 int linear_wgrad_split_launch(const float* dY, int lddy, const float* X, int ldx, int has_bias, int M, int N, int K, int nsplit,
-                              int rows_per_split, float* partial, hipStream_t s);
+                              int rows_per_split, float* partial, const RotArgs& rot, hipStream_t s);
 
 constexpr int LT_BM = 64;
 constexpr int LT_BN = 64;
@@ -213,13 +215,9 @@
   }
 }
 
-__global__ __launch_bounds__(1024) void wgrad_reduce_kernel(const float* __restrict__ partial, int nsplit,
-                                                            float* __restrict__ dW, int lddw, float* __restrict__ db,
-                                                            int N, int K, int KE) {
+__device__ __forceinline__ bool wgrad_slab_sum(const float* __restrict__ partial, int nsplit, int total, int idx, float* v_out) {
   __shared__ float red[16][64];
   const int lane = threadIdx.x & 63, zg = threadIdx.x >> 6;
-  const int idx = blockIdx.x * 64 + lane;
-  const int total = N * KE;
   float s0 = 0.f, s1 = 0.f;
   if (idx < total) {
     int z = zg;
@@ -231,13 +229,43 @@
   }
   red[zg][lane] = s0 + s1;
   __syncthreads();
-  if (zg != 0 || idx >= total) return;
+  if (zg != 0 || idx >= total) return false;
   float v = 0.f;
 #pragma unroll
   for (int u = 0; u < 16; ++u) v += red[u][lane];
+  *v_out = v;
+  return true;
+}
+
+__global__ __launch_bounds__(1024) void wgrad_reduce_kernel(const float* __restrict__ partial, int nsplit,
+                                                            float* __restrict__ dW, int lddw, float* __restrict__ db,
+                                                            int N, int K, int KE) {
+  const int idx = blockIdx.x * 64 + (threadIdx.x & 63);
+  float v;
+  if (!wgrad_slab_sum(partial, nsplit, N * KE, idx, &v)) return;
   const int n = idx / KE, k = idx - n * KE;
   if (k < K) dW[(size_t)n * lddw + k] += v;
   else db[n] += v;
+}
+
+constexpr int WG_MAX_SLICES = 8;
+struct WgradSlices {
+  float* dW[WG_MAX_SLICES];
+  float* db[WG_MAX_SLICES];
+};
+__global__ __launch_bounds__(1024) void wgrad_reduce_slices_kernel(const float* __restrict__ partial, int nsplit, WgradSlices dst,
+                                                                   int lddw, int slice_rows, int N, int K, int KE) {
+  const int idx = blockIdx.x * 64 + (threadIdx.x & 63);
+  float v;
+  if (!wgrad_slab_sum(partial, nsplit, N * KE, idx, &v)) return;
+  const int n = idx / KE, k = idx - n * KE;
+  const int sl = n / slice_rows, nl = n - sl * slice_rows;
+  float *dW = dst.dW[0], *db = dst.db[0];
+#pragma unroll
+  for (int i = 1; i < WG_MAX_SLICES; ++i)
+    if (sl == i) { dW = dst.dW[i]; db = dst.db[i]; }
+  if (k < K) dW[(size_t)nl * lddw + k] += v;
+  else db[nl] += v;
 }
 
 __global__ __launch_bounds__(256) void add_ln_fwd_kernel(
@@ -431,7 +459,7 @@
   dim3 grid(cdiv(M, LT_BM), cdiv(N, LT_BN));
   hipStream_t s = (hipStream_t)stream;
   if (linear_split_applicable(X, ldx, W, ldw, bias, Y, ldy, mask, ldm, M, N, K, act))
-    return linear_split_launch(X, ldx, W, ldw, bias, Y, ldy, mask, ldm, M, N, K, act, w_transposed, s);
+    return linear_split_launch(X, ldx, W, ldw, bias, Y, ldy, mask, ldm, M, N, K, act, w_transposed, RotArgs{nullptr, nullptr, 1, 0, 1}, s);
   if (w_transposed)
     hipLaunchKernelGGL((linear_fwd_kernel<true, false>), grid, dim3(256), 0, s, X, ldx, W, ldw, bias, Y, ldy, mask, ldm, M, N, K, act,
                        (const unsigned long long*)nullptr, 0u, 0u, 0.f);
@@ -439,6 +467,42 @@
     hipLaunchKernelGGL((linear_fwd_kernel<false, false>), grid, dim3(256), 0, s, X, ldx, W, ldw, bias, Y, ldy, mask, ldm, M, N, K, act,
                        (const unsigned long long*)nullptr, 0u, 0u, 0.f);
   return check_launch("a3d_linear_fwd");
+}
+
+static int rot_args(const char* fn, const float* rot_xyz, const float* rot_freq, int rot_period, int rot_width, int rot_E, int cols,
+                    RotArgs* out) {
+  *out = RotArgs{nullptr, nullptr, 1, 0, 1};
+  if (!rot_xyz) return A3D_OK;
+  const int third = rot_E / 3;
+  if (!rot_freq || rot_period <= 0 || rot_width <= 0 || rot_E <= 0 || (rot_period & 3) || (rot_width & 3) || (rot_E % 3) ||
+      (third & 3) || rot_width > rot_period || rot_width > rot_E || (cols & 3)) {
+    set_error("%s: bad rotation (period=%d width=%d E=%d over rows of %d columns; need period %% 4 == 0, width %% 4 == 0, "
+              "width <= min(period, E), (E / 3) %% 4 == 0, columns %% 4 == 0 and the frequency table)", fn, rot_period, rot_width,
+              rot_E, cols);
+    return A3D_ERR_ARG;
+  }
+  *out = RotArgs{rot_xyz, rot_freq, rot_period, rot_width, third};
+  return A3D_OK;
+}
+
+extern "C" int a3d_linear_fwd_rot(const float* X, int ldx, const float* W, int ldw, const float* bias, float* Y, int ldy,
+                                  const float* mask, int ldm, int M, int N, int K, int act, int w_transposed,
+                                  const float* rot_xyz, const float* rot_freq, int rot_period, int rot_width, int rot_E,
+                                  void* stream) {
+  if (!X || !W || !Y || M < 0 || N <= 0 || K <= 0 || ldx < K || ldy < N) {
+    set_error("a3d_linear_fwd_rot: bad argument (M=%d N=%d K=%d ldx=%d ldy=%d)", M, N, K, ldx, ldy);
+    return A3D_ERR_ARG;
+  }
+  if (act == 2 && !mask) { set_error("a3d_linear_fwd_rot: act=2 needs a mask"); return A3D_ERR_ARG; }
+  RotArgs rot;
+  const int rc = rot_args("a3d_linear_fwd_rot", rot_xyz, rot_freq, rot_period, rot_width, rot_E, K, &rot);
+  if (rc) return rc;
+  if (!linear_split_applicable(X, ldx, W, ldw, bias, Y, ldy, mask, ldm, M, N, K, act)) {
+    set_error("a3d_linear_fwd_rot: M=%d N=%d K=%d is not served by the bf16x3 kernel (M >= 4096, N, K >= 32 and %% 4 == 0, 16-byte "
+              "aligned rows, A3D_LINEAR_SPLIT != 0); the exact-f32 kernel has no rotating loader", M, N, K);
+    return A3D_ERR_ARG;
+  }
+  return linear_split_launch(X, ldx, W, ldw, bias, Y, ldy, mask, ldm, M, N, K, act, w_transposed, rot, (hipStream_t)stream);
 }
 
 static int linear_drop_params(const char* fn, float p, uint32_t* thr16, float* scale) {
@@ -510,33 +574,90 @@
   return two ? (size_t)nsplit * N * KE * sizeof(float) : 0;
 }
 
+static int wgrad_ws_impl(const char* fn, const float* dY, int lddy, const float* X, int ldx, float* dW, int lddw, float* db,
+                         const WgradSlices* slices, int slice_rows, bool has_bias, int M, int N, int K, float* ws, size_t ws_bytes,
+                         const RotArgs& rot, bool need_split, void* stream) {
+  if (M == 0) return A3D_OK;
+  const int KE = has_bias ? K + 1 : K;
+  int nsplit, rows;
+  bool two_stage;
+  wgrad_plan(M, N, KE, ws != nullptr, &nsplit, &rows, &two_stage);
+  if (two_stage && ws_bytes < (size_t)nsplit * N * KE * sizeof(float)) {
+    set_error("%s: workspace too small (%zu bytes, need %zu)", fn, ws_bytes, (size_t)nsplit * N * KE * sizeof(float));
+    return A3D_ERR_ARG;
+  }
+  dim3 grid(cdiv(N, 64), cdiv(KE, 64), nsplit);
+  if (two_stage && linear_wgrad_split_applicable(dY, lddy, X, ldx, M)) {
+    const int rc = linear_wgrad_split_launch(dY, lddy, X, ldx, has_bias, M, N, K, nsplit, rows, ws, rot, (hipStream_t)stream);
+    if (rc) return rc;
+  } else if (need_split) {
+    set_error("%s: M=%d is not served by the two-stage bf16x3 kernel (M >= 4096, a workspace, 16-byte aligned rows, "
+              "A3D_LINEAR_SPLIT != 0); the exact-f32 kernel has neither the rotating loader nor the slice reduce", fn, M);
+    return A3D_ERR_ARG;
+  } else
+  hipLaunchKernelGGL(linear_wgrad_kernel, grid, dim3(256), 0, (hipStream_t)stream, dY, lddy, X, ldx, dW,
+                     lddw, db, M, N, K, rows, two_stage ? ws : nullptr);
+  if (two_stage && slices)
+    hipLaunchKernelGGL(wgrad_reduce_slices_kernel, dim3(cdiv(N * KE, 64)), dim3(1024), 0, (hipStream_t)stream, ws, nsplit, *slices,
+                       lddw, slice_rows, N, K, KE);
+  else if (two_stage)
+    hipLaunchKernelGGL(wgrad_reduce_kernel, dim3(cdiv(N * KE, 64)), dim3(1024), 0, (hipStream_t)stream, ws, nsplit, dW,
+                       lddw, db, N, K, KE);
+  return check_launch(fn);
+}
+
 extern "C" int a3d_linear_wgrad_ws(const float* dY, int lddy, const float* X, int ldx, float* dW, int lddw,
                                    float* db, int M, int N, int K, float* ws, size_t ws_bytes, void* stream) {
   if (!dY || !X || !dW || M < 0 || N <= 0 || K <= 0) {
     set_error("a3d_linear_wgrad: bad argument (M=%d N=%d K=%d)", M, N, K);
     return A3D_ERR_ARG;
   }
-  if (M == 0) return A3D_OK;
-  const int KE = db ? K + 1 : K;
-  int nsplit, rows;
-  bool two_stage;
-  wgrad_plan(M, N, KE, ws != nullptr, &nsplit, &rows, &two_stage);
-  if (two_stage && ws_bytes < (size_t)nsplit * N * KE * sizeof(float)) {
-    set_error("a3d_linear_wgrad_ws: workspace too small (%zu bytes, need %zu)", ws_bytes,
-              (size_t)nsplit * N * KE * sizeof(float));
-    return A3D_ERR_ARG;
-  }
-  dim3 grid(cdiv(N, 64), cdiv(KE, 64), nsplit);
-  if (two_stage && linear_wgrad_split_applicable(dY, lddy, X, ldx, M)) {
-    const int rc = linear_wgrad_split_launch(dY, lddy, X, ldx, db != nullptr, M, N, K, nsplit, rows, ws, (hipStream_t)stream);
-    if (rc) return rc;
-  } else
-  hipLaunchKernelGGL(linear_wgrad_kernel, grid, dim3(256), 0, (hipStream_t)stream, dY, lddy, X, ldx, dW,
-                     lddw, db, M, N, K, rows, two_stage ? ws : nullptr);
-  if (two_stage)
-    hipLaunchKernelGGL(wgrad_reduce_kernel, dim3(cdiv(N * KE, 64)), dim3(1024), 0, (hipStream_t)stream, ws, nsplit, dW,
-                       lddw, db, N, K, KE);
-  return check_launch("a3d_linear_wgrad");
+  return wgrad_ws_impl("a3d_linear_wgrad", dY, lddy, X, ldx, dW, lddw, db, nullptr, 0, db != nullptr, M, N, K, ws, ws_bytes,
+                       RotArgs{nullptr, nullptr, 1, 0, 1}, false, stream);
+}
+
+extern "C" int a3d_linear_wgrad_ws_rot(const float* dY, int lddy, const float* X, int ldx, float* dW, int lddw, float* db, int M,
+                                       int N, int K, float* ws, size_t ws_bytes, const float* rot_xyz, const float* rot_freq,
+                                       int rot_period, int rot_width, int rot_E, void* stream) {
+  if (!dY || !X || !dW || M < 0 || N <= 0 || K <= 0) {
+    set_error("a3d_linear_wgrad_ws_rot: bad argument (M=%d N=%d K=%d)", M, N, K);
+    return A3D_ERR_ARG;
+  }
+  RotArgs rot;
+  const int rc = rot_args("a3d_linear_wgrad_ws_rot", rot_xyz, rot_freq, rot_period, rot_width, rot_E, N, &rot);
+  if (rc) return rc;
+  return wgrad_ws_impl("a3d_linear_wgrad_ws_rot", dY, lddy, X, ldx, dW, lddw, db, nullptr, 0, db != nullptr, M, N, K, ws, ws_bytes,
+                       rot, true, stream);
+}
+
+extern "C" int a3d_linear_wgrad_ws_rot_slices(const float* dY, int lddy, const float* X, int ldx, float* const* dW_slices,
+                                              int lddw, float* const* db_slices, int n_slices, int M, int N, int K, float* ws,
+                                              size_t ws_bytes, const float* rot_xyz, const float* rot_freq, int rot_period,
+                                              int rot_width, int rot_E, void* stream) {
+  if (!dY || !X || !dW_slices || M < 0 || N <= 0 || K <= 0 || n_slices < 1 || n_slices > WG_MAX_SLICES || (N % n_slices) != 0) {
+    set_error("a3d_linear_wgrad_ws_rot_slices: bad argument (M=%d N=%d K=%d in %d slices; 1 .. %d slices of N / slices rows)", M, N,
+              K, n_slices, WG_MAX_SLICES);
+    return A3D_ERR_ARG;
+  }
+  WgradSlices sl;
+  for (int i = 0; i < WG_MAX_SLICES; ++i) {
+    sl.dW[i] = i < n_slices ? dW_slices[i] : nullptr;
+    sl.db[i] = (i < n_slices && db_slices) ? db_slices[i] : nullptr;
+    if (i < n_slices && (!sl.dW[i] || (db_slices && !sl.db[i]))) {
+      set_error("a3d_linear_wgrad_ws_rot_slices: null gradient pointer of slice %d", i);
+      return A3D_ERR_ARG;
+    }
+  }
+  RotArgs rot;
+  const int rc = rot_args("a3d_linear_wgrad_ws_rot_slices", rot_xyz, rot_freq, rot_period, rot_width, rot_E, N, &rot);
+  if (rc) return rc;
+  return wgrad_ws_impl("a3d_linear_wgrad_ws_rot_slices", dY, lddy, X, ldx, nullptr, lddw, nullptr, &sl, N / n_slices,
+                       db_slices != nullptr, M, N, K, ws, ws_bytes, rot, true, stream);
+}
+
+extern "C" int a3d_linear_rot_serves(int M, int ld) {
+  return (M > 0 && ld > 0 && (ld & 3) == 0 && linear_split_serves_rows(M) && linear_wgrad_split_serves_rows(M) &&
+          M >= wg_two_stage_min_rows()) ? 1 : 0;
 }
 
 extern "C" int a3d_sq_wgrad_reduce(const float* partial, int nsplit, float* dW, int lddw, float* db, int E, void* stream) {
diff --git a/act3d-chained-diffuser_amd/csrc/linear_split.hip b/act3d-chained-diffuser_amd/csrc/linear_split.hip
--- a/act3d-chained-diffuser_amd/csrc/linear_split.hip
+++ b/act3d-chained-diffuser_amd/csrc/linear_split.hip
@@ -16,10 +16,22 @@
   l = __builtin_bit_cast(unsigned int, __builtin_convertvector((ls_f32x2){ra, rb}, ls_bf16x2));
 }
 
-template <int WN, bool WT>
+__device__ __forceinline__ void unrotate2(float& g0, float& g1, float th) {
+  float sn, cs;
+  fast_sincos(th, &sn, &cs);
+  const float a0 = g0, a1 = g1;
+  g0 = add_rn(mul_rn(cs, a0), mul_rn(sn, a1));
+  g1 = __builtin_fmaf(cs, a1, -mul_rn(sn, a0));
+}
+__device__ __forceinline__ void unrotate4(float4& v, float x, float f0, float f1) {
+  unrotate2(v.x, v.y, mul_rn(x, f0));
+  unrotate2(v.z, v.w, mul_rn(x, f1));
+}
+
+template <int WN, bool WT, bool ROT>
 __global__ __launch_bounds__(256, 2) void linear_split_kernel(
     const float* __restrict__ X, int ldx, const float* __restrict__ W, int ldw, const float* __restrict__ bias,
-    float* __restrict__ Y, int ldy, const float* __restrict__ mask, int ldm, int M, int N, int K, int act) {
+    float* __restrict__ Y, int ldy, const float* __restrict__ mask, int ldm, int M, int N, int K, int act, RotArgs rot) {
   constexpr int WM = 4 / WN, BM = 32 * WM, BN = 64 * WN;
   constexpr int XL = BM * 8 / 256, WL = BN * 8 / 256;
   __shared__ __attribute__((aligned(16))) unsigned short Xs[3][BM * 32];
@@ -39,12 +51,27 @@
     return make_float4(p[0], p[1], p[2], p[3]);
   };
   float4 xr[XL], wr[WL];
+  float xrot[XL], rf0 = 0.f, rf1 = 0.f;
+  bool rot_on = false;
   auto load = [&](int ks) {
+    int axis = 0;
+    if (ROT && rot.xyz) {
+      const int k = ks * 32 + (t & 7) * 4;
+      const int c = (int)((unsigned)k % (unsigned)rot.period);
+      rot_on = k < K && c < rot.width;
+      if (rot_on) {
+        axis = c / rot.third;
+        const int j = (c - axis * rot.third) >> 1;
+        rf0 = rot.freq[j];
+        rf1 = rot.freq[j + 1];
+      }
+    }
 #pragma unroll
     for (int i = 0; i < XL; ++i) {
       const int idx = t + i * 256, row = idx >> 3, k = ks * 32 + (idx & 7) * 4;
       const int m = min(m0 + row, M - 1);
       xr[i] = (k < K) ? *reinterpret_cast<const float4*>(X + (size_t)m * ldx + k) : make_float4(0.f, 0.f, 0.f, 0.f);
+      if (ROT && rot_on) xrot[i] = rot.xyz[(size_t)m * 3 + axis];
     }
 #pragma unroll
     for (int i = 0; i < WL; ++i) {
@@ -65,6 +92,7 @@
     for (int i = 0; i < XL; ++i) {
       const int idx = t + i * 256, row = idx >> 3, s4 = idx & 7;
       unsigned int h0, m0_, l0, h1, m1, l1;
+      if (ROT && rot_on) unrotate4(xr[i], xrot[i], rf0, rf1);
       split3(xr[i].x, xr[i].y, h0, m0_, l0);
       split3(xr[i].z, xr[i].w, h1, m1, l1);
       const int off = plane_off(row, s4 >> 1) + (s4 & 1) * 4;
@@ -159,32 +187,42 @@
   }
 }
 
+bool linear_split_serves_rows(int M) {
+  static const bool on = !(getenv("A3D_LINEAR_SPLIT") && atoi(getenv("A3D_LINEAR_SPLIT")) == 0);
+  static const int min_m = getenv("A3D_LINEAR_SPLIT_MIN_M") ? atoi(getenv("A3D_LINEAR_SPLIT_MIN_M")) : 4096;
+  return on && M >= min_m;
+}
+bool linear_wgrad_split_serves_rows(int M) {
+  static const bool on = !(getenv("A3D_WGRAD_SPLIT") && atoi(getenv("A3D_WGRAD_SPLIT")) == 0);
+  return on && linear_split_serves_rows(M);
+}
+
 bool linear_split_applicable(const float* X, int ldx, const float* W, int ldw, const float* bias, const float* Y, int ldy,
                              const float* mask, int ldm, int M, int N, int K, int act) {
-  static const bool on = !(getenv("A3D_LINEAR_SPLIT") && atoi(getenv("A3D_LINEAR_SPLIT")) == 0);
-  static const int min_m = getenv("A3D_LINEAR_SPLIT_MIN_M") ? atoi(getenv("A3D_LINEAR_SPLIT_MIN_M")) : 4096;
-  if (!on || M < min_m || K < 32 || N < 32 || (K & 3) || (N & 3) || ((ldx | ldy) & 3)) return false;
+  if (!linear_split_serves_rows(M) || K < 32 || N < 32 || (K & 3) || (N & 3) || ((ldx | ldy) & 3)) return false;
   if ((((uintptr_t)X | (uintptr_t)Y) & 15) != 0) return false;
   if (act == 2 && (!mask || (ldm & 3) || (((uintptr_t)mask) & 15) != 0)) return false;
   return true;
 }
 
 int linear_split_launch(const float* X, int ldx, const float* W, int ldw, const float* bias, float* Y, int ldy, const float* mask,
-                        int ldm, int M, int N, int K, int act, int w_transposed, hipStream_t s) {
+                        int ldm, int M, int N, int K, int act, int w_transposed, const RotArgs& rot, hipStream_t s) {
   const bool wide = N > 64;
   const int BM = wide ? 64 : 128, BN = wide ? 128 : 64;
   dim3 grid(xcd_grid(cdiv(M, BM), cdiv(N, BN)));
 #define A3D_LS(WNV, WTV) \
-  hipLaunchKernelGGL((linear_split_kernel<WNV, WTV>), grid, dim3(256), 0, s, X, ldx, W, ldw, bias, Y, ldy, mask, ldm, M, N, K, act)
+  do { if (rot.xyz) hipLaunchKernelGGL((linear_split_kernel<WNV, WTV, true>), grid, dim3(256), 0, s, X, ldx, W, ldw, bias, Y, ldy, mask, ldm, M, N, K, act, rot); \
+       else hipLaunchKernelGGL((linear_split_kernel<WNV, WTV, false>), grid, dim3(256), 0, s, X, ldx, W, ldw, bias, Y, ldy, mask, ldm, M, N, K, act, rot); } while (0)
   if (wide) { if (w_transposed) A3D_LS(2, true); else A3D_LS(2, false); }
   else { if (w_transposed) A3D_LS(1, true); else A3D_LS(1, false); }
 #undef A3D_LS
   return check_launch("a3d_linear_fwd(split)");
 }
 
+template <bool ROT>
 __global__ __launch_bounds__(256, 2) void linear_wgrad_split_kernel(
     const float* __restrict__ dY, int lddy, const float* __restrict__ X, int ldx, int has_bias, int M, int N, int K,
-    int rows_per_split, float* __restrict__ partial) {
+    int rows_per_split, float* __restrict__ partial, RotArgs rot) {
   __shared__ __attribute__((aligned(16))) unsigned short Ys[3][64 * 32];
   __shared__ __attribute__((aligned(16))) unsigned short Xt[3][64 * 32];
   const int t = threadIdx.x, lane = t & 63, wave = t >> 6;
@@ -207,11 +245,25 @@
     return v;
   };
   float4 yr[2], xr[2];
+  float yrot[2] = {0.f, 0.f}, rf0 = 0.f, rf1 = 0.f;
+  bool rot_on = false;
+  int axis = 0;
+  if (ROT && rot.xyz) {
+    const int c = (int)((unsigned)(n0 + c4) % (unsigned)rot.period);
+    rot_on = n0 + c4 < N && c < rot.width;
+    if (rot_on) {
+      axis = c / rot.third;
+      const int j = (c - axis * rot.third) >> 1;
+      rf0 = rot.freq[j];
+      rf1 = rot.freq[j + 1];
+    }
+  }
   auto load = [&](int mb) {
 #pragma unroll
     for (int u = 0; u < 2; ++u) {
       yr[u] = ld4(dY, lddy, mb + 2 * mp + u, n0 + c4, N, false);
       xr[u] = ld4(X, ldx, mb + 2 * mp + u, k0 + c4, K, has_bias != 0);
+      if (ROT && rot_on) yrot[u] = rot.xyz[(size_t)min(mb + 2 * mp + u, mend - 1) * 3 + axis];
     }
   };
   auto stage_one = [&](unsigned short (*T)[64 * 32], const float4& r0, const float4& r1) {
@@ -233,6 +285,7 @@
   load(mbeg);
   for (int mb = mbeg; mb < mend; mb += 32) {
     if (mb > mbeg) __syncthreads();
+    if (ROT && rot_on) { unrotate4(yr[0], yrot[0], rf0, rf1); unrotate4(yr[1], yrot[1], rf0, rf1); }
     stage_one(Ys, yr[0], yr[1]);
     stage_one(Xt, xr[0], xr[1]);
     __syncthreads();
@@ -269,17 +322,17 @@
 }
 
 bool linear_wgrad_split_applicable(const float* dY, int lddy, const float* X, int ldx, int M) {
-  static const bool on = !(getenv("A3D_LINEAR_SPLIT") && atoi(getenv("A3D_LINEAR_SPLIT")) == 0) &&
-                         !(getenv("A3D_WGRAD_SPLIT") && atoi(getenv("A3D_WGRAD_SPLIT")) == 0);
-  static const int min_m = getenv("A3D_LINEAR_SPLIT_MIN_M") ? atoi(getenv("A3D_LINEAR_SPLIT_MIN_M")) : 4096;
-  return on && M >= min_m && ((lddy | ldx) & 3) == 0 && ((((uintptr_t)dY | (uintptr_t)X) & 15) == 0);
+  return linear_wgrad_split_serves_rows(M) && ((lddy | ldx) & 3) == 0 && ((((uintptr_t)dY | (uintptr_t)X) & 15) == 0);
 }
 
 int linear_wgrad_split_launch(const float* dY, int lddy, const float* X, int ldx, int has_bias, int M, int N, int K, int nsplit,
-                              int rows_per_split, float* partial, hipStream_t s) {
+                              int rows_per_split, float* partial, const RotArgs& rot, hipStream_t s) {
   const int KE = has_bias ? K + 1 : K;
   dim3 grid(cdiv(N, 64), cdiv(KE, 64), nsplit);
-  hipLaunchKernelGGL(linear_wgrad_split_kernel, grid, dim3(256), 0, s, dY, lddy, X, ldx, has_bias, M, N, K, rows_per_split, partial);
+  if (rot.xyz)
+    hipLaunchKernelGGL(linear_wgrad_split_kernel<true>, grid, dim3(256), 0, s, dY, lddy, X, ldx, has_bias, M, N, K, rows_per_split, partial, rot);
+  else
+    hipLaunchKernelGGL(linear_wgrad_split_kernel<false>, grid, dim3(256), 0, s, dY, lddy, X, ldx, has_bias, M, N, K, rows_per_split, partial, rot);
   return check_launch("a3d_linear_wgrad(split)");
 }
 
diff --git a/act3d-chained-diffuser_amd/lib.py b/act3d-chained-diffuser_amd/lib.py
--- a/act3d-chained-diffuser_amd/lib.py
+++ b/act3d-chained-diffuser_amd/lib.py
@@ -39,6 +39,10 @@
     "a3d_linear_wgrad": (_i, [_p, _i, _p, _i, _p, _i, _p, _i, _i, _i, _p]),
     "a3d_linear_wgrad_ws": (_i, [_p, _i, _p, _i, _p, _i, _p, _i, _i, _i, _p, _z, _p]),
     "a3d_linear_wgrad_ws_bytes": (_z, [_i, _i, _i, _i]),
+    "a3d_linear_rot_serves": (_i, [_i, _i]),
+    "a3d_linear_fwd_rot": (_i, [_p, _i, _p, _i, _p, _p, _i, _p, _i, _i, _i, _i, _i, _i, _p, _p, _i, _i, _i, _p]),
+    "a3d_linear_wgrad_ws_rot": (_i, [_p, _i, _p, _i, _p, _i, _p, _i, _i, _i, _p, _z, _p, _p, _i, _i, _i, _p]),
+    "a3d_linear_wgrad_ws_rot_slices": (_i, [_p, _i, _p, _i, _p, _i, _p, _i, _i, _i, _i, _p, _z, _p, _p, _i, _i, _i, _p]),
     "a3d_add_layernorm_fwd": (_i, [_p, _p, _p, _p, _p, _p, _p, _i, _i, _f, _p]),
     "a3d_add_layernorm_bwd": (_i, [_p, _p, _p, _p, _p, _p, _p, _p, _p, _i, _i, _p]),
     "a3d_rope_split_qk": (_i, [_p, _i, _p, _p, _f, _p, _i, _i, _i, _i, _i, _p]),
@@ -64,6 +68,7 @@
     "a3d_attn8_operand_bytes": (_z, [_i, _i, _i]),
     "a3d_attn8_fwd": (_i, [_p] * 8 + [_i] * 7 + [_p]),
     "a3d_attn16_bwd": (_i, [_p] * 16 + [_i] * 7 + [_p, C.c_uint, _f, _p]),
+    "a3d_attn16_bwd_merged": (_i, [_p] * 16 + [_i] * 7 + [_p, C.c_uint, _f, _p, _p, _i, _p]),
     "a3d_pose_to_signal": (_i, [_p, _p, _p, _i, _i, _p]),
     "a3d_signal_to_pose": (_i, [_p, _p, _p, _i, _i, _p]),
     "a3d_traj_condition": (_i, [_p, _i, _p, _i, _p] + [_p] * 8 + [_i] * 5 + [_p]),
diff --git a/act3d-chained-diffuser_amd/ops.py b/act3d-chained-diffuser_amd/ops.py
--- a/act3d-chained-diffuser_amd/ops.py
+++ b/act3d-chained-diffuser_amd/ops.py
@@ -1,5 +1,7 @@
+import ctypes
 import math
 import os
+import warnings
 
 import torch
 
@@ -38,8 +40,15 @@
 
 
 def linear_raw(x_ptr, ldx, W_ptr, ldw, b_ptr, M, N, K, device, act=0, mask_ptr=None, ldm=0, transposed=False,
-               out=None, drop=None, site=0):
+               out=None, drop=None, site=0, rot=None):
     y = out if out is not None else torch.empty((M, N), device=device, dtype=F32)
+    if rot is not None:
+        if drop is not None:
+            raise ValueError("linear_raw: the rotating loader has no dropout form")
+        xyz, freq, period, width, E = rot
+        L.call("a3d_linear_fwd_rot", x_ptr, ldx, W_ptr, ldw, b_ptr, y.data_ptr(), N, mask_ptr, ldm, M, N, K, act,
+               1 if transposed else 0, None if xyz is None else xyz.data_ptr(), freq.data_ptr(), period, width, E, L.stream())
+        return y
     if drop is not None and DROP_FOLD:
         L.call("a3d_linear_fwd_drop", x_ptr, ldx, W_ptr, ldw, b_ptr, y.data_ptr(), N, mask_ptr, ldm, M, N, K, act,
                1 if transposed else 0, drop.state.data_ptr(), int(site), drop.p, L.stream())
@@ -73,9 +82,21 @@
                       ldm=K, transposed=True, drop=drop, site=site)
 
 
-def wgrad_raw(dy_ptr, lddy, x_ptr, ldx, gw_ptr, lddw, gb_ptr, M, N, K, device, st=None):
-    nbytes = L.load().a3d_linear_wgrad_ws_bytes(M, N, K, 0 if gb_ptr is None else 1)
+def wgrad_raw(dy_ptr, lddy, x_ptr, ldx, gw_ptr, lddw, gb_ptr, M, N, K, device, st=None, rot=None, slices=None):
+    nbytes = L.load().a3d_linear_wgrad_ws_bytes(M, N, K, 0 if (gb_ptr is None and slices is None) else 1)
     ws = torch.empty((nbytes // 4,), device=device, dtype=F32) if nbytes else None
+    if rot is not None or slices is not None:
+        xyz, freq, period, width, E = rot if rot is not None else (None, None, 0, 0, 0)
+        tail = (None if ws is None else ws.data_ptr(), nbytes, None if xyz is None else xyz.data_ptr(),
+                None if freq is None else freq.data_ptr(), period, width, E, st if st is not None else L.stream())
+        if slices is None:
+            L.call("a3d_linear_wgrad_ws_rot", dy_ptr, lddy, x_ptr, ldx, gw_ptr, lddw, gb_ptr, M, N, K, *tail)
+        else:
+            gws, gbs = slices
+            tw = (ctypes.c_void_p * len(gws))(*[g.data_ptr() for g in gws])
+            tb = (ctypes.c_void_p * len(gbs))(*[g.data_ptr() for g in gbs])
+            L.call("a3d_linear_wgrad_ws_rot_slices", dy_ptr, lddy, x_ptr, ldx, tw, lddw, tb, len(gws), M, N, K, *tail)
+        return
     L.call("a3d_linear_wgrad_ws", dy_ptr, lddy, x_ptr, ldx, gw_ptr, lddw, gb_ptr, M, N, K,
            None if ws is None else ws.data_ptr(), nbytes, st if st is not None else L.stream())
 
@@ -351,13 +372,15 @@
     return O, LSE
 
 
-def attn_core_bwd(Qs, Ks, Vt, kmask, O, dO, LSE, B, H, Lq, Lqp, S, Sp, nsplit, extra=None, drop=None, site=0):
+def attn_core_bwd(Qs, Ks, Vt, kmask, O, dO, LSE, B, H, Lq, Lqp, S, Sp, nsplit, extra=None, drop=None, site=0, dkv_out=None):
     dev = Qs.device
     dropping = drop is not None and drop.p > 0
     D = torch.empty((B, H, Lqp), device=dev, dtype=F32)
     dQp = torch.empty((nsplit, B, H, Lqp, 16), device=dev, dtype=F32)
-    dK = torch.empty((B, H, Sp, 16), device=dev, dtype=F32)
-    dV = torch.empty((B, H, Sp, 16), device=dev, dtype=F32)
+    if dkv_out is not None and Qs.dtype != torch.float16:
+        raise RuntimeError("attn_core_bwd: only the split-fp16 kernels write merged dK / dV rows")
+    dK = torch.empty((B, H, Sp, 16), device=dev, dtype=F32) if dkv_out is None else None
+    dV = torch.empty((B, H, Sp, 16), device=dev, dtype=F32) if dkv_out is None else None
     km = None if kmask is None else kmask.data_ptr()
     if Qs.dtype == torch.float16:
         if extra is None or extra[2] is None:
@@ -366,10 +389,13 @@
         dOr = torch.empty((B, H, Lqp, 32), device=dev, dtype=torch.float16)
         dOp = torch.empty((L.load().a3d_attn16_bwd_pack_bytes(B, H, Lqp) // 2,), device=dev, dtype=torch.float16)
         rexp = torch.empty((B, H, Lqp), device=dev, dtype=torch.int32)
-        L.call("a3d_attn16_bwd", Qs.data_ptr(), None, Ks.data_ptr(), None, Vr.data_ptr(), km, O.data_ptr(),
-               dO.data_ptr(), LSE.data_ptr(), dOr.data_ptr(), dOp.data_ptr(), D.data_ptr(), rexp.data_ptr(), dQp.data_ptr(),
-               dK.data_ptr(), dV.data_ptr(), B, H, Lq, Lqp, S, Sp, nsplit, drop.state.data_ptr() if dropping else None,
-               int(site), drop.p if dropping else 0.0, L.stream())
+        head = (Qs.data_ptr(), None, Ks.data_ptr(), None, Vr.data_ptr(), km, O.data_ptr(),
+                dO.data_ptr(), LSE.data_ptr(), dOr.data_ptr(), dOp.data_ptr(), D.data_ptr(), rexp.data_ptr(), dQp.data_ptr())
+        tail = (B, H, Lq, Lqp, S, Sp, nsplit, drop.state.data_ptr() if dropping else None, int(site), drop.p if dropping else 0.0)
+        if dkv_out is None:
+            L.call("a3d_attn16_bwd", *head, dK.data_ptr(), dV.data_ptr(), *tail, L.stream())
+        else:
+            L.call("a3d_attn16_bwd_merged", *head, None, None, *tail, dkv_out[0], dkv_out[1], dkv_out[2], L.stream())
         return dQp, dK, dV
     if extra is None or extra[0] is None:
         raise RuntimeError("attn_core_bwd: the forward wrote no backward operand formats (it ran with need_bwd=False)")
@@ -397,6 +423,16 @@
 CTX_DEFER = os.environ.get("A3D_CTX_DEFER", "1") not in ("0", "", "off")
 
 
+CTX_MERGED = os.environ.get("A3D_CTX_MERGED", "1") not in ("0", "", "off")
+CTX_MERGED_MIN_ROWS = 4096
+CTX_MERGED_MAX_BLOCKS = 8
+
+
+def ctx_merged_serves(M, E, blocks=1):
+    return bool(CTX_MERGED and M >= CTX_MERGED_MIN_ROWS and blocks <= CTX_MERGED_MAX_BLOCKS and
+                L.load().a3d_linear_rot_serves(M, 2 * E))
+
+
 class GradSink:
     live = []
 
@@ -406,8 +442,21 @@
         self.writers = 0
         self.expected = 0
         self.dkv, self.parked, self.x = None, [], None
-
-    def park(self, x, E2):
+        self.rot, self.rot_freq = None, None
+        self.merged = False
+
+    def parks_rotated(self, xyz):
+        if not self.parked:
+            return True
+        if self.rot is None or xyz is None:
+            return self.rot is None and xyz is None
+        return self.rot.data_ptr() == xyz.data_ptr() and self.rot.shape == xyz.shape
+
+    def park(self, x, E2, rot_xyz=None, rot_freq=None, merged=False):
+        assert self.parks_rotated(rot_xyz), "GradSink.park: the parked blocks of one context must share k_xyz"
+        if not self.parked:
+            self.rot, self.rot_freq, self.merged = rot_xyz, rot_freq, False
+        self.merged = self.merged or merged
         cur = torch.cuda.current_stream(self.device)
         if self.event is not None:
             cur.wait_event(self.event)
@@ -434,6 +483,15 @@
         acc = self.buf is not None
         if not acc:
             self.buf = torch.empty(self.shape, device=self.device, dtype=F32)
+        if self.merged:
+            rot = (self.rot, self.rot_freq if self.rot_freq is not None else rope_freq(E, self.device), E2, E, E)
+            linear_raw(self.dkv.data_ptr(), ld, wstack.data_ptr(), E, None, M, E, K, self.device, act=3 if acc else 0,
+                       transposed=True, out=self.buf.view(M, E), rot=rot)
+            wgrad_raw(self.dkv.data_ptr(), ld, self.x.data_ptr(), E, None, self.parked[0][1].stride(0), None, M, K, E, self.device,
+                      rot=rot, slices=([gw for _, gw, _ in self.parked], [gb for _, _, gb in self.parked]))
+            self.dkv, self.parked, self.x, self.rot, self.rot_freq = None, [], None, None, None
+            return
+        assert self.rot is None
         linear_raw(self.dkv.data_ptr(), ld, wstack.data_ptr(), E, None, M, E, K, self.device, act=3 if acc else 0, transposed=True,
                    out=self.buf.view(M, E))
         gstack = torch.zeros((K, E), device=self.device, dtype=F32)
@@ -495,7 +553,7 @@
 def begin_grad_sinks():
     for sk in GradSink.live:
         sk.buf, sk.event, sk.writers = None, None, 0
-        sk.dkv, sk.parked, sk.x = None, [], None
+        sk.dkv, sk.parked, sk.x, sk.rot, sk.rot_freq = None, [], None, None, None
     GradSink.live = []
 
 
@@ -600,8 +658,28 @@
             dS, dYo = add_layernorm_bwd(resid.view(B * Lq, E), Y, ln_g, ln_b, mean, rstd, dy, drop=ctx.drop, site=ctx.site + 1)
         dO = dgrad2d(dYo, out_w)
         wgrad2d(dYo, O.view(B * Lq, E), out_w, out_b)
+        defer = mode == "kv" and ctx.sink is not None and CTX_DEFER
+        merged = (mode == "kv" and Qs.dtype == torch.float16 and
+                  ctx_merged_serves(B * S, E, ctx.sink.expected if defer else 1))
+        if merged and defer and not ctx.sink.parks_rotated(k_xyz):
+            merged = False
+            warnings.warn("merged context gradients: this block's k_xyz is not the tensor the context's parked rows are rotated by; "
+                          "it takes head records + a3d_rope_merge_bwd", RuntimeWarning)
+        if defer and not merged and not ctx.sink.parks_rotated(None):
+            defer = False
+            warnings.warn("merged context gradients: a block that cannot park rotated rows next to the context's merged blocks "
+                          "runs its own input- and weight-gradient GEMMs", RuntimeWarning)
+        dkv, dkv_out, krot = None, None, None
+        if merged:
+            krot = (k_xyz, freq, 2 * E, E, E)
+            if defer:
+                ptr, ld = ctx.sink.park(k_in, 2 * E, k_xyz, freq, merged=True)
+            else:
+                dkv = torch.empty((B * S, 2 * E), device=dev, dtype=F32)
+                ptr, ld = dkv.data_ptr(), 2 * E
+            dkv_out = (ptr, ptr + E * f4, ld)
         dQp, dK, dV = attn_core_bwd(Qs, Ks, Vt, kmask, O, dO.view(B, Lq, E), LSE, B, H, Lq, Lqp, S, Sp, nsplit,
-                                    extra=ctx.extra, drop=ctx.drop, site=ctx.site)
+                                    extra=ctx.extra, drop=ctx.drop, site=ctx.site, dkv_out=dkv_out)
         gW, gb = grad_buf(in_w), grad_buf(in_b)
         st = L.stream()
         need_q, need_k, need_v = ctx.needs_input_grad[0], ctx.needs_input_grad[1], ctx.needs_input_grad[2]
@@ -634,25 +712,27 @@
                 dgrad2d(dq_pre, in_w[:E], accum_into=dS)
             elif need_q:
                 d_q_in = dgrad2d(dq_pre, in_w[:E]).view(B, Lq, E)
-            if mode == "kv" and ctx.sink is not None and CTX_DEFER:
-                ptr, ld = ctx.sink.park(k_in, 2 * E)
-                rope_merge(dK, 1, k_xyz, freq, 1.0, ptr, ld, B, S, Sp, E, H)
-                rope_merge(dV, 1, None, freq, 1.0, ptr + E * f4, ld, B, S, Sp, E, H)
+            if defer:
+                if not merged:
+                    ptr, ld = ctx.sink.park(k_in, 2 * E)
+                    rope_merge(dK, 1, k_xyz, freq, 1.0, ptr, ld, B, S, Sp, E, H)
+                    rope_merge(dV, 1, None, freq, 1.0, ptr + E * f4, ld, B, S, Sp, E, H)
                 d_k_in = ctx.sink.parked_done(in_w[E:], gW[E:], gb[E:])
             elif mode == "kv":
-                dkv = torch.empty((B * S, 2 * E), device=dev, dtype=F32)
-                rope_merge(dK, 1, k_xyz, freq, 1.0, dkv.data_ptr(), 2 * E, B, S, Sp, E, H)
-                rope_merge(dV, 1, None, freq, 1.0, dkv.data_ptr() + E * f4, 2 * E, B, S, Sp, E, H)
+                if not merged:
+                    dkv = torch.empty((B * S, 2 * E), device=dev, dtype=F32)
+                    rope_merge(dK, 1, k_xyz, freq, 1.0, dkv.data_ptr(), 2 * E, B, S, Sp, E, H)
+                    rope_merge(dV, 1, None, freq, 1.0, dkv.data_ptr() + E * f4, 2 * E, B, S, Sp, E, H)
                 wgrad_raw(dkv.data_ptr(), 2 * E, k_in.data_ptr(), E, gW.data_ptr() + E * E * f4, E,
-                       gb.data_ptr() + E * f4, B * S, 2 * E, E, dev, st)
+                       gb.data_ptr() + E * f4, B * S, 2 * E, E, dev, st, rot=krot)
                 if ctx.sink is not None:
                     buf, acc = ctx.sink.begin()
                     linear_raw(dkv.data_ptr(), 2 * E, in_w.data_ptr() + E * E * f4, E, None, B * S, E, 2 * E, dev,
-                               act=3 if acc else 0, transposed=True, out=buf.view(B * S, E))
+                               act=3 if acc else 0, transposed=True, out=buf.view(B * S, E), rot=krot)
                     d_k_in = ctx.sink.end()
                 elif need_k or need_v:
                     d_k_in = linear_raw(dkv.data_ptr(), 2 * E, in_w.data_ptr() + E * E * f4, E, None, B * S, E, 2 * E,
-                                        dev, transposed=True).view(B, S, E)
+                                        dev, transposed=True, rot=krot).view(B, S, E)
             else:
                 dk_pre = torch.empty((B * S, E), device=dev, dtype=F32)
                 dv_pre = torch.empty((B * S, E), device=dev, dtype=F32)
diff --git a/include/act3d_hip.h b/include/act3d_hip.h
--- a/include/act3d_hip.h
+++ b/include/act3d_hip.h
@@ -16,6 +16,17 @@
 size_t a3d_linear_wgrad_ws_bytes(int M, int N, int K, int has_bias);
 int a3d_linear_wgrad_ws(const float* dY, int lddy, const float* X, int ldx, float* dW, int lddw, float* db, int M,
                         int N, int K, float* ws, size_t ws_bytes, void* stream);
+int a3d_linear_rot_serves(int M, int ld);
+int a3d_linear_fwd_rot(const float* X, int ldx, const float* W, int ldw, const float* bias, float* Y, int ldy,
+                       const float* mask, int ldm, int M, int N, int K, int act, int w_transposed, const float* rot_xyz,
+                       const float* rot_freq, int rot_period, int rot_width, int rot_E, void* stream);
+int a3d_linear_wgrad_ws_rot(const float* dY, int lddy, const float* X, int ldx, float* dW, int lddw, float* db, int M,
+                            int N, int K, float* ws, size_t ws_bytes, const float* rot_xyz, const float* rot_freq,
+                            int rot_period, int rot_width, int rot_E, void* stream);
+int a3d_linear_wgrad_ws_rot_slices(const float* dY, int lddy, const float* X, int ldx, float* const* dW_slices, int lddw,
+                                   float* const* db_slices, int n_slices, int M, int N, int K, float* ws, size_t ws_bytes,
+                                   const float* rot_xyz, const float* rot_freq, int rot_period, int rot_width, int rot_E,
+                                   void* stream);
 int a3d_add_layernorm_fwd(const float* A, const float* R, const float* gamma, const float* beta, float* Y,
                           float* mean, float* rstd, int M, int E, float eps, void* stream);
 int a3d_add_layernorm_bwd(const float* A, const float* R, const float* gamma, const float* mean, const float* rstd,
@@ -67,6 +78,11 @@
                    const unsigned char* kmask, const float* O, const float* dO, const float* LSE2, void* dOr, void* pack,
                    float* D, int* rexp, float* dQp, float* dK, float* dV, int B, int H, int Lq, int Lqp, int S, int Sp,
                    int nsplit, const unsigned long long* drop_state, unsigned int drop_site, float drop_p, void* stream);
+int a3d_attn16_bwd_merged(const void* Qr, const void* Qp, const void* Kr, const void* Kp, const void* Vr,
+                          const unsigned char* kmask, const float* O, const float* dO, const float* LSE2, void* dOr, void* pack,
+                          float* D, int* rexp, float* dQp, float* dK, float* dV, int B, int H, int Lq, int Lqp, int S, int Sp,
+                          int nsplit, const unsigned long long* drop_state, unsigned int drop_site, float drop_p, float* dKm,
+                          float* dVm, int ldm, void* stream);
 
 size_t a3d_attn8_operand_bytes(int B, int H, int Sp);
 int a3d_attn8_fwd(const void* Qr, const void* Kr, const void* Vp, void* ops8, const unsigned char* kmask, float* O,
```

Result: no change. 3476 samples/s (-0.1%).
